# uber-research/UPSNet

Hardware: AMD Instinct MI355X
Metric: images/sec (whole node), UPSNet-50 1024x2048 (higher is better)
Workload: dtype f32

## Files before the change

include/upsnet_hip.h:

```cpp
#ifndef UPSNET_HIP_H
#define UPSNET_HIP_H

#include <stddef.h>
#include <stdint.h>

#ifdef __cplusplus
extern "C" {
#endif

const char *upsnet_last_error(void);
const char *upsnet_last_kernel_form(void);
int upsnet_abi_version(void);

int upsnet_zero_fill(void *stream, void *ptr, size_t bytes);


int upsnet_roi_align_forward(void *stream, const float *bottom_data, float spatial_scale, int num_rois,
                             int height, int width, int channels, int pooled_height, int pooled_width,
                             int sampling_ratio, const float *bottom_rois, float *top_data);

int upsnet_roi_align_forward_nhwc(void *stream, const float *feat_nhwc, int batch, int height, int width,
                                  int channels, float spatial_scale, const float *rois, int num_rois,
                                  int pooled_height, int pooled_width, int sampling_ratio, float *out_nhwc);

int upsnet_fpn_roi_align_forward(void *stream, const float *const feat_nhwc[4], const int feat_h[4],
                                 const int feat_w[4], const float spatial_scale[4], int channels,
                                 const float *rois, int num_rois, const int *num_rois_dev, int pooled_height,
                                 int pooled_width, int sampling_ratio, float *out_nhwc, int *levels_out);

int upsnet_fpn_roi_order(void *stream, const float *rois, int num_rois, const int *num_rois_dev, int image_height, int image_width,
                         int *order_out);
int upsnet_fpn_roi_align_forward_ordered(void *stream, const float *const feat_nhwc[4], const int feat_h[4], const int feat_w[4],
                                         const float spatial_scale[4], int channels, const float *rois, int num_rois, const int *num_rois_dev,
                                         int pooled_height, int pooled_width, int sampling_ratio, float *out_nhwc, int *levels_out,
                                         const int *order);

void upsnet_roi_tuning(int variant);
void upsnet_roi_geometry(int target_workgroups, int min_bins);


int upsnet_deform_im2col(void *stream, const float *data_im, const float *data_offset, int channels,
                         int height, int width, int ksize_h, int ksize_w, int pad_h, int pad_w, int stride_h,
                         int stride_w, int dilation_h, int dilation_w, int parallel_imgs, int deformable_group,
                         float *data_col);

int upsnet_mod_deform_im2col(void *stream, const float *data_im, const float *data_offset,
                             const float *data_mask, int batch_size, int channels, int height_im, int width_im,
                             int height_col, int width_col, int kernel_h, int kernel_w, int pad_h, int pad_w,
                             int stride_h, int stride_w, int dilation_h, int dilation_w, int deformable_group,
                             float *data_col);


int upsnet_roi_align_backward(void *stream, const float *top_diff, float spatial_scale, int batch_size, int num_rois,
                              int height, int width, int channels, int pooled_height, int pooled_width,
                              int sampling_ratio, const float *bottom_rois, float *bottom_diff);

int upsnet_deform_col2im(void *stream, const float *data_col, const float *data_offset, int channels, int height,
                         int width, int ksize_h, int ksize_w, int pad_h, int pad_w, int stride_h, int stride_w,
                         int dilation_h, int dilation_w, int parallel_imgs, int deformable_group, float *grad_im);

int upsnet_deform_col2im_coord(void *stream, const float *data_col, const float *data_im, const float *data_offset,
                               int channels, int height, int width, int ksize_h, int ksize_w, int pad_h, int pad_w,
                               int stride_h, int stride_w, int dilation_h, int dilation_w, int parallel_imgs,
                               int deformable_group, float *grad_offset);

int upsnet_mod_deform_col2im(void *stream, const float *data_col, const float *data_offset, const float *data_mask,
                             int batch_size, int channels, int height_im, int width_im, int height_col, int width_col,
                             int kernel_h, int kernel_w, int pad_h, int pad_w, int stride_h, int stride_w,
                             int dilation_h, int dilation_w, int deformable_group, float *grad_im);

int upsnet_mod_deform_col2im_coord(void *stream, const float *data_col, const float *data_im, const float *data_offset,
                                   const float *data_mask, int batch_size, int channels, int height_im, int width_im,
                                   int height_col, int width_col, int kernel_h, int kernel_w, int pad_h, int pad_w,
                                   int stride_h, int stride_w, int dilation_h, int dilation_w, int deformable_group,
                                   float *grad_offset, float *grad_mask);

int upsnet_deform_conv_forward_nhwc(void *stream, int nlev, const float *const x[], const float *const offset[],
                                    const float *const mask[], float *const out[], const int height[],
                                    const int width[], int cin, int cout, int kh, int kw, int pad_h, int pad_w,
                                    int stride_h, int stride_w, int dil_h, int dil_w, int deformable_group,
                                    const float *wpack, int ldw, const float *bias, int relu);

size_t upsnet_dcn_packed_weight_floats(int cout, int cin, int kh, int kw);
int upsnet_dcn_pack_weight(void *stream, const float *weight, int cout, int cin, int kh, int kw, float *wpack);
int upsnet_deform_conv_fused_nhwc(void *stream, int nlev, const float *const x[], const float *const offset[],
                                  const float *const mask[], float *const out[], const int height[], const int width[],
                                  int cin, int cout, int kh, int kw, int pad, int stride, int dil, const float *wpack,
                                  const float *bias, int relu);
size_t upsnet_deform_conv_fused_splitk_workspace_bytes(int height, int width, int cout, int kh, int kw, int pad, int stride, int dil,
                                                       int ksplit);
int upsnet_deform_conv_fused_nhwc_splitk(void *stream, const float *x, const float *offset, const float *mask, float *out, int height,
                                         int width, int cin, int cout, int kh, int kw, int pad, int stride, int dil,
                                         const float *wpack, const float *bias, int relu, int ksplit, void *workspace);
void upsnet_dcn_tuning(int variant);

size_t upsnet_dcn_packed_weight_bf16_elems(int cout, int cin, int kh, int kw);
int upsnet_dcn_pack_weight_bf16(void *stream, const float *weight, int cout, int cin, int kh, int kw, void *wpack);
int upsnet_deform_conv_fused_nhwc_bf16(void *stream, int nlev, const float *const x[], const float *const offset[],
                                       const float *const mask[], float *const out[], const int height[], const int width[], int cin,
                                       int cout, int kh, int kw, int pad, int stride, int dil, const void *wpack, const float *bias,
                                       int relu);


int upsnet_prep_image_u8(void *stream, const unsigned char *image_hwc, int height, int width, const double pixel_means[3],
                         double im_scale, int resized_h, int resized_w, int padded_h, int padded_w, int nhwc4, float *blob);

int upsnet_image_to_nhwc4(void *stream, const float *nchw, int batch, int channels, int height, int width, float *nhwc4);


int upsnet_conv2d_nhwc_f32_multiw(void *stream, int nseg, const float *const x[], float *const out[], const int batch[],
                                  const int height[], const int width[], int Cin, const float *const wpack[], int ldw, int Cout,
                                  int KH, int KW, int stride, int pad, int relu);

int upsnet_conv2d_nhwc_f32(void *stream, int nseg, const float *const x[], const float *const residual[],
                           float *const out[], const int batch[], const int height[], const int width[], int Cin,
                           const float *wpack, int ldw, const float *bias, int Cout, int KH, int KW, int stride, int pad,
                           int relu, int residual_up);

size_t upsnet_conv2d_splitk_workspace_bytes(int batch, int height, int width, int Cout, int KH, int KW, int stride, int pad, int ksplit);
int upsnet_conv2d_nhwc_f32_splitk(void *stream, const float *x, const float *residual, float *out, int batch, int height, int width,
                                  int Cin, const float *wpack, int ldw, const float *bias, int Cout, int KH, int KW, int stride,
                                  int pad, int relu, int ksplit, void *workspace);

int upsnet_conv2d_winograd_nhwc_f32(void *stream, int nseg, const float *const x[], const float *const residual[],
                                    float *const out[], const int batch[], const int height[], const int width[], int Cin,
                                    const float *wpack, int ldw, const float *bias, int Cout, int relu);

int upsnet_conv2d_winograd_nhwc_f32_splitk(void *stream, const float *x, const float *residual, float *out, int batch, int height,
                                           int width, int Cin, const float *wpack, int ldw, const float *bias, int Cout, int relu,
                                           int ksplit, void *workspace);
int upsnet_conv_pack_weight_winograd(void *stream, const float *weight, int cout, int cin, int ldw, float *wpack);

int upsnet_conv2d_winograd_nhwc_f32_tn32(void *stream, int nseg, const float *const x[], const float *const residual[],
                                         float *const out[], const int batch[], const int height[], const int width[], int Cin,
                                         const float *wpack, int ldw, const float *bias, int Cout, int relu);
int upsnet_conv_pack_weight_winograd_tn32(void *stream, const float *weight, int cout, int cin, int ldw, float *wpack);
int upsnet_conv2d_winograd_nhwc_f32_tail(void *stream, const float *x, float *out, int batch, int n_main, int height, int width, int Cin,
                                         const float *wpack, int ldw, const float *wpack32, int ldw32, const float *bias, int Cout, int relu);

int upsnet_conv2d_nhwc_bf16(void *stream, int nseg, const void *const x[], const void *const residual[], void *const out[],
                            const int batch[], const int height[], const int width[], int Cin, const void *wpack_hi,
                            const void *wpack_lo, int ldw, const float *bias, int Cout, int KH, int KW, int stride, int pad,
                            int relu);
int upsnet_conv_pack_weight_bf16(void *stream, const float *weight, int cout, int cin, int kh, int kw, int ldw, void *wpack_hi,
                                 void *wpack_lo);
int upsnet_bottleneck_proj_bf16(void *stream, const void *x, void *out, int batch, int height_in, int width_in, int cin, int cmid, int stride,
                                const void *w1, const void *w2, const void *w3d, const float *b1, const float *b2, const float *b3d);
int upsnet_conv_bf16_tuning(int enable, int tile_rows);
int upsnet_conv1x1_bf16_tuning(int enable);
int upsnet_stem_pool_pack_weight_f32(void *stream, const float *weight, int cin, float *wpack);
int upsnet_stem_pool_f32(void *stream, const float *x4, int batch, int height, int width, const float *wpack, const float *bias, float *out);
int upsnet_stem_pool_pack_weight_bf16(void *stream, const float *weight, int cin, void *wpack);
int upsnet_stem_pool_bf16(void *stream, const float *x4, int batch, int height, int width, const void *wpack, const float *bias, void *out);
int upsnet_deconv2x2_nhwc_bf16(void *stream, const void *x, int batch, int height, int width, int Cin, const void *wpack_hi, int ldw,
                               const float *bias, int Cout, int relu, void *out, int out_bf16);

int upsnet_bottleneck_bf16(void *stream, const void *x, void *out, int batch, int height, int width, int cmid, const void *w1,
                           const void *w2, const void *w3, const float *b1, const float *b2, const float *b3);

int upsnet_conv2d_stem_nhwc4_f32(void *stream, const float *x, int batch, int height, int width, const float *wpack,
                                 int ldw, const float *bias, int Cout, int KH, int KW, int stride, int pad, int relu,
                                 float *out);
int upsnet_conv_pack_weight_stem(void *stream, const float *weight, int cout, int cin, int kh, int kw, int ldw, float *wpack);

int upsnet_deconv2x2_nhwc_f32(void *stream, const float *x, int batch, int height, int width, int Cin, const float *wpack,
                              int ldw, const float *bias, int Cout, int relu, float *out);
int upsnet_deconv2x2_pack_weight(void *stream, const float *weight, int cin, int cout, int ldw, float *wpack);

int upsnet_deconv2x2_frag_nhwc_f32(void *stream, const float *x, float *out, int batch, int height, int width, int Cin,
                                   const float *wpack, const float *bias4, int Cout, int relu);

void upsnet_conv_tuning(int winograd_tiles, int force_tile);

int upsnet_conv_pack_weight(void *stream, const float *weight, int cout, int cin, int kh, int kw, int ldw, float *wpack);

int upsnet_conv1x1_frag_nhwc_f32(void *stream, const float *x, const float *residual, float *out, int batch, int height, int width,
                                 int Cin, const float *wpack, const float *bias, int Cout, int stride, int relu, int residual_up);
void upsnet_conv1x1_tuning(int bn);
int upsnet_conv1x1_siblings_nhwc_f32(void *stream, const float *x, float *out_a, float *out_b, int batch, int height, int width, int Cin,
                                     const float *wpack, const float *bias, int cout_a, int cout_b, int stride, int relu_a, int relu_b);
void upsnet_conv1x1_pair32_tuning(int waves);

int upsnet_residency_tuning(int kernel, int cap);
size_t upsnet_residency_pad_bytes(int cap, size_t static_lds, size_t dynamic_lds);
int upsnet_residency_last_dynamic_lds(void);

int upsnet_conv2d_winograd36_nhwc_f32(void *stream, int nseg, const float *const x[], float *const out[], const int batch[],
                                      const int height[], const int width[], int Cin, const float *wpack, int ldw, const float *bias,
                                      int Cout, int relu);
int upsnet_conv_pack_weight_winograd36(void *stream, const float *weight, int cout, int cin, int ldw, float *wpack);
size_t upsnet_conv2d_winograd36_splitk_workspace_bytes(int batch, int height, int width, int Cout, int ksplit);
int upsnet_conv2d_winograd36_nhwc_f32_splitk(void *stream, const float *x, float *out, int batch, int height, int width, int Cin,
                                             const float *wpack, int ldw, const float *bias, int Cout, int relu, int ksplit, void *workspace);

size_t upsnet_conv1x1_ksw_packed_weight_floats(int cout, int cin);
int upsnet_conv1x1_ksw_pack_weight(void *stream, const float *weight, int cout, int cin, float *wpack);
int upsnet_conv1x1_ksw_nhwc_f32(void *stream, const float *x, const float *residual, float *out, int batch, int height, int width, int Cin,
                                const float *wpack, const float *bias, int Cout, int stride, int relu, int tile_pixels, int tile_channels,
                                int split_n);
void upsnet_conv1x1_ksw_tuning(int tile);

size_t upsnet_conv3x3_ksw_packed_weight_floats(int cin);
int upsnet_conv3x3_ksw_pack_weight(void *stream, const float *weight, int cout, int cin, float *wpack);
int upsnet_conv3x3_ksw_nhwc_f32(void *stream, const float *x, float *out, int batch, int height, int width, int Cin, const float *wpack,
                                const float *bias, int Cout, int relu);

size_t upsnet_conv1x1_splitk_workspace_bytes(int batch, int out_height, int out_width, int Cout, int ksplit);
int upsnet_conv1x1_frag_nhwc_f32_splitk(void *stream, const float *x, const float *residual, float *out, int batch, int height, int width,
                                        int Cin, const float *wpack, const float *bias, int Cout, int stride, int relu, int ksplit,
                                        void *workspace);

int upsnet_conv1x1_pair_nhwc_f32(void *stream, const float *x, const float *residual, float *out1, float *out2, long pixels, int C0,
                                 const float *w3pack, const float *bias3, int C1, const float *w1pack, const float *bias1, int C2);


int upsnet_nms_host(int *keep_out_host, int *num_out_host, const float *boxes_host, int boxes_num,
                    int boxes_dim, float nms_overlap_thresh, int device_id);

size_t upsnet_nms_workspace_bytes(int num_problems, int nmax);
int upsnet_nms_batched(void *stream, const float *boxes, const float *scores, const int *counts,
                       const uint8_t *pre_removed, int num_problems, int nmax, float thresh, int *keep_idx,
                       int *keep_cnt, void *workspace);

void upsnet_nms_tuning(int lds_staging);

int upsnet_cpu_nms_batched(void *stream, const float *boxes, const float *scores, const int *counts, int num_problems,
                           int nmax, double thresh, int *keep_idx, int *keep_cnt, void *workspace);

size_t upsnet_soft_nms_batched_workspace_bytes(int num_problems, int nmax);
int upsnet_soft_nms_batched(void *stream, float *boxes, int64_t *inds, const int *counts, int num_problems, int nmax,
                            float sigma, float Nt, float threshold, int method, int *n_out, void *workspace);

size_t upsnet_soft_nms_workspace_bytes(int n);
int upsnet_soft_nms(void *stream, float *boxes, int64_t *inds, int n, float sigma, float Nt, float threshold,
                    int method, int *n_out, void *workspace);


size_t upsnet_proposal_workspace_bytes(int nlev, const int *heights_host, const int *widths_host, int num_anchors,
                                       int pre_nms_top_n, int post_nms_top_n);
int upsnet_pyramid_proposals(void *stream, int nlev, const float *const cls_prob[], const float *const bbox_pred[],
                             const int *heights_host, const int *widths_host, const int *strides_host,
                             const float *anchors_host, int num_anchors, const float *im_info, int pre_nms_top_n,
                             int post_nms_top_n, float nms_thresh, float min_size, float *rois_out,
                             float *scores_out, int *num_out, void *workspace);

int upsnet_pyramid_proposals_strided(void *stream, int nlev, const float *const cls_prob[], const float *const bbox_pred[],
                                     const long *cls_chan_stride, const long *cls_pix_stride, const long *box_chan_stride,
                                     const long *box_pix_stride, const int *heights_host, const int *widths_host,
                                     const int *strides_host, const float *anchors_host, int num_anchors, const float *im_info,
                                     int pre_nms_top_n, int post_nms_top_n, float nms_thresh, float min_size, float *rois_out,
                                     float *scores_out, int *num_out, void *workspace);
int upsnet_pyramid_proposals_strided_ordered(void *stream, int nlev, const float *const cls_prob[], const float *const bbox_pred[],
                                     const long *cls_chan_stride, const long *cls_pix_stride, const long *box_chan_stride,
                                     const long *box_pix_stride, const int *heights_host, const int *widths_host,
                                     const int *strides_host, const float *anchors_host, int num_anchors, const float *im_info,
                                     int pre_nms_top_n, int post_nms_top_n, float nms_thresh, float min_size, float *rois_out,
                                     float *scores_out, int *num_out, void *workspace, int *roi_order_out);

int upsnet_pyramid_proposals_joint_strided(void *stream, int nlev, const float *const cls_prob[], const float *const bbox_pred[],
                                           const long *cls_chan_stride, const long *cls_pix_stride, const long *box_chan_stride,
                                           const long *box_pix_stride, const int *heights_host, const int *widths_host,
                                           const int *strides_host, const float *anchors_host, int num_anchors, const float *im_info,
                                           int pre_nms_top_n, int post_nms_top_n, float nms_thresh, float min_size, float *rois_out,
                                           float *scores_out, int *num_out, void *workspace);


int upsnet_mask_roi_capacity(int num_rois, int num_classes, int class_agnostic);
size_t upsnet_mask_roi_workspace_bytes(int num_rois, int num_classes, int class_agnostic);
int upsnet_mask_roi(void *stream, const float *rois, const float *bbox_delta, const float *cls_prob, int num_rois,
                    const int *num_rois_dev, int num_classes, const float *im_info, int class_agnostic,
                    float score_thresh, float nms_thresh, int max_det, const float reg_weights_host[4],
                    float *boxes_out, float *scores_out, int64_t *cls_out, int *src_out, int *num_out,
                    void *workspace);
int upsnet_mask_roi_ex(void *stream, const float *rois, const float *bbox_delta, const float *cls_prob, int num_rois,
                       const int *num_rois_dev, int num_classes, const float *im_info, int class_agnostic, int clip_boxes,
                       float score_thresh, float nms_thresh, int max_det, const float reg_weights_host[4],
                       float *boxes_out, float *scores_out, int64_t *cls_out, int *src_out, int *num_out,
                       void *workspace);

int upsnet_mask_roi_dedup(void *stream, const int *a_src, const int64_t *a_cls, const int *num_a, int cap_a, const int *b_src,
                          const int64_t *b_cls, const float *b_boxes, const int *num_b, int cap_b, int *map_out,
                          float *extra_boxes, int *num_extra);

int upsnet_mask_logit_gather(void *stream, const float *mask_logit, int n_rows, int num_classes, int hw, long stride_n,
                             long stride_c, long stride_e, const int *row, const int64_t *cls, int K, float *out);


size_t upsnet_mask_removal_workspace_bytes(int m, int num_thing_classes, int height, int width);
int upsnet_mask_removal(void *stream, const float *mask_rois, const float *cls_prob, const float *mask_logit,
                        const int64_t *cls_idx, int m, const int *m_dev, int mask_size, int num_thing_classes, int height, int width,
                        double fraction_threshold, int64_t *keep_inds, int *num_keep, int *real_keep,
                        void *workspace);

int upsnet_panoptic_tail_pack(void *stream, const int64_t *keep, const int *num_keep, int K, const int64_t *cls, const float *scores,
                              const int *det_num, const int *pan_num, const int *extra_num, int64_t *kept_cls, float *kept_scores,
                              int *counters);

int upsnet_mask_paste(void *stream, const float *mask_rois, const float *mask_logit, const int64_t *keep_inds,
                      const int *num_keep, const int *real_keep, int kmax, int mask_size, int height, int width,
                      float *mask_energy);

int upsnet_seg_term(void *stream, const float *fcn_output, int num_seg, int height, int width, const float *boxes,
                    const int64_t *cls, const int64_t *class_map, int k, float *seg_inst);

int upsnet_panoptic_fuse(void *stream, const float *fcn_output, int num_seg, int height, int width, int num_stuff,
                         const float *mask_rois, const float *mask_logit, const int64_t *cls_idx,
                         const int64_t *keep_inds, const int *num_keep, const int *real_keep, int kmax,
                         int mask_size, const int64_t *class_map, int enable_void, int64_t *pan_out,
                         int64_t *sem_out);

int upsnet_fcn_score_combine(void *stream, int nlev, const float *const part[], int num_seg, int height, int width,
                             const float *bias, float *score);

int upsnet_panoptic_fuse_up(void *stream, const float *fcn_score, int score_nhwc, int num_seg, int score_h, int score_w,
                            int scale, int num_stuff, const float *mask_rois, const float *mask_logit,
                            const int64_t *cls_idx, const int64_t *keep_inds, const int *num_keep, const int *real_keep,
                            int kmax, int mask_size, const int64_t *class_map, int64_t *pan_out, int64_t *sem_out);

int upsnet_panoptic_fuse_up_conf(void *stream, const float *fcn_score, int score_nhwc, int num_seg, int score_h, int score_w,
                                 int scale, int num_stuff, const float *mask_rois, const float *mask_logit,
                                 const int64_t *cls_idx, const int64_t *keep_inds, const int *num_keep, const int *real_keep,
                                 int kmax, int mask_size, const int64_t *class_map, int64_t *pan_out, int64_t *sem_out,
                                 unsigned char *conf_out);

int upsnet_panoptic_argmax(void *stream, const float *fcn_output, int num_seg, int height, int width, int num_stuff,
                           const float *seg_inst, const float *mask_energy, int k, int enable_void,
                           int64_t *pan_out);


size_t upsnet_unified_pan_workspace_bytes(void);
int upsnet_unified_pan_result(void *stream, const int64_t *pan, const int64_t *seg, const int64_t *cls_inds, int num_inst,
                              int height, int width, int id_last_stuff, int num_seg_classes, int stuff_area_limit,
                              void *workspace, unsigned char *pan_2ch);

size_t upsnet_combined_pan_workspace_bytes(int num_images, long total_pixels);
int upsnet_combined_pan_result(void *stream, int num_images, const int64_t *images, int max_height, int max_width, long total_pixels,
                               const int *cand, const int *segments, int id_last_stuff, int num_classes, int stuff_area_limit,
                               double fraction_threshold, void *workspace);

int upsnet_im_post_rle(void *stream, const float *pred_boxes, const float *mask_prob, const int64_t *cls_inds, int num_det,
                       int num_mask_channels, int mask_size, int im_height, int im_width, int cap, unsigned *transitions,
                       int *transition_count);

int upsnet_restore_label_maps(void *stream, const int64_t *sseg, const int64_t *pano, long src_stride, int src_height, int src_width,
                              const int *y_ofs, int out_height, const int *x_ofs, int out_width, unsigned char *out_sseg,
                              unsigned char *out_pano);

int upsnet_restore_plane_u8(void *stream, const unsigned char *src, long src_stride, int src_height, int src_width, const int *y_ofs,
                            int out_height, const int *x_ofs, int out_width, unsigned char *out);


size_t upsnet_pq_workspace_bytes(int max_gt);
int upsnet_pq_accumulate(void *stream, const unsigned char *pred_2ch, const unsigned char *gt_rgb, int height, int width,
                         const int64_t *segments, int num_segments, const unsigned char *cat_known, int image_index, int max_gt,
                         void *workspace, int64_t *tp, int64_t *fp, int64_t *fn, double *iou, uint64_t *status);

size_t upsnet_pan_boundary_workspace_bytes(int height, int width);
int upsnet_pan_boundary_map(void *stream, int dilation, const unsigned char *pred_2ch, const unsigned char *gt_rgb, int height, int width,
                            void *workspace, unsigned char *out_bits);
size_t upsnet_pq_boundary_workspace_bytes(int max_gt, int height, int width);
int upsnet_pq_boundary_accumulate(void *stream, int dilation, const unsigned char *pred_2ch, const unsigned char *gt_rgb, int height,
                                  int width, const int64_t *segments, int num_segments, const unsigned char *cat_known, int image_index,
                                  int max_gt, void *workspace, int64_t *tp, int64_t *fp, int64_t *fn, double *iou, uint64_t *status);

int upsnet_confusion_accumulate(void *stream, const unsigned char *gt_label, const unsigned char *pred_label, long npix,
                                int class_num, int ignore_label, int64_t *confusion);


size_t upsnet_det_eval_image_workspace_bytes(int num_det, int num_rows, int num_gt, int height, int width, int segm);
int upsnet_det_eval_image(void *stream, int segm, int height, int width, int num_rows, int num_det, const double *det_xyxy,
                          const double *det_score, const int64_t *det_cls, const int *class_to_row, int num_classes,
                          const float *det_box_f32, const float *mask_prob, int num_mask_channels, int mask_size,
                          const int *det_trans, const int64_t *det_trans_off, int num_gt, const int *gt_row_off,
                          const double *gt_box, const double *gt_area, const int *gt_crowd, const int *gt_trans,
                          const int64_t *gt_trans_off, const int *gt_trans_dst, int num_gt_rle, const unsigned char *const *gt_u8,
                          const int *gt_u8_dst, int num_gt_u8, const int *rows_with_gt, int num_rows_with_gt,
                          const double *params, int image_index, void *workspace, double *rec_score, int *rec_img, int *rec_rk,
                          uint64_t *rec_match, uint64_t *rec_ign, int64_t *npig);

size_t upsnet_det_eval_accumulate_workspace_bytes(long num_records, int num_rows);
int upsnet_det_eval_accumulate(void *stream, long num_records, const double *rec_score, const int *rec_img, const int *rec_rk,
                               const uint64_t *rec_match, const uint64_t *rec_ign, const int *img_ord, int num_rows,
                               const int64_t *npig, const double *rec_thrs, void *workspace, double *precision, double *recall,
                               double *scores);

size_t upsnet_det_eval_boundary_image_workspace_bytes(int num_det, int num_rows, int num_gt, int height, int width);
int upsnet_det_eval_boundary_image(void *stream, int dilation, int height, int width, int num_rows, int num_det,
                                   const double *det_score, const int64_t *det_cls, const int *class_to_row, int num_classes,
                                   const float *det_box_f32, const float *mask_prob, int num_mask_channels, int mask_size,
                                   const int *det_trans, const int64_t *det_trans_off, int num_gt, const int *gt_row_off,
                                   const double *gt_area, const int *gt_crowd, const int *gt_trans,
                                   const int64_t *gt_trans_off, const int *gt_trans_dst, int num_gt_rle,
                                   const unsigned char *const *gt_u8, const int *gt_u8_dst, int num_gt_u8, const int *rows_with_gt,
                                   int num_rows_with_gt, const double *params, int image_index, void *workspace, double *rec_score,
                                   int *rec_img, int *rec_rk, uint64_t *rec_match, uint64_t *rec_ign, int64_t *npig);
int upsnet_boundary_dilation_fits(int height, int width, int dilation);

size_t upsnet_boundary_masks_workspace_bytes(int num_masks, int height, int width);
int upsnet_boundary_masks(void *stream, int dilation, int height, int width, int num_masks, const unsigned char *masks_u8,
                          const int *trans, const int64_t *trans_off, void *workspace, unsigned char *boundary_u8, int *boundary_area);

size_t upsnet_poly_raster_workspace_bytes(long total_vertices, long total_points);
int upsnet_poly_raster(void *stream, const double *vertices, const int *poly_off, const int *obj_off, const int *poly_off_dev,
                       const int *obj_off_dev, int num_poly, int num_obj, long total_points, int height, int width, void *workspace,
                       int *trans, int64_t *trans_off);


size_t upsnet_proposal_recall_workspace_bytes(int num_problems, long total_proposals);
int upsnet_proposal_recall(void *stream, int num_problems, const int64_t *problems, const float *proposals, const float *gt_boxes,
                           int max_gt, long total_proposals, void *workspace, float *out);


size_t upsnet_cs_inst_counts_ints(int num_preds);
size_t upsnet_cs_inst_workspace_bytes(int num_preds);
int upsnet_cs_inst_state_words(void);
int upsnet_cs_inst_image(void *stream, const uint16_t *gt_ids, int height, int width, int num_preds, const int *pred_cls,
                         const float *pred_scores, const int *trans, const int *trans_off, const unsigned char *masks, int walk_strided,
                         uint16_t *gt_t, const double *thresholds, int num_thr, int *counts, void *workspace, float *rec_score,
                         unsigned char *rec_cls, unsigned char *rec_code, int64_t *state);


size_t upsnet_cs_pixel_inst_ints(void);
int upsnet_cs_pixel_image(void *stream, const unsigned char *gt_labels, const uint16_t *gt_ids, const unsigned char *pred,
                          const unsigned char *lut, int height, int width, const double *avg_class_size, int64_t *conf, int *inst,
                          double *wsum, int *bad);


size_t upsnet_pan_format_workspace_bytes(void);
size_t upsnet_pan_format_table_ints(void);
int upsnet_pan_format(void *stream, const unsigned char *pred_2ch, int height, int width, const int *cat_table, void *workspace,
                      unsigned char *rgb, int *table);

int upsnet_pan_relabel(void *stream, const unsigned char *rgb, int height, int width, const int *table, int num_segments,
                       int image_index, unsigned char *out_2ch, int *counts, uint64_t *status);


size_t upsnet_gt_prepare_workspace_bytes(int seg_capacity);
int upsnet_gt_prepare(void *stream, const int *ids, const unsigned char *label_ids, int height, int width, const int *train_id,
                      const int *has_instances, const int *thing_row, int seg_capacity, int trans_capacity, void *workspace,
                      unsigned char *train_map, unsigned char *rgb, int *table, int *trans_off, int *trans, int *status);


int upsnet_vis_max_detections(void);
int upsnet_vis_max_label(void);
size_t upsnet_vis_workspace_bytes(int num_dets, int height, int width);
int upsnet_vis_font(unsigned char *cells);
int upsnet_vis_render(void *stream, const unsigned char *image, int height, int width, int num_dets, const float *boxes,
                      const unsigned char *colours, const unsigned char *labels, const int *label_len, const int *trans,
                      const int *trans_off, int num_trans, void *workspace, unsigned char *out);


size_t upsnet_pan_vis_workspace_bytes(void);
size_t upsnet_pan_vis_workspace_zeroed_bytes(void);
int upsnet_pan_vis_max_labels(void);
int upsnet_pan_vis(void *stream, int mode, const unsigned char *pred_2ch, const unsigned char *id_rgb, const int *seg_table,
                   const unsigned char *image, int height, int width, const int *cat_table, const unsigned char *names,
                   const int *name_len, int label_min_area, void *workspace, unsigned char *out, int *info);


int upsnet_group_norm_chunk_pixels(void);
size_t upsnet_group_norm_workspace_bytes(int nseg, const int batch[], const int height[], const int width[]);
int upsnet_group_norm_nhwc_f32(void *stream, int nseg, const float *const x[], float *const out[], const int batch[],
                               const int height[], const int width[], int C, const float *gamma, const float *beta, float eps,
                               int relu, const float *const residual[], const int res_height[], const int res_width[],
                               int residual_up, void *workspace);
int upsnet_group_norm_small_nhwc_f32(void *stream, const float *x, float *out, int batch, int height, int width, int C,
                                     const float *gamma, const float *beta, float eps, int relu);


int upsnet_cs_inst_expand(void *stream, const int *trans, const int *trans_off, int num_masks, int height, int width, int bits,
                          unsigned char *out);


int upsnet_tta_seg_merge(void *stream, int num_aug, const float *const maps[], const int map_h[], const int map_w[], const float q[],
                         const float resized_w[], const int flip[], int cell, int num_seg, int height, int width, float *out);

int upsnet_tta_roi_union(void *stream, int num_aug, const float *const rois[], const float *const delta[], const float *const prob[],
                         const int *const num_rois_dev[], const float r[], const float resized_w[], const int flip[], int capacity,
                         int delta_dim, int num_classes, float *rois_out, float *delta_out, float *prob_out, int *num_out);

int upsnet_tta_boxes_to_aug(void *stream, int num_aug, const float q[], const float resized_w[], const int flip[], const float *boxes,
                            int num_boxes, float *boxes_out);

int upsnet_tta_mask_merge(void *stream, int num_aug, const float *const logits[], const int flip[], int num_rois, int num_classes,
                          int mask_size, int nhwc, float *out);


int upsnet_box_vote(void *stream, const float *rois, const float *bbox_delta, const float *cls_prob, int num_rois,
                    const int *num_rois_dev, int num_classes, const float *im_info, int clip_boxes, const float reg_weights_host[4],
                    float vote_score_thresh, float vote_iou_thresh, const float *boxes, const int64_t *cls, const int *num, int cap,
                    float *voted);


size_t upsnet_mask_roi_soft_workspace_bytes(int num_rois, int num_classes);
int upsnet_mask_roi_soft(void *stream, const float *rois, const float *bbox_delta, const float *cls_prob, int num_rois,
                         const int *num_rois_dev, int num_classes, const float *im_info, int clip_boxes, float score_thresh,
// ... 63 lines not shown
```

upsnet_amd/_lib.py:

```python
import ctypes
import os

import torch

_HERE = os.path.dirname(os.path.abspath(__file__))
LIB_PATH = os.environ.get("UPSNET_LIB_PATH") or os.path.join(_HERE, "csrc", "libupsnet_hip.so")

c_int, c_float, c_double, c_void_p, c_size_t, c_long = ctypes.c_int, ctypes.c_float, ctypes.c_double, ctypes.c_void_p, ctypes.c_size_t, ctypes.c_long
P = c_void_p

_SIGNATURES = {
    "upsnet_last_error": (ctypes.c_char_p, []),
    "upsnet_last_kernel_form": (ctypes.c_char_p, []),
    "upsnet_abi_version": (c_int, []),
    "upsnet_zero_fill": (c_int, [P, P, c_size_t]),
    "upsnet_roi_align_forward": (c_int, [P, P, c_float, c_int, c_int, c_int, c_int, c_int, c_int, c_int, P, P]),
    "upsnet_roi_align_forward_nhwc": (c_int, [P, P, c_int, c_int, c_int, c_int, c_float, P, c_int, c_int, c_int, c_int, P]),
    "upsnet_fpn_roi_align_forward": (c_int, [P, P, P, P, P, c_int, P, c_int, P, c_int, c_int, c_int, P, P]),
    "upsnet_fpn_roi_order": (c_int, [P, P, c_int, P, c_int, c_int, P]),
    "upsnet_fpn_roi_align_forward_ordered": (c_int, [P, P, P, P, P, c_int, P, c_int, P, c_int, c_int, c_int, P, P, P]),
    "upsnet_roi_tuning": (None, [c_int]),
    "upsnet_roi_geometry": (None, [c_int, c_int]),
    "upsnet_deform_im2col": (c_int, [P, P, P] + [c_int] * 13 + [P]),
    "upsnet_mod_deform_im2col": (c_int, [P, P, P, P] + [c_int] * 15 + [P]),
    "upsnet_roi_align_backward": (c_int, [P, P, c_float] + [c_int] * 8 + [P, P]),
    "upsnet_deform_col2im": (c_int, [P, P, P] + [c_int] * 13 + [P]),
    "upsnet_deform_col2im_coord": (c_int, [P, P, P, P] + [c_int] * 13 + [P]),
    "upsnet_mod_deform_col2im": (c_int, [P, P, P, P] + [c_int] * 15 + [P]),
    "upsnet_mod_deform_col2im_coord": (c_int, [P, P, P, P, P] + [c_int] * 15 + [P, P]),
    "upsnet_deform_conv_forward_nhwc": (c_int, [P, c_int, P, P, P, P, P, P] + [c_int] * 11 + [P, c_int, P, c_int]),
    "upsnet_dcn_packed_weight_floats": (c_size_t, [c_int, c_int, c_int, c_int]),
    "upsnet_dcn_pack_weight": (c_int, [P, P, c_int, c_int, c_int, c_int, P]),
    "upsnet_deform_conv_fused_nhwc": (c_int, [P, c_int, P, P, P, P, P, P] + [c_int] * 7 + [P, P, c_int]),
    "upsnet_deform_conv_fused_splitk_workspace_bytes": (c_size_t, [c_int] * 9),
    "upsnet_deform_conv_fused_nhwc_splitk": (c_int, [P, P, P, P, P] + [c_int] * 9 + [P, P, c_int, c_int, P]),
    "upsnet_dcn_tuning": (None, [c_int]),
    "upsnet_dcn_packed_weight_bf16_elems": (c_size_t, [c_int, c_int, c_int, c_int]),
    "upsnet_dcn_pack_weight_bf16": (c_int, [P, P, c_int, c_int, c_int, c_int, P]),
    "upsnet_deform_conv_fused_nhwc_bf16": (c_int, [P, c_int, P, P, P, P, P, P] + [c_int] * 7 + [P, P, c_int]),
    "upsnet_conv1x1_frag_nhwc_f32": (c_int, [P, P, P, P, c_int, c_int, c_int, c_int, P, P, c_int, c_int, c_int, c_int]),
    "upsnet_conv1x1_tuning": (None, [c_int]),
    "upsnet_conv1x1_siblings_nhwc_f32": (c_int, [P, P, P, P, c_int, c_int, c_int, c_int, P, P, c_int, c_int, c_int, c_int, c_int]),
    "upsnet_conv1x1_pair32_tuning": (None, [c_int]),
    "upsnet_residency_tuning": (c_int, [c_int, c_int]),
    "upsnet_residency_pad_bytes": (c_size_t, [c_int, c_size_t, c_size_t]),
    "upsnet_residency_last_dynamic_lds": (c_int, []),
    "upsnet_conv1x1_splitk_workspace_bytes": (ctypes.c_size_t, [c_int, c_int, c_int, c_int, c_int]),
    "upsnet_conv1x1_frag_nhwc_f32_splitk": (c_int, [P, P, P, P, c_int, c_int, c_int, c_int, P, P, c_int, c_int, c_int, c_int, P]),
    "upsnet_conv1x1_ksw_packed_weight_floats": (ctypes.c_size_t, [c_int, c_int]),
    "upsnet_conv1x1_ksw_pack_weight": (c_int, [P, P, c_int, c_int, P]),
    "upsnet_conv1x1_ksw_nhwc_f32": (c_int, [P, P, P, P, c_int, c_int, c_int, c_int, P, P, c_int, c_int, c_int, c_int, c_int, c_int]),
    "upsnet_conv1x1_ksw_tuning": (None, [c_int]),
    "upsnet_conv3x3_ksw_packed_weight_floats": (ctypes.c_size_t, [c_int]),
    "upsnet_conv3x3_ksw_pack_weight": (c_int, [P, P, c_int, c_int, P]),
    "upsnet_conv3x3_ksw_nhwc_f32": (c_int, [P, P, P, c_int, c_int, c_int, c_int, P, P, c_int, c_int]),
    "upsnet_conv2d_winograd36_splitk_workspace_bytes": (ctypes.c_size_t, [c_int, c_int, c_int, c_int, c_int]),
    "upsnet_conv2d_winograd36_nhwc_f32_splitk": (c_int, [P, P, P, c_int, c_int, c_int, c_int, P, c_int, P, c_int, c_int, c_int, P]),
    "upsnet_conv1x1_pair_nhwc_f32": (c_int, [P, P, P, P, P, c_long, c_int, P, P, c_int, P, P, c_int]),
    "upsnet_conv2d_nhwc_f32": (c_int, [P, c_int, P, P, P, P, P, P, c_int, P, c_int, P, c_int, c_int, c_int, c_int, c_int, c_int, c_int]),
    "upsnet_conv2d_nhwc_f32_multiw": (c_int, [P, c_int, P, P, P, P, P, c_int, P, c_int, c_int, c_int, c_int, c_int, c_int, c_int]),
    "upsnet_conv_tuning": (None, [c_int, c_int]),
    "upsnet_conv_pack_weight": (c_int, [P, P, c_int, c_int, c_int, c_int, c_int, P]),
    "upsnet_nms_host": (c_int, [P, P, P, c_int, c_int, c_float, c_int]),
    "upsnet_nms_workspace_bytes": (c_size_t, [c_int, c_int]),
    "upsnet_nms_batched": (c_int, [P, P, P, P, P, c_int, c_int, c_float, P, P, P]),
    "upsnet_nms_tuning": (None, [c_int]),
    "upsnet_cpu_nms_batched": (c_int, [P, P, P, P, c_int, c_int, c_double, P, P, P]),
    "upsnet_soft_nms_batched_workspace_bytes": (c_size_t, [c_int, c_int]),
    "upsnet_soft_nms_batched": (c_int, [P, P, P, P, c_int, c_int, c_float, c_float, c_float, c_int, P, P]),
    "upsnet_soft_nms_workspace_bytes": (c_size_t, [c_int]),
    "upsnet_soft_nms": (c_int, [P, P, P, c_int, c_float, c_float, c_float, c_int, P, P]),
    "upsnet_proposal_workspace_bytes": (c_size_t, [c_int, P, P, c_int, c_int, c_int]),
    "upsnet_pyramid_proposals_strided": (c_int, [P, c_int, P, P, P, P, P, P, P, P, P, P, c_int, P, c_int, c_int, c_float, c_float, P, P, P, P]),
    "upsnet_pyramid_proposals_strided_ordered": (c_int, [P, c_int, P, P, P, P, P, P, P, P, P, P, c_int, P, c_int, c_int, c_float, c_float, P, P, P, P, P]),
    "upsnet_pyramid_proposals_joint_strided": (c_int, [P, c_int, P, P, P, P, P, P, P, P, P, P, c_int, P, c_int, c_int, c_float, c_float, P, P, P, P]),
    "upsnet_pyramid_proposals": (c_int, [P, c_int, P, P, P, P, P, P, c_int, P, c_int, c_int, c_float, c_float, P, P, P, P]),
    "upsnet_mask_roi_capacity": (c_int, [c_int, c_int, c_int]),
    "upsnet_mask_roi_workspace_bytes": (c_size_t, [c_int, c_int, c_int]),
    "upsnet_mask_roi": (c_int, [P, P, P, P, c_int, P, c_int, P, c_int, c_float, c_float, c_int, P, P, P, P, P, P, P]),
    "upsnet_mask_roi_ex": (c_int, [P, P, P, P, c_int, P, c_int, P, c_int, c_int, c_float, c_float, c_int, P, P, P, P, P, P, P]),
    "upsnet_mask_logit_gather": (c_int, [P, P, c_int, c_int, c_int, c_long, c_long, c_long, P, P, c_int, P]),
    "upsnet_mask_removal_workspace_bytes": (c_size_t, [c_int, c_int, c_int, c_int]),
    "upsnet_mask_removal": (c_int, [P, P, P, P, P, c_int, P, c_int, c_int, c_int, c_int, c_double, P, P, P, P]),
    "upsnet_panoptic_tail_pack": (c_int, [P, P, P, c_int, P, P, P, P, P, P, P, P]),
    "upsnet_mask_paste": (c_int, [P, P, P, P, P, P, c_int, c_int, c_int, c_int, P]),
    "upsnet_seg_term": (c_int, [P, P, c_int, c_int, c_int, P, P, P, c_int, P]),
    "upsnet_panoptic_fuse": (c_int, [P, P, c_int, c_int, c_int, c_int, P, P, P, P, P, P, c_int, c_int, P, c_int, P, P]),
    "upsnet_panoptic_fuse_up": (c_int, [P, P, c_int, c_int, c_int, c_int, c_int, c_int, P, P, P, P, P, P, c_int, c_int, P, P, P]),
    "upsnet_panoptic_fuse_up_conf": (c_int, [P, P, c_int, c_int, c_int, c_int, c_int, c_int, P, P, P, P, P, P, c_int, c_int, P, P, P, P]),
    "upsnet_conv2d_stem_nhwc4_f32": (c_int, [P, P, c_int, c_int, c_int, P, c_int, P, c_int, c_int, c_int, c_int, c_int, c_int, P]),
    "upsnet_conv_pack_weight_stem": (c_int, [P, P, c_int, c_int, c_int, c_int, c_int, P]),
    "upsnet_deconv2x2_nhwc_f32": (c_int, [P, P, c_int, c_int, c_int, c_int, P, c_int, P, c_int, c_int, P]),
    "upsnet_deconv2x2_pack_weight": (c_int, [P, P, c_int, c_int, c_int, P]),
    "upsnet_deconv2x2_frag_nhwc_f32": (c_int, [P, P, P, c_int, c_int, c_int, c_int, P, P, c_int, c_int]),
    "upsnet_prep_image_u8": (c_int, [P, P, c_int, c_int, P, c_double, c_int, c_int, c_int, c_int, c_int, P]),
    "upsnet_image_to_nhwc4": (c_int, [P, P, c_int, c_int, c_int, c_int, P]),
    "upsnet_unified_pan_workspace_bytes": (c_size_t, []),
    "upsnet_unified_pan_result": (c_int, [P, P, P, P, c_int, c_int, c_int, c_int, c_int, c_int, P, P]),
    "upsnet_combined_pan_workspace_bytes": (c_size_t, [c_int, c_long]),
    "upsnet_combined_pan_result": (c_int, [P, c_int, P, c_int, c_int, c_long, P, P, c_int, c_int, c_int, c_double, P]),
    "upsnet_mask_roi_dedup": (c_int, [P, P, P, P, c_int, P, P, P, P, c_int, P, P, P]),
    "upsnet_conv2d_winograd_nhwc_f32": (c_int, [P, c_int, P, P, P, P, P, P, c_int, P, c_int, P, c_int, c_int]),
    "upsnet_conv2d_winograd_nhwc_f32_splitk": (c_int, [P, P, P, P, c_int, c_int, c_int, c_int, P, c_int, P, c_int, c_int, c_int, P]),
    "upsnet_conv_pack_weight_winograd": (c_int, [P, P, c_int, c_int, c_int, P]),
    "upsnet_conv_pack_weight_winograd_tn32": (c_int, [P, P, c_int, c_int, c_int, P]),
    "upsnet_conv2d_winograd_nhwc_f32_tn32": (c_int, [P, c_int, P, P, P, P, P, P, c_int, P, c_int, P, c_int, c_int]),
    "upsnet_conv2d_winograd_nhwc_f32_tail": (c_int, [P, P, P, c_int, c_int, c_int, c_int, c_int, P, c_int, P, c_int, P, c_int, c_int]),
    "upsnet_conv2d_winograd36_nhwc_f32": (c_int, [P, c_int, P, P, P, P, P, c_int, P, c_int, P, c_int, c_int]),
    "upsnet_conv_pack_weight_winograd36": (c_int, [P, P, c_int, c_int, c_int, P]),
    "upsnet_conv2d_nhwc_bf16": (c_int, [P, c_int, P, P, P, P, P, P, c_int, P, P, c_int, P, c_int, c_int, c_int, c_int, c_int, c_int]),
    "upsnet_bottleneck_proj_bf16": (c_int, [P, P, P, c_int, c_int, c_int, c_int, c_int, c_int, P, P, P, P, P, P]),
    "upsnet_conv_bf16_tuning": (c_int, [c_int, c_int]),
    "upsnet_conv1x1_bf16_tuning": (c_int, [c_int]),
    "upsnet_stem_pool_pack_weight_f32": (c_int, [P, P, c_int, P]),
    "upsnet_stem_pool_f32": (c_int, [P, P, c_int, c_int, c_int, P, P, P]),
    "upsnet_stem_pool_pack_weight_bf16": (c_int, [P, P, c_int, P]),
    "upsnet_stem_pool_bf16": (c_int, [P, P, c_int, c_int, c_int, P, P, P]),
    "upsnet_deconv2x2_nhwc_bf16": (c_int, [P, P, c_int, c_int, c_int, c_int, P, c_int, P, c_int, c_int, P, c_int]),
    "upsnet_bottleneck_bf16": (c_int, [P, P, P, c_int, c_int, c_int, c_int, P, P, P, P, P, P]),
    "upsnet_conv_pack_weight_bf16": (c_int, [P, P, c_int, c_int, c_int, c_int, c_int, P, P]),
    "upsnet_conv2d_splitk_workspace_bytes": (c_size_t, [c_int, c_int, c_int, c_int, c_int, c_int, c_int, c_int, c_int]),
    "upsnet_conv2d_nhwc_f32_splitk": (c_int, [P, P, P, P, c_int, c_int, c_int, c_int, P, c_int, P, c_int, c_int, c_int, c_int, c_int, c_int, c_int, P]),
    "upsnet_im_post_rle": (c_int, [P, P, P, P, c_int, c_int, c_int, c_int, c_int, c_int, P, P]),
    "upsnet_fcn_score_combine": (c_int, [P, c_int, P, c_int, c_int, c_int, P, P]),
    "upsnet_panoptic_argmax": (c_int, [P, P, c_int, c_int, c_int, c_int, P, P, c_int, c_int, P]),
    "upsnet_pq_workspace_bytes": (c_size_t, [c_int]),
    "upsnet_pq_accumulate": (c_int, [P, P, P, c_int, c_int, P, c_int, P, c_int, c_int, P, P, P, P, P, P]),
    "upsnet_pan_boundary_workspace_bytes": (c_size_t, [c_int, c_int]),
    "upsnet_pan_boundary_map": (c_int, [P, c_int, P, P, c_int, c_int, P, P]),
    "upsnet_pq_boundary_workspace_bytes": (c_size_t, [c_int, c_int, c_int]),
    "upsnet_pq_boundary_accumulate": (c_int, [P, c_int, P, P, c_int, c_int, P, c_int, P, c_int, c_int, P, P, P, P, P, P]),
    "upsnet_restore_label_maps": (c_int, [P, P, P, c_long, c_int, c_int, P, c_int, P, c_int, P, P]),
    "upsnet_restore_plane_u8": (c_int, [P, P, c_long, c_int, c_int, P, c_int, P, c_int, P]),
    "upsnet_confusion_accumulate": (c_int, [P, P, P, c_long, c_int, c_int, P]),
    "upsnet_det_eval_image_workspace_bytes": (c_size_t, [c_int] * 6),
    "upsnet_det_eval_image": (c_int, [P, c_int, c_int, c_int, c_int, c_int, P, P, P, P, c_int, P, P, c_int, c_int, P, P, c_int, P, P, P, P,
                                      P, P, P, c_int, P, P, c_int, P, c_int, P, c_int, P, P, P, P, P, P, P]),
    "upsnet_det_eval_accumulate_workspace_bytes": (c_size_t, [c_long, c_int]),
    "upsnet_det_eval_accumulate": (c_int, [P, c_long, P, P, P, P, P, P, c_int, P, P, P, P, P, P]),
    "upsnet_det_eval_boundary_image_workspace_bytes": (c_size_t, [c_int] * 5),
    "upsnet_det_eval_boundary_image": (c_int, [P, c_int, c_int, c_int, c_int, c_int, P, P, P, c_int, P, P, c_int, c_int, P, P, c_int, P, P, P,
                                               P, P, P, c_int, P, P, c_int, P, c_int, P, c_int, P, P, P, P, P, P, P]),
    "upsnet_boundary_dilation_fits": (c_int, [c_int, c_int, c_int]),
    "upsnet_boundary_masks_workspace_bytes": (c_size_t, [c_int, c_int, c_int]),
    "upsnet_boundary_masks": (c_int, [P, c_int, c_int, c_int, c_int, P, P, P, P, P, P]),
    "upsnet_poly_raster_workspace_bytes": (c_size_t, [c_long, c_long]),
    "upsnet_poly_raster": (c_int, [P, P, P, P, P, P, c_int, c_int, c_long, c_int, c_int, P, P, P]),
    "upsnet_proposal_recall_workspace_bytes": (c_size_t, [c_int, c_long]),
    "upsnet_proposal_recall": (c_int, [P, c_int, P, P, P, c_int, c_long, P, P]),
    "upsnet_cs_inst_counts_ints": (c_size_t, [c_int]),
    "upsnet_cs_inst_workspace_bytes": (c_size_t, [c_int]),
    "upsnet_cs_inst_state_words": (c_int, []),
    "upsnet_cs_inst_image": (c_int, [P, P, c_int, c_int, c_int, P, P, P, P, P, c_int, P, P, c_int, P, P, P, P, P, P]),
    "upsnet_cs_pixel_inst_ints": (c_size_t, []),
    "upsnet_cs_pixel_image": (c_int, [P, P, P, P, P, c_int, c_int, P, P, P, P, P]),
    "upsnet_pan_format_workspace_bytes": (c_size_t, []),
    "upsnet_pan_format_table_ints": (c_size_t, []),
    "upsnet_pan_format": (c_int, [P, P, c_int, c_int, P, P, P, P]),
    "upsnet_pan_relabel": (c_int, [P, P, c_int, c_int, P, c_int, c_int, P, P, P]),
    "upsnet_gt_prepare_workspace_bytes": (c_size_t, [c_int]),
    "upsnet_gt_prepare": (c_int, [P, P, P, c_int, c_int, P, P, P, c_int, c_int, P, P, P, P, P, P, P]),
    "upsnet_vis_max_detections": (c_int, []),
    "upsnet_vis_max_label": (c_int, []),
    "upsnet_vis_workspace_bytes": (c_size_t, [c_int, c_int, c_int]),
    "upsnet_vis_font": (c_int, [P]),
    "upsnet_vis_render": (c_int, [P, P, c_int, c_int, c_int, P, P, P, P, P, P, c_int, P, P]),
    "upsnet_pan_vis_workspace_bytes": (c_size_t, []),
    "upsnet_pan_vis_workspace_zeroed_bytes": (c_size_t, []),
    "upsnet_pan_vis_max_labels": (c_int, []),
    "upsnet_pan_vis": (c_int, [P, c_int, P, P, P, P, c_int, c_int, P, P, P, c_int, P, P, P]),
    "upsnet_group_norm_chunk_pixels": (c_int, []),
    "upsnet_group_norm_workspace_bytes": (c_size_t, [c_int, P, P, P]),
    "upsnet_group_norm_nhwc_f32": (c_int, [P, c_int, P, P, P, P, P, c_int, P, P, c_float, c_int, P, P, P, c_int, P]),
    "upsnet_group_norm_small_nhwc_f32": (c_int, [P, P, P, c_int, c_int, c_int, c_int, P, P, c_float, c_int]),
    "upsnet_cs_inst_expand": (c_int, [P, P, P, c_int, c_int, c_int, c_int, P]),
    "upsnet_tta_seg_merge": (c_int, [P, c_int, P, P, P, P, P, P, c_int, c_int, c_int, c_int, P]),
    "upsnet_tta_roi_union": (c_int, [P, c_int, P, P, P, P, P, P, P, c_int, c_int, c_int, P, P, P, P]),
    "upsnet_tta_boxes_to_aug": (c_int, [P, c_int, P, P, P, P, c_int, P]),
    "upsnet_tta_mask_merge": (c_int, [P, c_int, P, P, c_int, c_int, c_int, c_int, P]),
    "upsnet_box_vote": (c_int, [P, P, P, P, c_int, P, c_int, P, c_int, P, c_float, c_float, P, P, P, c_int, P]),
    "upsnet_mask_roi_soft_workspace_bytes": (c_size_t, [c_int, c_int]),
    "upsnet_mask_roi_soft": (c_int, [P, P, P, P, c_int, P, c_int, P, c_int, c_float, c_float, c_int, P, c_int, c_float, c_float, P, P, P, P, P, P]),
    "upsnet_pan_track_workspace_bytes": (c_size_t, [c_int, c_int]),
    "upsnet_pan_track_stamp_offset": (c_size_t, []),
    "upsnet_pan_track_table_ints": (c_size_t, [c_int, c_int]),
    "upsnet_pan_track_table_offset": (c_size_t, []),
    "upsnet_pan_track_step": (c_int, [P, P, c_int, c_int, c_double, c_int, c_int, P, P, P, P, c_int]),
    "upsnet_pan_track_motion_workspace_bytes": (c_size_t, [c_int, c_int]),
    "upsnet_pan_track_motion_count_offset": (c_size_t, []),
    "upsnet_pan_track_motion_pred_offset": (c_size_t, []),
    "upsnet_pan_track_step_motion": (c_int, [P, P, c_int, c_int, c_double, c_int, c_int, P, P, P, P, c_int, P]),
    "upsnet_pan_stable_colors": (c_int, [P, P, c_int, c_int, P, c_int, P]),
    "upsnet_pan_components_workspace_bytes": (c_size_t, [c_int, c_int]),
    "upsnet_pan_components": (c_int, [P, P, c_int, c_int, c_int, c_int, c_int, P, P, P, P]),
    "upsnet_pan_absorb_workspace_bytes": (c_size_t, [c_int, c_int]),
    "upsnet_pan_absorb": (c_int, [P, P, c_int, c_int, c_int, c_int, c_int, P, P, P, P]),
    "upsnet_pan_segment_scores_workspace_bytes": (c_size_t, []),
    "upsnet_pan_segment_scores_table_ints": (c_size_t, []),
    "upsnet_pan_segment_scores": (c_int, [P, P, P, c_int, c_int, P, P]),
    "upsnet_pan_score_filter": (c_int, [P, P, c_int, c_int, P, c_double, P]),
    "upsnet_video_eval_workspace_bytes": (c_size_t, [c_int, c_int, c_int, c_int]),
    "upsnet_video_eval_sequence_ints": (c_size_t, []),
    "upsnet_video_eval_frame": (c_int, [P, P, P, c_int, c_int, P, c_int, c_int, c_int, P, c_int, c_int, c_int, c_int, P, P, P, P, P, P, P]),
    "upsnet_video_eval_end": (c_int, [P, c_int, c_int, c_int, c_int, P, P, P]),
    "upsnet_mots_eval_workspace_bytes": (c_size_t, [c_int, c_int, c_int]),
    "upsnet_mots_eval_frame": (c_int, [P, P, P, c_int, c_int, P, c_int, c_int, c_int, c_int, P, P, P, P, P]),
    "upsnet_mots_eval_end": (c_int, [P, c_int, c_int, P, c_int, c_int, P, P]),
    "upsnet_pan_rle_transitions": (c_int, [P, P, c_int, c_int, c_int, P, P]),
}

_lib = None


def exported_symbols():
    return sorted(_SIGNATURES)


def lib():
    global _lib
    if _lib is None:
        if not os.path.exists(LIB_PATH):
            raise RuntimeError("upsnet_amd: %s is missing -- build it with `python -m upsnet_amd.build` "
                               "(there is no CPU fallback)" % LIB_PATH)
        l = ctypes.CDLL(LIB_PATH)
        for name, (res, args) in _SIGNATURES.items():
            fn = getattr(l, name)
            fn.restype = res
            fn.argtypes = args
        _lib = l
    return _lib


def check(rc, what):
    if rc != 0:
        raise RuntimeError("upsnet_amd.%s failed: %s" % (what, lib().upsnet_last_error().decode()))


def ptr(t):
    return None if t is None else c_void_p(t.data_ptr())


def stream():
    return c_void_p(torch.cuda.current_stream().cuda_stream)


def require_cuda(*tensors):
    for t in tensors:
        if t is not None and not t.is_cuda:
            raise Exception("not implemented")


def f32c(t):
    if t is None:
        return None
    if t.dtype != torch.float32:
        t = t.float()
    return t.contiguous()


def i32c(t):
    if t is None:
        return None
    if t.dtype != torch.int32:
        t = t.to(torch.int32)
    return t.contiguous()


def i64c(t):
    if t is None:
        return None
    if t.dtype != torch.int64:
        t = t.to(torch.int64)
    return t.contiguous()


def written(t, dtype, what):
    if t is not None and ((dtype is not None and t.dtype != dtype) or not t.is_contiguous()):
        raise ValueError("%s must be a contiguous %s tensor (got %s, strides %s): the kernel writes it, a converted copy would swallow the writes"
                         % (what, 'any-type' if dtype is None else str(dtype).replace('torch.', ''), str(t.dtype).replace('torch.', ''),
                            tuple(t.stride())))
    return t


def nhwc(t):
    return t.contiguous(memory_format=torch.channels_last)


def int_array(vals):
    return (c_int * len(vals))(*[int(v) for v in vals])


def float_array(vals):
    return (c_float * len(vals))(*[float(v) for v in vals])


def ptr_array(tensors):
    return (c_void_p * len(tensors))(*[None if t is None else t.data_ptr() for t in tensors])


def addr(t):
    return t.data_ptr()
```

upsnet_amd/csrc/conv_wino36.hip:

```cpp
#include <cstdlib>
#include <type_traits>
#include "conv_params.h"
#include "upsnet_hip.h"

#define W36_TM 32
#define W36_TN 64
#define W36_PTS 36
#define W36_VBUF (W36_PTS * 4 * W36_TM * 16)
#define W36_BSTEP (2 * W36_TN * 16)
#define W36_STEPS (2 * W36_PTS)
#define W36_XCH (16 * W36_PTS * 64 * 4)
#define W36_RING 3

typedef unsigned w36_uintx4 __attribute__((ext_vector_type(4)));

#define W36_BT(D0, D1, D2, D3, D4, D5)                                                                               \
    {                                                                                                                \
        const float a0_ = D0, a1_ = D1, a2_ = D2, a3_ = D3, a4_ = D4, a5_ = D5;                                       \
        const float e1_ = __builtin_fmaf(-2.25f, a2_, a4_), o1_ = __builtin_fmaf(-2.25f, a1_, a3_);                   \
        const float e3_ = __builtin_fmaf(-0.5625f, a2_, a4_), o3_ = __builtin_fmaf(-0.5625f, a1_, a3_);               \
        D0 = __builtin_fmaf(1.265625f, a0_, __builtin_fmaf(-2.8125f, a2_, a4_));                                     \
        D1 = __builtin_fmaf(0.75f, o1_, e1_);                                                                        \
        D2 = __builtin_fmaf(-0.75f, o1_, e1_);                                                                       \
        D3 = __builtin_fmaf(1.5f, o3_, e3_);                                                                         \
        D4 = __builtin_fmaf(-1.5f, o3_, e3_);                                                                        \
        D5 = __builtin_fmaf(1.265625f, a1_, __builtin_fmaf(-2.8125f, a3_, a5_));                                     \
    }
#define W36_AT(M0, M1, M2, M3, M4, M5, Y0, Y1, Y2, Y3)                                                               \
    {                                                                                                                \
        const float s1_ = (M1) + (M2), d1_ = (M1) - (M2), s2_ = (M3) + (M4), d2_ = (M3) - (M4);                      \
        Y0 = ((M0) + s1_) + s2_;                                                                                     \
        Y1 = __builtin_fmaf(1.5f, d2_, 0.75f * d1_);                                                                 \
        Y2 = __builtin_fmaf(2.25f, s2_, 0.5625f * s1_);                                                              \
        Y3 = __builtin_fmaf(3.375f, d2_, __builtin_fmaf(0.421875f, d1_, (M5)));                                      \
    }

template <bool SK>
__global__ void __launch_bounds__(512, 1) conv_wino36_f32_kernel(const ConvParams p)
{
    extern __shared__ __attribute__((aligned(16))) unsigned char smem_raw[];
    const int tid = threadIdx.x, lane = tid & 63;
    const int wave = __builtin_amdgcn_readfirstlane(tid >> 6);
    const int cb = wave >> 2, pg = wave & 3;
    const int lhalf = lane >> 5, l32 = lane & 31;
    int m_t, n_t, kz = 0;
    {
        const int nt = p.n_tiles;
        const int per = (p.m_tiles + 7) >> 3;
        int bid = (int)blockIdx.x;
        if constexpr (SK) { const int base_grid = 8 * per * nt; kz = bid / base_grid; bid -= kz * base_grid; }
        const int q = bid >> 3;
        n_t = q % nt;
        const int local = q / nt;
        m_t = (bid & 7) * per + local;
        if (local >= per || m_t >= p.m_tiles) return;
    }
    int si = 0;
#pragma unroll
    for (int q = 1; q < CV_MAXSEG; ++q) if (q < p.nseg && m_t >= p.seg[q].tile_start) si = q;
    const ConvSeg sg = p.seg[si];
    const long p0 = (long)(m_t - sg.tile_start) * W36_TM;
    const int nslabs_all = p.Cin >> 4;
    const int s_first = SK ? (kz * nslabs_all) / p.ksplit : 0;
    const int nslabs = SK ? ((kz + 1) * nslabs_all) / p.ksplit - s_first : nslabs_all;
    const long HoWo = (long)sg.Ho * sg.Wo;

    const int ltile = tid >> 4, lch = tid & 15;
    int hrow0, wcol0;
    int hlo, hhi;
    unsigned tbase, nrmask = 0, ncmask = 0;
    bool lane_fix;
    {
        const long pp = p0 + ltile;
        const bool tile_ok = pp < sg.M;
        const long ppc = tile_ok ? pp : sg.M - 1;
        const int n = (int)(ppc / HoWo);
        const int rem = (int)(ppc - (long)n * HoWo);
        const int ty = rem / sg.Wo, tx = rem - ty * sg.Wo;
        const int h0 = 4 * ty - 1;
        hlo = n * sg.H; hhi = tile_ok ? hlo + sg.H : hlo;
        hrow0 = hlo + h0;
        wcol0 = 4 * tx - 1;
#pragma unroll
        for (int r = 0; r < 6; ++r) nrmask |= (h0 + r >= 0 && h0 + r < sg.H) ? 0u : (1u << r);
#pragma unroll
        for (int c = 0; c < 6; ++c) ncmask |= (wcol0 + c >= 0 && wcol0 + c < sg.W) ? 0u : (1u << c);
        lane_fix = tile_ok && (nrmask | ncmask) != 0;
        tbase = (unsigned)(hrow0 * sg.W + wcol0) * (4u * (unsigned)p.Cin) + 4u * (unsigned)lch;
    }
    const bool fix = __builtin_amdgcn_ballot_w64(lane_fix) != 0ull;
    bool risky;
    {
        const long plast = min(p0 + (long)W36_TM, sg.M) - 1;
        const long nl = plast / HoWo;
        const long tyl = (plast - nl * HoWo) / sg.Wo;
        risky = (nl * sg.H + 4 * tyl + 4) * (long)sg.W + 4L * sg.Wo >= (long)sg.N * sg.H * sg.W;
    }
    const unsigned cin4 = 4u * (unsigned)p.Cin;
    const unsigned rowpitch = (unsigned)sg.W * cin4;
    const unsigned cin4_s = __builtin_amdgcn_readfirstlane(cin4);
    const unsigned rowpitch_s = __builtin_amdgcn_readfirstlane((unsigned)sg.W) * cin4_s;
    const unsigned cbase = (unsigned)wcol0 * cin4 + 4u * (unsigned)lch;
#define W36_ROWOFF(R) (((unsigned)min(max(hrow0 + (R), hlo), max(hhi - 1, hlo)) * rowpitch) | ((hrow0 + (R) >= hlo && hrow0 + (R) < hhi) ? 0u : 0x80000000u))
    const size_t xaddr = reinterpret_cast<size_t>(sg.x);
    const unsigned xlo = __builtin_amdgcn_readfirstlane((unsigned)xaddr), xhi = __builtin_amdgcn_readfirstlane((unsigned)(xaddr >> 32));
    const unsigned xbytes = __builtin_amdgcn_readfirstlane((unsigned)(sg.N * sg.H * sg.W) * 4u * (unsigned)p.Cin - (SK ? (unsigned)s_first * 64u : 0u));
    const char *xbase = reinterpret_cast<const char *>(((size_t)xhi << 32) | xlo) + (SK ? (size_t)s_first * 64 : 0);
#define W36_SWZ(Q) ((((Q) & 1) << 2) | (((Q) >> 1) << 1))
    const unsigned st_base = (unsigned)((((lch >> 2) * W36_TM + (ltile ^ W36_SWZ(lch >> 2))) * 16) + (lch & 3) * 4);
    constexpr unsigned XI_PITCH = 4 * W36_TM * 16;
    const unsigned fr_base0 = (unsigned)((lhalf * W36_TM + (l32 ^ W36_SWZ(lhalf))) * 16) + (unsigned)pg * 9u * XI_PITCH;
    const unsigned fr_base1 = (unsigned)(((2 + lhalf) * W36_TM + (l32 ^ W36_SWZ(2 + lhalf))) * 16) + (unsigned)pg * 9u * XI_PITCH;
    const size_t waddr = reinterpret_cast<size_t>(p.w) + ((size_t)n_t * (size_t)nslabs_all + (size_t)s_first) * (W36_STEPS * W36_BSTEP);
    const unsigned wlo = __builtin_amdgcn_readfirstlane((unsigned)waddr), whi = __builtin_amdgcn_readfirstlane((unsigned)(waddr >> 32));
    const __amdgpu_buffer_rsrc_t wrsrc = __builtin_amdgcn_make_buffer_rsrc(reinterpret_cast<void *>(((size_t)whi << 32) | wlo), 0,
                                                                            nslabs * (int)(W36_STEPS * W36_BSTEP), 0x00020000);
    const unsigned b_lane = (unsigned)(lhalf * (W36_TN * 16) + (32 * cb + l32) * 16);
    const int gmax = nslabs * W36_STEPS - 1;

    floatx16 acc[9];
#pragma unroll
    for (int i = 0; i < 9; ++i)
#pragma unroll
        for (int r = 0; r < 16; ++r) acc[i][r] = 0.f;

    float ld[36];
    float4 breg[W36_RING];

#define W36_LOADROW_FAST(R, RS) { unsigned so_ = (unsigned)((R) ? (R) - 1 : 0) * rowpitch_s; asm volatile("" : "+s"(so_));              \
        ld[6 * (R)] = __uint_as_float(__builtin_amdgcn_raw_buffer_load_b32(RS, (R) ? tbase + rowpitch_s : tbase, so_, 0));               \
        _Pragma("unroll") for (int c_ = 1; c_ < 6; ++c_) ld[6 * (R) + c_] = __uint_as_float(__builtin_amdgcn_raw_buffer_load_b32(       \
            RS, ((R) ? tbase + rowpitch_s : tbase) + cin4_s, so_ + (unsigned)(c_ - 1) * cin4_s, 0)); }
#define W36_LOADROW_SAFE(R, RS) { unsigned cb_ = cbase; asm volatile("" : "+v"(cb_)); const unsigned rb_ = W36_ROWOFF(R) + cb_; _Pragma("unroll") for (int c_ = 0; c_ < 6; ++c_) \
        ld[6 * (R) + c_] = __uint_as_float(__builtin_amdgcn_raw_buffer_load_b32(RS, (rb_ + (unsigned)c_ * cin4) | ((ncmask << (30 - c_)) & 0x40000000u), 0, 0)); }
#define W36_FIXROW(R) if (fix) { asm volatile("" ::: "memory"); const unsigned bad_ = ((nrmask >> (R)) & 1u) ? 0x3fu : ncmask;           \
        _Pragma("unroll") for (int c_ = 0; c_ < 6; ++c_) ld[6 * (R) + c_] = ((bad_ >> c_) & 1u) ? 0.f : ld[6 * (R) + c_]; }
#define W36_ROWPASS(R) W36_BT(ld[6 * (R) + 0], ld[6 * (R) + 1], ld[6 * (R) + 2], ld[6 * (R) + 3], ld[6 * (R) + 4], ld[6 * (R) + 5])
#define W36_COLSTASH(J, SB)                                                                                           \
    {                                                                                                                 \
        float c0_ = ld[0 + (J)], c1_ = ld[6 + (J)], c2_ = ld[12 + (J)], c3_ = ld[18 + (J)], c4_ = ld[24 + (J)], c5_ = ld[30 + (J)]; \
        W36_BT(c0_, c1_, c2_, c3_, c4_, c5_)                                                                          \
        *reinterpret_cast<float *>(smem_raw + (SB) + (0 * 6 + (J)) * XI_PITCH) = c0_;                                 \
        *reinterpret_cast<float *>(smem_raw + (SB) + (1 * 6 + (J)) * XI_PITCH) = c1_;                                 \
        *reinterpret_cast<float *>(smem_raw + (SB) + (2 * 6 + (J)) * XI_PITCH) = c2_;                                 \
        *reinterpret_cast<float *>(smem_raw + (SB) + (3 * 6 + (J)) * XI_PITCH) = c3_;                                 \
        *reinterpret_cast<float *>(smem_raw + (SB) + (4 * 6 + (J)) * XI_PITCH) = c4_;                                 \
        *reinterpret_cast<float *>(smem_raw + (SB) + (5 * 6 + (J)) * XI_PITCH) = c5_;                                 \
    }
#define W36_BLOAD(SLOT, G) { const w36_uintx4 v_ = __builtin_amdgcn_raw_buffer_load_b128(wrsrc, b_lane, (unsigned)min((G), gmax) * W36_BSTEP, 0); \
        breg[SLOT] = make_float4(__uint_as_float(v_.x), __uint_as_float(v_.y), __uint_as_float(v_.z), __uint_as_float(v_.w)); }

#pragma unroll
    for (int u = 0; u < W36_RING; ++u) W36_BLOAD(u, 18 * pg + u)
    {
        const __amdgpu_buffer_rsrc_t xr = __builtin_amdgcn_make_buffer_rsrc(const_cast<char *>(xbase), 0, xbytes, 0x00020000);
#pragma unroll
        for (int r = 0; r < 6; ++r) { W36_LOADROW_SAFE(r, xr) }
#pragma unroll
        for (int r = 0; r < 6; ++r) { W36_ROWPASS(r) }
#pragma unroll
        for (int j = 0; j < 6; ++j) { W36_COLSTASH(j, st_base) }
    }
    __syncthreads();
    float4 afr = *reinterpret_cast<const float4 *>(smem_raw + fr_base0);

    auto slab_loop = [&](auto fast_tag) __attribute__((always_inline)) {
    constexpr bool FAST = decltype(fast_tag)::value;
    for (int s = 0; s < nslabs; ++s) {
        const int sn = min(s + 1, nslabs - 1);
        const __amdgpu_buffer_rsrc_t xr = __builtin_amdgcn_make_buffer_rsrc(const_cast<char *>(xbase) + (size_t)sn * 64, 0, xbytes - (unsigned)sn * 64u, 0x00020000);
        const unsigned cur = (s & 1) ? W36_VBUF : 0u, nxt = W36_VBUF - cur;
        const unsigned sb = nxt + st_base;
        const int g0 = s * W36_STEPS + 18 * pg;
#pragma unroll
        for (int u = 0; u < 18; ++u) {
            if (u < 6) { if constexpr (FAST) { W36_LOADROW_FAST(u, xr) } else { W36_LOADROW_SAFE(u, xr) } }
            float4 afn;
            if (u < 17) afn = *reinterpret_cast<const float4 *>(smem_raw + cur + (((u + 1) & 1) ? fr_base1 : fr_base0) + (unsigned)((u + 1) >> 1) * XI_PITCH);
            else afn = *reinterpret_cast<const float4 *>(smem_raw + nxt + fr_base0);
            if (u == 6) { if constexpr (FAST) { W36_FIXROW(0) } W36_ROWPASS(0) }
            if (u == 7) { if constexpr (FAST) { W36_FIXROW(1) } W36_ROWPASS(1) }
            if (u == 8) { if constexpr (FAST) { W36_FIXROW(2) } W36_ROWPASS(2) }
            if (u == 9) { if constexpr (FAST) { W36_FIXROW(3) } W36_ROWPASS(3) }
            if (u == 10) { if constexpr (FAST) { W36_FIXROW(4) } W36_ROWPASS(4) }
            if (u == 11) { if constexpr (FAST) { W36_FIXROW(5) } W36_ROWPASS(5) W36_COLSTASH(0, sb) }
            if (u == 12) { W36_COLSTASH(1, sb) }
            if (u == 13) { W36_COLSTASH(2, sb) }
            if (u == 14) { W36_COLSTASH(3, sb) }
            if (u == 15) { W36_COLSTASH(4, sb) }
            if (u == 16) { W36_COLSTASH(5, sb) }
            const float4 bf = breg[u % W36_RING];
            acc[u >> 1] = __builtin_amdgcn_mfma_f32_32x32x2f32(afr.x, bf.x, acc[u >> 1], 0, 0, 0);
            acc[u >> 1] = __builtin_amdgcn_mfma_f32_32x32x2f32(afr.y, bf.y, acc[u >> 1], 0, 0, 0);
            acc[u >> 1] = __builtin_amdgcn_mfma_f32_32x32x2f32(afr.z, bf.z, acc[u >> 1], 0, 0, 0);
            acc[u >> 1] = __builtin_amdgcn_mfma_f32_32x32x2f32(afr.w, bf.w, acc[u >> 1], 0, 0, 0);
            W36_BLOAD(u % W36_RING, (u + W36_RING < 18 ? g0 : g0 + W36_STEPS - 18) + u + W36_RING)
            if (u == 16) __syncthreads();
            afr = afn;
            __builtin_amdgcn_sched_barrier(0);
        }
    }
    };
    if (risky) slab_loop(std::false_type{}); else slab_loop(std::true_type{});
#undef W36_LOADROW_FAST
#undef W36_LOADROW_SAFE
#undef W36_ROWOFF
#undef W36_FIXROW
#undef W36_ROWPASS
#undef W36_COLSTASH
#undef W36_BLOAD

    const unsigned crow = (unsigned)p.Cout * 4u;
    const size_t oaddr_ = reinterpret_cast<size_t>(SK ? p.partial + (size_t)kz * (size_t)p.m_total * (size_t)p.Cout : sg.out);
    const unsigned obytes_ = __builtin_amdgcn_readfirstlane((unsigned)((long)sg.N * sg.OH * sg.OW) * crow);
    const __amdgpu_buffer_rsrc_t orsrc = __builtin_amdgcn_make_buffer_rsrc(
        reinterpret_cast<void *>(((size_t)(unsigned)__builtin_amdgcn_readfirstlane((unsigned)(oaddr_ >> 32)) << 32) | (unsigned)__builtin_amdgcn_readfirstlane((unsigned)oaddr_)),
        0, (int)obytes_, 0x00020000);
    float *xch = reinterpret_cast<float *>(smem_raw);
#pragma unroll 1
    for (int bb = 0; bb < 2; ++bb) {
        __syncthreads();
        if (cb == bb) {
#pragma unroll
            for (int u = 0; u < 9; ++u)
#pragma unroll
                for (int r = 0; r < 16; ++r) xch[(r * W36_PTS + 9 * pg + u) * 64 + lane] = acc[u][r];
        }
        __syncthreads();
        const int co_ch = n_t * W36_TN + 32 * bb + l32;
        const bool co_ok = co_ch < p.Cout;
        const float bv = (p.bias != nullptr && co_ok) ? p.bias[co_ch] : 0.f;
#pragma unroll 1
        for (int rr = 0; rr < 2; ++rr) {
            const int r = 2 * wave + rr;
            const long pp = p0 + 8 * (r >> 2) + 4 * lhalf + (r & 3);
            float m[36];
#pragma unroll
            for (int x = 0; x < 36; ++x) m[x] = xch[(r * W36_PTS + x) * 64 + lane];
            if (!(co_ok && pp < sg.M)) continue;
            const int n = (int)(pp / HoWo);
            const int rem = (int)(pp - (long)n * HoWo);
            const int ty = rem / sg.Wo, tx = rem - ty * sg.Wo;
            float t[6][4];
#pragma unroll
            for (int i = 0; i < 6; ++i) W36_AT(m[6 * i + 0], m[6 * i + 1], m[6 * i + 2], m[6 * i + 3], m[6 * i + 4], m[6 * i + 5], t[i][0], t[i][1], t[i][2], t[i][3])
#pragma unroll
            for (int c = 0; c < 4; ++c) {
                float y[4];
                W36_AT(t[0][c], t[1][c], t[2][c], t[3][c], t[4][c], t[5][c], y[0], y[1], y[2], y[3])
                const int ox = 4 * tx + c;
#pragma unroll
                for (int a = 0; a < 4; ++a) {
                    const int oy = 4 * ty + a;
                    float v = y[a];
                    if constexpr (!SK) { v = v + bv; if (p.relu) v = fmaxf(v, 0.f); }
                    const unsigned off = (oy < sg.OH && ox < sg.OW) ? (unsigned)((n * sg.OH + oy) * sg.OW + ox) * crow + 4u * (unsigned)co_ch : 0x80000000u;
                    __builtin_amdgcn_raw_buffer_store_b32(__float_as_uint(v), orsrc, off, 0, 0);
                }
            }
        }
    }
}

static int w36_fill(ConvParams &p, const char *who, int nseg, const float *const x[], float *const out[], const int batch[], const int height[],
                    const int width[], int Cin, int Cout, const float *wpack, int ldw, const float *bias, int relu)
{
    UPS_REQUIRE(Cin > 0 && Cin % 32 == 0 && ldw % W36_TN == 0, "%s: Cin %% 32 == 0 and ldw %% 64 == 0 (got %d, %d)", who, Cin, ldw);
    int rc = conv_fill(p, who, nseg, x, nullptr, nullptr, nullptr, out, batch, height, width, Cin, Cout, wpack, ldw, bias, 3, 3, 1, 1, 1, relu);
    if (rc) return rc;
    UPS_REQUIRE((long)W36_PTS * Cin * ldw < (1L << 29), "%s: packed weight exceeds 2 GiB", who);
    int tiles = 0;
    for (int i = 0; i < nseg; ++i) {
        ConvSeg &s = p.seg[i];
        s.OH = s.Ho; s.OW = s.Wo;
        s.Ho = (s.OH + 3) / 4; s.Wo = (s.OW + 3) / 4;
        s.M = (long)s.N * s.Ho * s.Wo;
        UPS_REQUIRE((long)s.N * s.H * s.W * Cin < (1L << 28), "%s: feature map %d exceeds 1 GiB; split the batch", who, i);
        UPS_REQUIRE((long)s.N * s.OH * s.OW * Cout < (1L << 29), "%s: output %d exceeds 2 GiB; split the batch", who, i);
        s.tile_start = tiles;
        tiles += (int)((s.M + W36_TM - 1) / W36_TM);
    }
    p.m_tiles = tiles;
    p.n_tiles = ldw / W36_TN;
    return 0;
}

extern "C" int upsnet_conv2d_winograd36_nhwc_f32(void *stream, int nseg, const float *const x[], float *const out[], const int batch[],
                                                 const int height[], const int width[], int Cin, const float *wpack, int ldw, const float *bias,
                                                 int Cout, int relu)
{
    ConvParams p;
    int rc = w36_fill(p, "conv2d_winograd36_nhwc_f32", nseg, x, out, batch, height, width, Cin, Cout, wpack, ldw, bias, relu);
    if (rc) return rc;
    static std::atomic<unsigned long long> attr_dev{0};
    UPS_ONCE_PER_DEVICE(attr_dev, UPS_CHECK_HIP(hipFuncSetAttribute(reinterpret_cast<const void *>(&conv_wino36_f32_kernel<false>), hipFuncAttributeMaxDynamicSharedMemorySize, W36_XCH)));
    const int grid = 8 * ((p.m_tiles + 7) / 8) * p.n_tiles;
    hipLaunchKernelGGL(conv_wino36_f32_kernel<false>, dim3(grid), dim3(512), W36_XCH, (hipStream_t)stream, p);
    UPS_CHECK_LAUNCH("conv_wino36_f32_kernel");
    ups_set_form("wino36<%d,%d>", W36_TM, W36_TN);
    return 0;
}

extern "C" size_t upsnet_conv2d_winograd36_splitk_workspace_bytes(int batch, int height, int width, int Cout, int ksplit)
{
    return (size_t)ksplit * (size_t)batch * height * width * Cout * sizeof(float);
}

extern "C" int upsnet_conv2d_winograd36_nhwc_f32_splitk(void *stream, const float *x, float *out, int batch, int height, int width, int Cin,
                                                        const float *wpack, int ldw, const float *bias, int Cout, int relu, int ksplit,
                                                        void *workspace)
{
    const float *xs[1] = {x};
    float *os[1] = {out};
    const int nb[1] = {batch}, hh[1] = {height}, ww[1] = {width};
    ConvParams p;
    int rc = w36_fill(p, "conv2d_winograd36_nhwc_f32_splitk", 1, xs, os, nb, hh, ww, Cin, Cout, wpack, ldw, bias, relu);
    if (rc) return rc;
    UPS_REQUIRE(workspace && ksplit >= 2 && ksplit <= 8 && Cin / 16 >= ksplit, "conv2d_winograd36_nhwc_f32_splitk: ksplit 2..8, <= Cin / 16, and a workspace");
    p.ksplit = ksplit;
    p.partial = (float *)workspace;
    p.m_total = (long)batch * height * width;
    UPS_REQUIRE(p.m_total * Cout < (1L << 29), "conv2d_winograd36_nhwc_f32_splitk: output exceeds 2 GiB; split the batch");
    static std::atomic<unsigned long long> attr_dev{0};
    UPS_ONCE_PER_DEVICE(attr_dev, UPS_CHECK_HIP(hipFuncSetAttribute(reinterpret_cast<const void *>(&conv_wino36_f32_kernel<true>), hipFuncAttributeMaxDynamicSharedMemorySize, W36_XCH)));
    const int grid = 8 * ((p.m_tiles + 7) / 8) * p.n_tiles * ksplit;
    hipLaunchKernelGGL(conv_wino36_f32_kernel<true>, dim3(grid), dim3(512), W36_XCH, (hipStream_t)stream, p);
    UPS_CHECK_LAUNCH("conv_wino36_f32_kernel<splitk>");
    ups_set_form("wino36<%d,%d> splitk%d", W36_TM, W36_TN, ksplit);
    return conv_splitk_reduce((hipStream_t)stream, p.partial, ksplit, p.m_total, p.m_total, Cout, bias, nullptr, relu, out);
}

__global__ void conv_pack_weight_wino36_kernel(const float *__restrict__ w, int cout, int cin, int ldw, float *__restrict__ wp)
{
    const long total = (long)ldw * cin;
    const int nslabs = cin >> 4;
    const double G[6][3] = {{64.0 / 81, 0.0, 0.0}, {-128.0 / 243, -32.0 / 81, -8.0 / 27}, {-128.0 / 243, 32.0 / 81, -8.0 / 27},
                            {32.0 / 243, 16.0 / 81, 8.0 / 27}, {32.0 / 243, -16.0 / 81, 8.0 / 27}, {0.0, 0.0, 1.0}};
    for (long idx = (long)blockIdx.x * blockDim.x + threadIdx.x; idx < total; idx += (long)blockDim.x * gridDim.x) {
        const int co = idx % ldw, c = idx / ldw;
        double g[3][3], t[6][3];
#pragma unroll
        for (int a = 0; a < 3; ++a)
#pragma unroll
            for (int b = 0; b < 3; ++b) g[a][b] = co < cout ? (double)w[(((long)co * cin + c) * 3 + a) * 3 + b] : 0.0;
#pragma unroll
        for (int i = 0; i < 6; ++i)
#pragma unroll
            for (int b = 0; b < 3; ++b) t[i][b] = G[i][0] * g[0][b] + G[i][1] * g[1][b] + G[i][2] * g[2][b];
        const long blk = ((long)(co / W36_TN) * nslabs + (c >> 4)) * W36_PTS;
        const int q = (c & 15) >> 2, ci = c & 3, cl = co % W36_TN;
#pragma unroll
        for (int i = 0; i < 6; ++i)
#pragma unroll
            for (int j = 0; j < 6; ++j) {
                const double u = t[i][0] * G[j][0] + t[i][1] * G[j][1] + t[i][2] * G[j][2];
                wp[(((blk + i * 6 + j) * 4 + q) * W36_TN + cl) * 4 + ci] = (float)u;
            }
    }
}

extern "C" int upsnet_conv_pack_weight_winograd36(void *stream, const float *weight, int cout, int cin, int ldw, float *wpack)
{
    UPS_REQUIRE(weight && wpack && cout > 0 && cin > 0 && ldw >= cout, "conv_pack_weight_winograd36: bad args");
    UPS_REQUIRE(cin % 16 == 0 && ldw % W36_TN == 0, "conv_pack_weight_winograd36: Cin %% 16 must be 0 and ldw a multiple of 64");
    const long total = (long)ldw * cin;
    int blocks = (int)((total + 255) / 256);
    if (blocks > 65535) blocks = 65535;
    hipLaunchKernelGGL(conv_pack_weight_wino36_kernel, dim3(blocks), dim3(256), 0, (hipStream_t)stream, weight, cout, cin, ldw, wpack);
    UPS_CHECK_LAUNCH("conv_pack_weight_wino36_kernel");
    return 0;
}
```

upsnet_amd/knobs.py:

```python
import os
import re

_ROOT = os.path.dirname(os.path.abspath(__file__))
_NAME = re.compile(r'UPSNET_[A-Z0-9_]+')

REGISTRY = {
    'UPSNET_ALLOW_LIBRARY_CONV': ('0', 'models/hipconv.py', 'a convolution no hand-written kernel covers runs on the library instead of raising'),
    'UPSNET_BF16_ACT': ('1', 'models/hipconv.py', 'bf16 mode: bf16 activations between the layers (0: fp32 activations)'),
    'UPSNET_BF16_BLOCK': ('1', 'models/hipconv.py', 'bf16 mode: one-launch bottlenecks (0: three launches)'),
    'UPSNET_BF16_BLOCK_MIN_TILES': ('128', 'models/hipconv.py', 'bf16 mode: fewest tiles for the one-launch bottleneck'),
    'UPSNET_BF16_HALO': ('1', 'csrc/conv_bf16.hip', 'bf16 3x3 layers on the haloed-patch kernel (0: general kernel)'),
    'UPSNET_BF16_MIN_WG': ('192', 'models/hipconv.py', 'bf16 mode: fewest workgroups for a bf16 layer'),
    'UPSNET_BF16_MIN_WG_WREG': ('16', 'models/hipconv.py', 'bf16 mode: fewest workgroups for the weights-from-L2 3x3 kernel'),
    'UPSNET_BF16_NARROW_BELOW': ('384', 'csrc/conv_bf16.hip', 'bf16 general kernel: 128 x 64 tiles below this many workgroups'),
    'UPSNET_BF16_PROJ': ('1', 'models/hipconv.py', 'bf16 mode: projection bottlenecks as one launch'),
    'UPSNET_BF16_STEM': ('1', 'models/hipconv.py', 'bf16 mode: fused stem + pool kernel'),
    'UPSNET_BF16_WREG': ('1', 'csrc/conv3x3_wreg_bf16.hip', 'bf16 3x3 layers on the weights-from-L2 kernel'),
    'UPSNET_BF16_WREG1': ('1', 'csrc/conv1x1_wreg_bf16.hip', 'bf16 1x1 layers on the no-LDS kernel where it wins'),
    'UPSNET_BF16_WREG_TH': ('auto', 'csrc/conv3x3_wreg_bf16.hip', 'tile rows of the weights-from-L2 3x3 kernel'),
    'UPSNET_CONV1X1': ('1', 'models/hipconv.py', '1x1 layers on the lean GEMM kernel (0: implicit-GEMM kernel)'),
    'UPSNET_CONV1X1_BALANCE': ('0', 'models/hipconv.py', 'split-K tail for unevenly tiled 1x1 layers'),
    'UPSNET_CONV1X1_MIN_WG': ('256', 'models/hipconv.py', 'fewest workgroups for the lean 1x1 kernel'),
    'UPSNET_CONV1X1_KSW': ('1', 'models/hipconv.py', 'small-tile (16x16x4 fragment) 1x1 kernel for maps the 64-pixel tiles do not fill evenly'),
    'UPSNET_CONV1X1_KSW_MAX_FILL': ('0.75', 'models/hipconv.py', 'use it when the last round of 64-pixel workgroups is less than this full'),
    'UPSNET_CONV3X3_KSW': ('1', 'models/hipconv.py', 'small-tile 3x3 kernel for <= 32-channel layers (offset predictors) on small maps'),
    'UPSNET_CONV1X1_PAIR': ('1', 'models/hipconv.py', 'conv3 + next conv1 in one launch'),
    'UPSNET_CONV1X1_PAIR32_WAVES': ('8', 'ops.py', 'waves per workgroup of the res4 pair kernel'),
    'UPSNET_CONV1X1_PAIR_MIN_TILES': ('1024', 'models/hipconv.py', 'fewest tiles for the res2 pair kernel'),
    'UPSNET_CONV1X1_PAIR_RES3': ('1', 'models/hipconv.py', 'pair kernel on res3'),
    'UPSNET_CONV1X1_PAIR_RES4': ('1', 'models/hipconv.py', 'pair kernel on res4'),
    'UPSNET_CONV1X1_SIBLINGS': ('1', 'models/hipconv.py', 'conv1 + projection shortcut in one launch'),
    'UPSNET_CONV_PRECISION': ('fp32', 'models/hipconv.py', 'fp32 | bf16 | bf16x3 (bench.py --conv-precision)'),
    'UPSNET_DCN_BF16': ('1', 'ops.py', 'bf16 mode: fused deformable convolution on the bf16 cores'),
    'UPSNET_DCN_KERNEL': ('frag', 'ops.py', 'generation of the fused deformable kernel'),
    'UPSNET_DCN_SMALL_GRID': ('0', 'csrc/deform_fused.hip', 'small-grid variant threshold of the fused deformable kernel'),
    'UPSNET_DCN_SPLITK': ('1', 'ops.py', 'split-K for the offset predictors of small maps'),
    'UPSNET_DCN_VARIANT': ('5', 'csrc/deform_fused.hip', 'schedule variant of the fused deformable kernel'),
    'UPSNET_DECONV_FRAG': ('1', 'models/hipconv.py', 'transposed convolution on the lean GEMM kernel'),
    'UPSNET_DIST_BACKEND': ('nccl', 'upsnet_end2end_test.py', 'torch.distributed backend of the harness (gloo when ranks share a GPU)'),
    'UPSNET_EARLY_MASK': ('1', 'models/resnet_upsnet.py', 'mask head on the side stream as soon as the detections exist'),
    'UPSNET_FC_RELU': ('1', 'models/rcnn.py', 'ReLU of fc6 / fc7 in the library GEMM epilogue (0: separate elementwise launch)'),
    'UPSNET_GRAPH': ('1', 'models/resnet_upsnet.py', 'whole forward as one HIP graph'),
    'UPSNET_GRAPH_ALIAS': ('1', 'models/resnet_upsnet.py', 'outputs are views into the graph buffers (0: copies)'),
    'UPSNET_GRAPH_OWN_STREAM': ('0', 'models/resnet_upsnet.py', 'capture / replay on an own stream with one instance'),
    'UPSNET_GRAPH_SLOTS': ('2', 'models/resnet_upsnet.py', 'graph instances per input shape'),
    'UPSNET_HIP_MEMSET': ('0', 'csrc/fill.hip', 'zero scratch with hipMemsetAsync instead of a kernel'),
    'UPSNET_LIB_PATH': ('', '_lib.py', 'path of libupsnet_hip.so (same-box A/B of two builds)'),
    'UPSNET_NMS_LDS': ('0', 'csrc/nms.hip', 'stage the suppression mask in LDS'),
    'UPSNET_NMS_SCAN16': ('1', 'csrc/nms.hip', 'unrolled scan for <= 1024 boxes'),
    'UPSNET_OVERLAP': ('1', 'models/resnet_upsnet.py', 'semantic branch on a side stream'),
    'UPSNET_PIN': ('1', 'upsnet_end2end_test.py', 'pin each rank to its CPU slice'),
    'UPSNET_ROI_KERNEL': ('auto', 'csrc/roi_align.hip', 'ROIAlign kernel variant 0..4; auto = 3 (corner-sharing) for >= 100 bins per ROI, else 0 -- so '
                                                        '"0" is NOT the default; upsnet_roi_tuning(v >= 0) overrides the variable, (v < 0) returns to it'),
    'UPSNET_ROI_XCD_ORDER': ('1', 'ops.py', 'deal the ROIs of the box head\'s ROIAlign launch to the XCDs by image neighbourhood (table written by prop_merge_kernel)'),
    'UPSNET_ROI_XCD_ORDER_MIN': ('512', 'ops.py', 'only for launches with at least this many ROIs'),
    'UPSNET_ROI_XCD_ORDER_STANDALONE': ('0', 'ops.py', 'build the table with a launch of its own for ROI sets that do not come from pyramid_proposals'),
    'UPSNET_ROI_PER_BIN': ('0', 'csrc/roi_align.hip', 'one wave per (roi, bin) (older decomposition)'),
    'UPSNET_SHARE_GPU': ('0', 'upsnet_end2end_test.py', 'let N ranks share one GPU (functional runs of the N > 1 path)'),
    'UPSNET_SPLITK': ('1', 'models/hipconv.py', 'split-K forms for small maps'),
    'UPSNET_STEM_POOL': ('1', 'models/hipconv.py', 'fused stem + pool kernel (0: stem kernel + library pool)'),
    'UPSNET_WINO36': ('1', 'models/hipconv.py', 'largest 3x3 / stride 1 layers on the Winograd F(4x4,3x3) kernel'),
    'UPSNET_WINO36_SPLITK': ('0', 'models/hipconv.py', 'res3 / res4 conv2 and FPN P4 on the split-K F(4x4) form (3-5 us per launch; more rounding error)'),
    'UPSNET_WINO36_PREFIX': ('0', 'models/hipconv.py', 'multi-map F(4x4) launches keep only the leading maps that fill whole rounds of workgroups (measured: no gain)'),
    'UPSNET_WINO36_ROI': ('1', 'models/hipconv.py', 'mask head (ROI batches) on the Winograd F(4x4,3x3) kernel (0: F(2x2) with the half-size tail)'),
    'UPSNET_WINO36_MIN_FILL': ('0.65', 'models/hipconv.py', 'F(4x4,3x3) only if its last round of workgroups is at least this full'),
    'UPSNET_WINOGRAD': ('1', 'models/hipconv.py', '3x3 / stride 1 layers on the Winograd kernel'),
    'UPSNET_WINOGRAD_MIN_WG': ('128', 'models/hipconv.py', 'fewest workgroups for the Winograd kernel'),
    'UPSNET_WINO_TAIL_FUSED': ('1', 'models/hipconv.py', 'mask-head tail inside the main launch (0: two launches)'),
    'UPSNET_WINO_TAIL_SPLIT': ('1', 'models/hipconv.py', 'mask-head tail on half-size workgroups'),
    'UPSNET_WINO_TM64_MIN': ('768', 'models/hipconv.py', '64-tile Winograd workgroups above this many'),
}


def known():
    return set(REGISTRY)


def scan_sources():
    names = set()
    files = [os.path.join(os.path.dirname(_ROOT), 'bench.py')]
    for d, _, fs in os.walk(_ROOT):
        files += [os.path.join(d, f) for f in fs if f.endswith(('.py', '.hip', '.cpp', '.h')) and f != 'knobs.py']
    for f in files:
        try:
            with open(f, errors='ignore') as fh:
                names.update(_NAME.findall(fh.read()))
        except OSError:
            pass
    return names


def active(env=None):
    env = os.environ if env is None else env
    return {k: env[k] for k in sorted(env) if k.startswith('UPSNET_')}


def check(env=None):
    act = active(env)
    unknown = sorted(set(act) - known())
    if unknown:
        raise ValueError('unknown UPSNET_* environment variable(s) %s -- no source file reads them (typo?)' % ', '.join(unknown))
    return act
```

upsnet_amd/models/fpn.py:

```python
import torch.nn as nn
import torch.nn.functional as F

from ..config.config import config
from . import hipconv


class FPN(nn.Module):

    def __init__(self, feature_dim, with_extra_level=True, with_bottom_up_path_aggregation=False, with_norm='none',
                 upsample_method='nearest'):
        super(FPN, self).__init__()
        assert upsample_method in ['nearest', 'bilinear']
        norm = hipconv.head_norm(with_norm)
        self.feature_dim = feature_dim
        self.upsample_method = upsample_method
        if with_extra_level:
            self.fpn_p6 = nn.MaxPool2d(kernel_size=1, stride=2)
        if config.network.fpn_with_gap:
            self.fpn_gap = nn.Linear(2048, feature_dim)
        self.with_norm = with_norm
        if norm is not None:
            for name, cin in (('fpn_p5_1x1', 2048), ('fpn_p4_1x1', 1024), ('fpn_p3_1x1', 512), ('fpn_p2_1x1', 256)):
                setattr(self, name, nn.Sequential(nn.Conv2d(cin, feature_dim, 1, bias=False), norm(feature_dim)))
            for name in ('fpn_p5', 'fpn_p4', 'fpn_p3', 'fpn_p2'):
                setattr(self, name, nn.Sequential(nn.Conv2d(feature_dim, feature_dim, 3, padding=1, bias=False), norm(feature_dim)))
        else:
            self.fpn_p5_1x1 = nn.Conv2d(2048, feature_dim, 1)
            self.fpn_p4_1x1 = nn.Conv2d(1024, feature_dim, 1)
            self.fpn_p3_1x1 = nn.Conv2d(512, feature_dim, 1)
            self.fpn_p2_1x1 = nn.Conv2d(256, feature_dim, 1)
            self.fpn_p5 = nn.Conv2d(feature_dim, feature_dim, 3, padding=1)
            self.fpn_p4 = nn.Conv2d(feature_dim, feature_dim, 3, padding=1)
            self.fpn_p3 = nn.Conv2d(feature_dim, feature_dim, 3, padding=1)
            self.fpn_p2 = nn.Conv2d(feature_dim, feature_dim, 3, padding=1)
        self.initialize()

    def initialize(self):
        for m in self.modules():
            if isinstance(m, nn.Conv2d):
                nn.init.kaiming_uniform_(m.weight.data, a=1)
                if m.bias is not None:
                    m.bias.data.zero_()

    def fpn_upsample(self, x):
        return F.interpolate(x, scale_factor=2, mode=self.upsample_method,
                             align_corners=False if self.upsample_method == 'bilinear' else None)

    def _forward_norm(self, res2, res3, res4, res5):
        cn = lambda seq, x, **kw: hipconv.norm(seq[1], hipconv.conv(seq[0], x), **kw)
        p5_1x1 = cn(self.fpn_p5_1x1, res5)
        if hasattr(self, 'fpn_gap'):
            gap = self.fpn_gap(F.adaptive_avg_pool2d(res5.float(), (1, 1)).flatten(1)).view(-1, self.feature_dim, 1, 1)
            p5_1x1 = p5_1x1 + gap
        if self.upsample_method == 'nearest' and all(t.shape[2] % 2 == 0 and t.shape[3] % 2 == 0 for t in (res2, res3, res4)):
            up = lambda t: dict(residual=t, residual_up=True)
        else:
            up = lambda t: dict(residual=self.fpn_upsample(t))
        p4_plus = cn(self.fpn_p4_1x1, res4, **up(p5_1x1))
        p3_plus = cn(self.fpn_p3_1x1, res3, **up(p4_plus))
        p2_plus = cn(self.fpn_p2_1x1, res2, **up(p3_plus))
        p5, p4, p3, p2 = (cn(seq, x) for seq, x in ((self.fpn_p5, p5_1x1), (self.fpn_p4, p4_plus), (self.fpn_p3, p3_plus), (self.fpn_p2, p2_plus)))
        if hasattr(self, 'fpn_p6'):
            return p2, p3, p4, p5, self.fpn_p6(p5)
        return p2, p3, p4, p5

    def forward(self, res2, res3, res4, res5):
        if self.with_norm != 'none':
            return self._forward_norm(res2, res3, res4, res5)
        p5_1x1 = hipconv.conv(self.fpn_p5_1x1, res5)
        if hasattr(self, 'fpn_gap'):
            gap = self.fpn_gap(F.adaptive_avg_pool2d(res5.float(), (1, 1)).flatten(1)).view(-1, self.feature_dim, 1, 1)
            p5_1x1 = p5_1x1 + gap
        if self.upsample_method == 'nearest' and all(t.shape[2] % 2 == 0 and t.shape[3] % 2 == 0 for t in (res2, res3, res4)):
            ad = hipconv.act_dtype()
            p4_plus = hipconv.conv(self.fpn_p4_1x1, res4, residual=p5_1x1, residual_up=True)
            p3_plus = hipconv.conv(self.fpn_p3_1x1, res3, residual=p4_plus, residual_up=True, out_dtype=ad)
            p2_plus = hipconv.conv(self.fpn_p2_1x1, res2, residual=p3_plus, residual_up=True, out_dtype=ad)
        else:
            p4_plus = hipconv.conv(self.fpn_p4_1x1, res4, residual=self.fpn_upsample(p5_1x1))
            p3_plus = hipconv.conv(self.fpn_p3_1x1, res3, residual=self.fpn_upsample(p4_plus))
            p2_plus = hipconv.conv(self.fpn_p2_1x1, res2, residual=self.fpn_upsample(p3_plus))
        p5 = hipconv.conv(self.fpn_p5, p5_1x1)
        p4 = hipconv.conv(self.fpn_p4, p4_plus)
        p3 = hipconv.conv(self.fpn_p3, p3_plus)
        p2 = hipconv.conv(self.fpn_p2, p2_plus)
        if hasattr(self, 'fpn_p6'):
            return p2, p3, p4, p5, self.fpn_p6(p5)
        return p2, p3, p4, p5
```

upsnet_amd/models/hipconv.py:

```python
import collections
import os

import torch
import torch.nn as nn
import torch.nn.functional as F

from .. import group_norm, ops

ENABLED = True
ALLOW_LIBRARY = os.environ.get('UPSNET_ALLOW_LIBRARY_CONV', '0') == '1'
FALLBACKS = []
TRACE = None


def _library(m, x, why):
    if x.is_cuda:
        FALLBACKS.append((repr(m), why))
        if not ALLOW_LIBRARY:
            raise RuntimeError('upsnet_amd.hipconv: %r on a CUDA tensor %s is not covered by the hand-written kernels (%s); set '
                               'UPSNET_ALLOW_LIBRARY_CONV=1 to run it on the library convolution' % (m, tuple(x.shape), why))


def _trace(kind, **kw):
    if TRACE is not None:
        kw['kind'] = kind
        TRACE.append(kw)


WINOGRAD = os.environ.get('UPSNET_WINOGRAD', '1') != '0'
WINOGRAD_MIN_WORKGROUPS = int(os.environ.get('UPSNET_WINOGRAD_MIN_WG', '128'))
WINO_TM64_MIN = int(os.environ.get('UPSNET_WINO_TM64_MIN', '768'))
WINO36 = os.environ.get('UPSNET_WINO36', '1') != '0'
WINO36_ROI = os.environ.get('UPSNET_WINO36_ROI', '1') != '0'
WINO36_MIN_FILL = float(os.environ.get('UPSNET_WINO36_MIN_FILL', '0.65'))
WINO36_SPLITK = os.environ.get('UPSNET_WINO36_SPLITK', '0') != '0'
SPLITK = os.environ.get('UPSNET_SPLITK', '1') != '0'
CONV1X1 = os.environ.get('UPSNET_CONV1X1', '1') != '0'
CONV1X1_MIN_WG = int(os.environ.get('UPSNET_CONV1X1_MIN_WG', '256'))
PRECISION = os.environ.get('UPSNET_CONV_PRECISION', 'fp32')
BF16_ACT = os.environ.get('UPSNET_BF16_ACT', '1') != '0'


def act_dtype():
    return torch.bfloat16 if (PRECISION == 'bf16' and BF16_ACT) else torch.float32


def _pack(m, slot, pack, *extra):
    return ops.cached_pack(m, slot, (m.weight, m.bias), lambda: pack(m.weight.detach()), *extra)


def _out_hw(m, x):
    k, st, pd, dl = m.kernel_size[0], m.stride[0], m.padding[0], m.dilation[0]
    return (x.shape[2] + 2 * pd - dl * (k - 1) - 1) // st + 1, (x.shape[3] + 2 * pd - dl * (k - 1) - 1) // st + 1


def _out_pixels(m, xs):
    pix = 0
    for x in xs:
        ho, wo = _out_hw(m, x)
        pix += x.shape[0] * ho * wo
    return pix


def _plain(m, k, pad, strides=(1,)):
    return (tuple(m.kernel_size) == (k, k) and tuple(m.padding) == (pad, pad) and m.stride[0] == m.stride[1] and m.stride[0] in strides and
            tuple(m.dilation) == (1, 1) and m.groups == 1)


def _tiles(x, t):
    return -(-x.shape[2] // t) * -(-x.shape[3] // t)


def _wino_workgroups(m, xs, tm=64):
    tiles = sum(-(-(x.shape[0] * _tiles(x, 2)) // tm) for x in xs)
    return tiles * (1 if m.out_channels <= 32 else -(-m.out_channels // 64))


def _wino36_workgroups(m, xs):
    return [-(-(x.shape[0] * _tiles(x, 4)) // 32) * (m.out_channels // 64) for x in xs]


def _ldw32(cout):
    return (cout + 31) // 32 * 32


def _plan(m):
    return _pack(m, 'direct', ops.pack_conv_weight)


def _conv1x1_plan(m):
    return _pack(m, 'c1x1', ops.pack_conv1x1_weight)


def _use_conv1x1(m, x, always=False):
    if not (CONV1X1 and _plain(m, 1, 0, (1, 2)) and m.in_channels % 32 == 0 and m.out_channels >= 32):
        return False
    if always:
        return True
    return -(-_out_pixels(m, [x]) // 64) * -(-m.out_channels // 64) >= CONV1X1_MIN_WG


BALANCE = os.environ.get('UPSNET_CONV1X1_BALANCE', '0') == '1'
_BAL_OVERHEAD_US = 6.0
_BAL_STEP_US = 0.49
_CUS = {}


def _cus(device):
    if device.index not in _CUS:
        _CUS[device.index] = torch.cuda.get_device_properties(device).multi_processor_count
    return _CUS[device.index]


def _c1_bn(m_tiles, cout):
    return 128 if (cout > 64 and m_tiles * -(-cout // 128) >= 512) else 64


def _c1_walk_us(m_tiles, cin, cout):
    bn = _c1_bn(m_tiles, cout)
    return m_tiles * -(-cout // bn), (cin // 32) * (2 if bn == 128 else 1) * _BAL_STEP_US


def _c1_best_split(wgs, walk_us, nsl, cus):
    best, best_t = 1, -(-wgs // cus) * walk_us
    for ks in range(2, min(16, nsl // 2) + 1):
        if -(-nsl // ks) * (ks - 1) >= nsl:
            continue
        t = -(-wgs * ks // cus) * (walk_us / ks) + _BAL_OVERHEAD_US
        if t < best_t - 1.0:
            best, best_t = ks, t
    return best, best_t


def _c1_balance(m, x, cus=None):
    M = _out_pixels(m, [x])
    if not BALANCE or m.stride[0] != 1:
        return M, 1
    cus = cus or _cus(x.device)
    cin, cout, nsl = m.in_channels, m.out_channels, m.in_channels // 32
    m_tiles = -(-M // 64)
    wgs, walk = _c1_walk_us(m_tiles, cin, cout)
    plain = -(-wgs // cus) * walk
    if wgs % cus == 0 or wgs >= 8 * cus:
        return M, 1
    nt = wgs // m_tiles
    main_tiles = (wgs // cus) * cus // nt
    main_t = 0.0
    if main_tiles > 0:
        mw, mwalk = _c1_walk_us(main_tiles, cin, cout)
        main_t = -(-mw // cus) * mwalk
    tw, twalk = _c1_walk_us(m_tiles - main_tiles, cin, cout)
    ks, tail_t = _c1_best_split(tw, twalk, nsl, cus)
    if ks == 1 or main_t + tail_t + (_BAL_OVERHEAD_US if main_tiles else 0.0) >= plain - 1.0:
        return M, 1
    return main_tiles * 64, ks


def _conv1x1_balanced(m, x, rows_main, ks, relu, residual):
    wp = _conv1x1_plan(m)
    x = ops.nhwc(x.float())
    N, C, H, W = x.shape
    M, co = N * H * W, m.out_channels
    out = ops._nhwc_out(N, co, H, W, x.device)
    slab = lambda t, c: t.permute(0, 2, 3, 1).reshape(M, c)
    img = lambda rows, c: rows.view(1, 1, rows.shape[0], c).permute(0, 3, 1, 2)
    xr, orow = slab(x, C), slab(out, co)
    rr = None if residual is None else slab(ops.nhwc(residual.float()), co)
    if rows_main:
        ops.conv1x1_frag(img(xr[:rows_main], C), wp, m.bias, co, 1, relu=relu, residual=None if rr is None else img(rr[:rows_main], co),
                         out=img(orow[:rows_main], co))
    ops.conv1x1_frag(img(xr[rows_main:], C), wp, m.bias, co, 1, relu=relu, residual=None if rr is None else img(rr[rows_main:], co),
                     out=img(orow[rows_main:], co), ksplit=ks)
    return out


KSW = os.environ.get('UPSNET_CONV1X1_KSW', '1') != '0'
KSW_MAX_FILL = float(os.environ.get('UPSNET_CONV1X1_KSW_MAX_FILL', '0.75'))
KSW_TILE = (16, 64)


def _ksw_plan(m):
    return _pack(m, 'ksw', ops.pack_conv1x1_ksw_weight)


def _use_ksw(m, x, cus=None):
    if not (KSW and PRECISION == 'fp32' and x.dtype == torch.float32 and _plain(m, 1, 0, (1, 2)) and m.in_channels % 16 == 0 and
            m.out_channels % 4 == 0 and m.in_channels >= 256 and m.in_channels >= 2 * m.out_channels):
        return False
    m_tiles = -(-_out_pixels(m, [x]) // 64)
    wgs = m_tiles * -(-m.out_channels // _c1_bn(m_tiles, m.out_channels))
    cus = cus or _cus(x.device)
    return wgs < KSW_MAX_FILL * -(-wgs // cus) * cus


KSW3 = os.environ.get('UPSNET_CONV3X3_KSW', '1') != '0'


def _ksw3_plan(m):
    return _pack(m, 'ksw3', ops.pack_conv3x3_ksw_weight)


def _use_ksw3(m, x):
    return KSW3 and PRECISION == 'fp32' and x.dtype == torch.float32 and _plain(m, 3, 1) and m.out_channels <= 32 and m.in_channels % 16 == 0


PAIR = os.environ.get('UPSNET_CONV1X1_PAIR', '1') != '0'
PAIR_MIN_TILES = int(os.environ.get('UPSNET_CONV1X1_PAIR_MIN_TILES', '1024'))


PAIR_RES3 = os.environ.get('UPSNET_CONV1X1_PAIR_RES3', '1') != '0'
PAIR_RES4 = os.environ.get('UPSNET_CONV1X1_PAIR_RES4', '1') != '0'


def use_pair(m3, m1, x, residual):
    if not (PAIR and CONV1X1 and PRECISION == 'fp32' and supported(m3, x) and residual is not None and isinstance(m1, nn.Conv2d)):
        return False
    if not (_plain(m3, 1, 0) and _plain(m1, 1, 0) and m3.out_channels % 128 == 0 and m1.in_channels == m3.out_channels):
        return False
    tiles = _out_pixels(m3, [x]) // 64
    if m3.in_channels == 64 and m1.out_channels == 64:
        return tiles >= PAIR_MIN_TILES
    if PAIR_RES3 and m3.in_channels == 128 and m1.out_channels == 128:
        return tiles >= PAIR_MIN_TILES // 2
    if PAIR_RES4 and m3.in_channels == 256 and m1.out_channels == 256:
        return 2 * tiles >= PAIR_MIN_TILES // 4
    return False


def conv_pair(m3, m1, x, residual):
    out1, out2 = ops.conv1x1_pair(x, residual, _conv1x1_plan(m3), m3.bias, m3.out_channels, _conv1x1_plan(m1), m1.bias, m1.out_channels)
    _trace('conv', module=m3, x=x, out=out1, relu=True, residual=residual, residual_up=False, form='pair(conv3)')
    _trace('conv', module=m1, x=out1, out=out2, relu=True, residual=None, residual_up=False, form='pair(conv1)')
    return out1, out2


SIBLINGS = os.environ.get('UPSNET_CONV1X1_SIBLINGS', '1') != '0'


def use_siblings(ma, mb, x):
    if not (SIBLINGS and CONV1X1 and PRECISION == 'fp32' and isinstance(ma, nn.Conv2d) and isinstance(mb, nn.Conv2d) and supported(ma, x) and
            supported(mb, x) and x.dtype == torch.float32):
        return False
    if not (_use_conv1x1(ma, x) and _use_conv1x1(mb, x)):
        return False
    return (_plain(ma, 1, 0, (1, 2)) and _plain(mb, 1, 0, (1, 2)) and ma.stride == mb.stride and ma.in_channels == mb.in_channels and ma.in_channels % 32 == 0 and
            ma.out_channels % 32 == 0 and (ma.bias is None) == (mb.bias is None))


def conv_siblings(ma, mb, x, relu_a=True, relu_b=False):
    wp, b = ops.cached_pack(ma, 'siblings', (ma.weight, ma.bias, mb.weight, mb.bias), lambda: (
        ops.pack_conv1x1_weight(torch.cat([ma.weight.detach(), mb.weight.detach()], 0)),
        None if ma.bias is None else torch.cat([ma.bias.detach(), mb.bias.detach()], 0).contiguous()))
    ya, yb = ops.conv1x1_siblings(x, wp, b, ma.out_channels, mb.out_channels, ma.stride[0], relu_a=relu_a, relu_b=relu_b)
    _trace('conv', module=ma, x=x, out=ya, relu=relu_a, residual=None, residual_up=False, form='conv1x1 siblings(a)')
    _trace('conv', module=mb, x=x, out=yb, relu=relu_b, residual=None, residual_up=False, form='conv1x1 siblings(b)')
    return ya, yb


def supported(m, x):
    return (ENABLED and isinstance(m, nn.Conv2d) and x.is_cuda and
            (x.dtype == torch.float32 or (x.dtype == torch.bfloat16 and PRECISION == 'bf16')) and
            ops.conv_supported(m.in_channels, m.kernel_size[0], m.kernel_size[1], m.groups, m.dilation) and
            m.stride[0] == m.stride[1] and m.padding[0] == m.padding[1] and m.padding_mode == 'zeros')


BF16_MIN_WG = int(os.environ.get('UPSNET_BF16_MIN_WG', '192'))
BF16_MIN_WG_WREG = int(os.environ.get('UPSNET_BF16_MIN_WG_WREG', '16'))


def _use_bf16(m, xs, always=False):
    if PRECISION == 'fp32' or m.kernel_size[0] * m.kernel_size[1] > 9 or m.out_channels < 64:
        return False
    if always or xs[0].dtype == torch.bfloat16:
        return True
    k, st, dl = m.kernel_size[0], m.stride[0], m.dilation[0]
    wgs = sum(-(-_out_pixels(m, [x]) // 128) for x in xs)
    small_ok = PRECISION == 'bf16' and k == 3 and st == 1 and dl == 1 and m.out_channels % 256 == 0
    return wgs * -(-m.out_channels // 128) >= (BF16_MIN_WG_WREG if small_ok else BF16_MIN_WG)


def _bf16_form():
    return PRECISION if TRACE is None else '%s %s' % (PRECISION, ops.last_kernel_form())


def _bf16_plan(m):
    return _pack(m, 'bf16', lambda w: ops.pack_conv_weight_bf16(w, split=(PRECISION == 'bf16x3')), PRECISION)


BF16_BLOCK = os.environ.get('UPSNET_BF16_BLOCK', '1') != '0'
BF16_BLOCK_MIN_TILES = int(os.environ.get('UPSNET_BF16_BLOCK_MIN_TILES', '128'))
BF16_PROJ = os.environ.get('UPSNET_BF16_PROJ', '1') != '0'


def use_block(blk, x):
    if not (ENABLED and BF16_BLOCK and PRECISION == 'bf16' and BF16_ACT and x.is_cuda and x.dtype == torch.bfloat16 and not blk.deformable):
        return False
    c1, c2, c3 = blk.conv1, blk.conv2, blk.conv3
    cm, cin, st = c1.out_channels, c1.in_channels, c1.stride[0]
    plain = lambda m, k, p, s=1: _plain(m, k, p, (s,))
    if not (plain(c2, 3, 1) and plain(c3, 1, 0) and c2.in_channels == cm and c2.out_channels == cm and c3.in_channels == cm and
            c3.out_channels == 4 * cm):
        return False
    ho, wo = _out_hw(c1, x)
    th, tw = {64: (8, 16), 128: (8, 8)}.get(cm, (4, 8))
    if x.shape[0] * -(-ho // th) * -(-wo // tw) < BF16_BLOCK_MIN_TILES or x.shape[0] * ho * wo * 4 * cm >= (1 << 30):
        return False
    if blk.downsample is None:
        return cm in (64, 128, 256, 512) and plain(c1, 1, 0) and cin == 4 * cm
    pr = blk.downsample[0]
    return (BF16_PROJ and isinstance(pr, nn.Conv2d) and len(blk.downsample) == 2 and isinstance(blk.downsample[1], nn.Identity) and
            st in (1, 2) and plain(c1, 1, 0, st) and plain(pr, 1, 0, st) and pr.in_channels == cin and pr.out_channels == 4 * cm and
            (cm, cin) in ((64, 64), (128, 256), (256, 512)))


def block(blk, x):
    ms = (blk.conv1, blk.conv2, blk.conv3) + (() if blk.downsample is None else (blk.downsample[0],))
    pack = ops.pack_bottleneck_bf16 if blk.downsample is None else ops.pack_bottleneck_proj_bf16
    p = ops.cached_pack(blk.conv1, 'block16', [t for m in ms for t in (m.weight, m.bias)], lambda: pack(*(m.weight for m in ms), *(m.bias for m in ms)))
    if blk.downsample is None:
        y = ops.bottleneck_bf16(x, p)
    else:
        y = ops.bottleneck_proj_bf16(x, p, blk.conv1.stride[0])
    _trace('block', module=blk, x=x, out=y, form='bottleneck_bf16' if blk.downsample is None else 'bottleneck_proj_bf16')
    return y


def _winograd_plan(m, tn32=False):
    return _pack(m, 'wino32' if tn32 else 'wino', lambda w: ops.pack_winograd_weight(w, tn32=tn32))


WINO_TAIL_SPLIT = os.environ.get('UPSNET_WINO_TAIL_SPLIT', '1') != '0'


def _wino_tail_split(m, x, tm=None):
    if not WINO_TAIL_SPLIT or x.shape[0] < 2 or m.out_channels % 64:
        return 0
    cus = _cus(x.device)
    n, tiles, nt = x.shape[0], _tiles(x, 2), m.out_channels // 64
    slots = 2 * cus
    wgs = _wino_workgroups(m, [x], 32)
    if wgs <= slots or (_wino_tm(m, [x]) if tm is None else tm) != 32:
        return 0
    n_main = ((wgs // slots) * slots // nt) * 32 // tiles
    fit = (cus // (m.out_channels // 32)) * 32 // tiles
    n_main = min(n_main, n - fit) if n - fit > 0 else n_main
    tail = n - n_main
    if n_main <= 0 or tail <= 0 or -(-(tail * tiles) // 32) * (m.out_channels // 32) > cus:
        return 0
    return n_main


WINO_TAIL_FUSED = os.environ.get('UPSNET_WINO_TAIL_FUSED', '1') != '0'


def _wino_split_launch(m, x, n_main, relu):
    wp, ldw = _winograd_plan(m)
    if WINO_TAIL_FUSED:
        wp32, ldw32 = _winograd_plan(m, tn32=True)
        return ops.conv2d_winograd_tail(x, wp, ldw, wp32, ldw32, m.bias, m.out_channels, n_main, relu=relu)
    out = ops._nhwc_out(x.shape[0], m.out_channels, x.shape[2], x.shape[3], x.device)
    ops.conv2d_winograd_multi([x[:n_main]], wp, ldw, m.bias, m.out_channels, relu=relu, outs=[out[:n_main]])
    wp32, ldw32 = _winograd_plan(m, tn32=True)
    ops.conv2d_winograd_multi([x[n_main:]], wp32, ldw32, m.bias, m.out_channels, relu=relu, outs=[out[n_main:]], tn32=True)
    return out


def _winograd36_plan(m):
    return _pack(m, 'wino36', ops.pack_winograd36_weight)


def _winograd36_shape_ok(m):
    return _plain(m, 3, 1) and m.in_channels % 32 == 0 and m.out_channels % 64 == 0


def _use_winograd36(m, xs):
    if not (WINO36 and WINOGRAD and _winograd36_shape_ok(m) and all(x.dtype == torch.float32 for x in xs)):
        return False
    cus = _cus(xs[0].device)
    wgs = sum(_wino36_workgroups(m, xs))
    if cus // 2 <= wgs < cus and m.in_channels >= 256:
        return True
    return wgs >= cus and wgs >= WINO36_MIN_FILL * (-(-wgs // cus)) * cus


WINO36_PREFIX = os.environ.get('UPSNET_WINO36_PREFIX', '0') != '0'


def _wino36_round_prefix(m, xs):
    n = len(xs)
    if not WINO36_PREFIX or n < 2:
        return n
    cus = _cus(xs[0].device)
    per = _wino36_workgroups(m, xs)
    fill = lambda w: w / float(-(-w // cus) * cus)
    last = sum(per) % cus
    if last == 0 or last >= cus // 2:
        return n
    for k in range(n - 1, 0, -1):
        w = sum(per[:k])
        if w >= cus and fill(w) >= 0.95:
            return k
    return n


def _wino36_ksplit(m, x):
    if not (WINO36 and WINOGRAD and _winograd36_shape_ok(m) and x.dtype == torch.float32):
        return 1
    cus = _cus(x.device)
    wgs = _wino36_workgroups(m, [x])[0]
    if wgs >= cus or wgs < cus // 4 or (wgs >= cus // 2 and m.in_channels >= 256):
        return 1
    ks = min(cus // wgs, (m.in_channels // 16) // 4, 8)
    return ks if ks >= 2 else 1


def _wino_choice(m, xs, always=False):
    if not (WINOGRAD and _plain(m, 3, 1) and m.in_channels % 16 == 0):
        return None
    tm = _wino_tm(m, xs)
    ks = 1 if always else _wino_ksplit(m, xs, tm)
    return (tm, ks) if always or _wino_workgroups(m, xs, tm) * ks >= WINOGRAD_MIN_WORKGROUPS else None


def _use_winograd(m, xs, always=False):
    return _wino_choice(m, xs, always) is not None


def _wino_tm(m, xs):
    return 64 if m.out_channels > 32 and _wino_workgroups(m, xs, 64) > WINO_TM64_MIN else 32


def _wino_ksplit(m, xs, tm=None):
    if not SPLITK or len(xs) != 1 or m.out_channels % 4 or (_wino_tm(m, xs) if tm is None else tm) == 64:
        return 1
    wgs, slabs = _wino_workgroups(m, xs, 32), m.in_channels // 16
    if wgs >= 256:
        return 1
    k = 1
    while k < 8 and wgs * (k + 1) <= 512 and slabs // (k + 1) >= 4:
        k += 1
    return k


def _ksplit(m, x, ldw):
    if not SPLITK:
        return 1
    pix = _out_pixels(m, [x])
    slabs = m.kernel_size[0] * m.kernel_size[0] * m.in_channels // 32
    if ldw == 32:
        blocks, ks = -(-pix // 128), 1
        while ks < 8 and blocks * (ks + 1) <= 384 and slabs // (ks + 1) >= 6:
            ks += 1
        while ks > 1 and -(-slabs // ks) * (ks - 1) >= slabs:
            ks -= 1
        return ks
    if ldw % 64 or m.out_channels % 4:
        return 1
    blocks = -(-pix // 64) * (ldw // 64)
    if blocks <= 128 and slabs >= 32:
        return 4
    if blocks <= 256 and slabs >= 128:
        return 3
    return 1


Route = collections.namedtuple('Route', 'launcher form ksplit n_main prefix tile out_dtype widen_x widen_residual',
                               defaults=(1, 0, None, None, torch.float32, False, False))
_Map = collections.namedtuple('_Map', 'shape dtype device is_cuda')


def _same_geometry(ms):
    m0 = ms[0]
    return all(isinstance(m, nn.Conv2d) and m.kernel_size == m0.kernel_size and m.stride == m0.stride and m.padding == m0.padding and
               m.dilation == m0.dilation and m.in_channels == m0.in_channels and (m.bias is None) == (m0.bias is None) for m in ms)


def route(m, xs, residual=None, residual_up=False, winograd=True, pin=False, out_dtype=None, multi=False, cat=None):
    pinned, sfx, widen = pin or winograd == 'always', ' multi' if multi else '', {}
    if multi:
        if len(xs) > 5 or not all(supported(m, x) for x in xs):
            return Route('per_map', None)
        x, use16 = xs[0], _use_bf16(m, xs)
    else:
        x = xs[0]
        ok = supported(m, x)
        if not ok and x.dtype == torch.bfloat16:
            x = _Map(x.shape, torch.float32, x.device, x.is_cuda)
            ok = supported(m, x)
        use16 = ok and _use_bf16(m, [x], always=pinned)
        if not use16 and x.dtype == torch.bfloat16:
            x = _Map(x.shape, torch.float32, x.device, x.is_cuda)
        widen = dict(widen_x=x.dtype != xs[0].dtype, widen_residual=residual is not None and residual.dtype == torch.bfloat16 and not use16)
        if not ok:
            return Route('library', 'library', **widen)
        xs = [x]
    f32, bare = x.dtype == torch.float32, residual is None
    if use16 and (not residual_up or tuple(m.kernel_size) == (1, 1)):
        return Route('bf16', PRECISION, out_dtype=out_dtype if (out_dtype == torch.bfloat16 and PRECISION != 'bf16x3') else torch.float32, **widen)
    if winograd is True and not pinned and bare:
        if WINO36_SPLITK and not multi:
            ks = _wino36_ksplit(m, x)
            if ks > 1:
                return Route('wino36', 'winograd36 splitk%d' % ks, ksplit=ks, **widen)
        if _use_winograd36(m, xs):
            return Route('wino36', 'winograd36' + sfx, prefix=_wino36_round_prefix(m, xs), **widen)
    if winograd == 'always' and WINO36 and WINO36_ROI and bare and f32 and _winograd36_shape_ok(m) and x.shape[2] * x.shape[3] <= 1024:
        return Route('wino36', 'winograd36 roi', **widen)
    wino = _wino_choice(m, xs, winograd == 'always') if (winograd and not residual_up) else None
    if wino:
        tm, ks = wino
        if ks > 1 and not multi:
            return Route('wino', 'winograd splitk%d' % ks, ksplit=ks, **widen)
        n_main = _wino_tail_split(m, x, tm) if (bare and f32 and not multi) else 0
        if n_main:
            return Route('wino', 'winograd tm32 + tail tn32', n_main=n_main, **widen)
        return Route('wino', 'winograd tm%d%s' % (tm, sfx), **widen)
    if not multi:
        if not pinned and bare and _use_ksw3(m, x):
            return Route('ksw3', 'conv3x3 ksw 16x32', **widen)
        if not pinned and not residual_up and _use_ksw(m, x):
            return Route('ksw', 'conv1x1 ksw %dx%d' % KSW_TILE, tile=KSW_TILE, **widen)
        if _use_conv1x1(m, x, always=pinned):
            if not pinned and not residual_up and m.stride[0] == 1:
                rows_main, ks = _c1_balance(m, x)
                if ks > 1:
                    return Route('c1x1', 'conv1x1 %s splitk%d' % ('main + tail' if rows_main else 'all', ks), ksplit=ks, n_main=rows_main, **widen)
            return Route('c1x1', 'conv1x1', **widen)
        ks = 1 if (residual_up or pinned) else _ksplit(m, x, _ldw32(m.out_channels))
        if ks > 1:
            return Route('igemm', 'igemm splitk%d' % ks, ksplit=ks, **widen)
    if cat is not None and f32 and _ldw32(sum(c.out_channels for c in cat)) == 32 and _same_geometry(cat):
        return Route('cat', 'igemm multi cat')
    return Route('igemm', 'igemm' + sfx, **widen)


def _each(t):
    return None if t is None else [t]


def _launch_library(m, xs, r, relu, residual, residual_up):
    _library(m, xs[0], 'hipconv.supported() is false')
    y = m(xs[0])
    if residual is not None:
        y = y + (F.interpolate(residual, scale_factor=2, mode='nearest') if residual_up else residual)
    return [F.relu(y, inplace=True) if relu else y]


def _launch_bf16(m, xs, r, relu, residual, residual_up):
    hi, lo, ldw = _bf16_plan(m)
    return ops.conv2d_nhwc_bf16_multi(xs, hi, lo, ldw, m.bias, m.out_channels, m.kernel_size[0], m.stride[0], m.padding[0], relu=relu,
                                      residuals=_each(residual), residual_up=residual_up, out_dtype=r.out_dtype)


def _launch_wino36(m, xs, r, relu, residual, residual_up):
    wp, ldw = _winograd36_plan(m)
    if r.ksplit > 1:
        return [ops.conv2d_winograd36_splitk(xs[0], wp, ldw, m.bias, m.out_channels, r.ksplit, relu=relu)]
    return ops.conv2d_winograd36_multi(xs, wp, ldw, m.bias, m.out_channels, relu=relu)


def _launch_wino(m, xs, r, relu, residual, residual_up):
    if r.n_main:
        return [_wino_split_launch(m, xs[0], r.n_main, relu)]
    wp, ldw = _winograd_plan(m)
    if r.ksplit > 1:
        return [ops.conv2d_winograd_splitk(xs[0], wp, ldw, m.bias, m.out_channels, r.ksplit, relu=relu, residual=residual)]
    return ops.conv2d_winograd_multi(xs, wp, ldw, m.bias, m.out_channels, relu=relu, residuals=_each(residual))


def _launch_ksw3(m, xs, r, relu, residual, residual_up):
    return [ops.conv3x3_ksw(xs[0], _ksw3_plan(m), m.bias, m.out_channels, relu=relu)]


def _launch_ksw(m, xs, r, relu, residual, residual_up):
    return [ops.conv1x1_ksw(xs[0], _ksw_plan(m), m.bias, m.out_channels, r.tile, stride=m.stride[0], relu=relu, residual=residual)]


def _launch_c1x1(m, xs, r, relu, residual, residual_up):
    if r.ksplit > 1:
        return [_conv1x1_balanced(m, xs[0], r.n_main, r.ksplit, relu, residual)]
    return [ops.conv1x1_frag(xs[0], _conv1x1_plan(m), m.bias, m.out_channels, m.stride[0], relu=relu, residual=residual, residual_up=residual_up)]


def _launch_igemm(m, xs, r, relu, residual, residual_up):
    wp, ldw = _plan(m)
    geom = (m.out_channels, m.kernel_size[0], m.stride[0], m.padding[0])
    if r.ksplit > 1:
        return [ops.conv2d_nhwc_splitk(xs[0], wp, ldw, m.bias, *geom, r.ksplit, relu=relu, residual=residual)]
    return ops.conv2d_nhwc_multi(xs, wp, ldw, m.bias, *geom, relu=relu, residuals=_each(residual), residual_up=residual_up)


def _launch_cat(ms, xs, r, relu, residual, residual_up):
    m0 = ms[0]
    (wp, ldw), b = ops.cached_pack(m0, 'cat', [t for m in ms for t in (m.weight, m.bias)], lambda: (
        ops.pack_conv_weight(torch.cat([m.weight.detach() for m in ms], 0)),
        None if m0.bias is None else torch.cat([m.bias.detach() for m in ms], 0)))
    return ops.conv2d_nhwc_multi(xs, wp, ldw, b, sum(m.out_channels for m in ms), m0.kernel_size[0], m0.stride[0], m0.padding[0], relu=relu)


_LAUNCH = {'library': _launch_library, 'bf16': _launch_bf16, 'wino36': _launch_wino36, 'wino': _launch_wino, 'ksw3': _launch_ksw3, 'ksw': _launch_ksw,
           'c1x1': _launch_c1x1, 'igemm': _launch_igemm, 'cat': _launch_cat}


def _form(r):
    return _bf16_form() if r.launcher == 'bf16' else r.form


def conv(m, x, relu=False, residual=None, residual_up=False, winograd=True, pin=False, out_dtype=None):
    r = route(m, [x], residual, residual_up, winograd, pin, out_dtype)
    if r.widen_x:
        x = x.float()
    if r.widen_residual:
        residual = residual.float()
    y = _LAUNCH[r.launcher](m, [x], r, relu, residual, residual_up)[0]
    _trace('conv', module=m, x=x, out=y, relu=relu, residual=residual, residual_up=residual_up, form=_form(r))
    return y


def conv_multi(m, xs, relu=False):
    xs = list(xs)
    r = route(m, xs, multi=True)
    if r.launcher == 'per_map':
        return [conv(m, x, relu=relu) for x in xs]
    n = len(xs) if r.prefix is None else r.prefix
    ys = _LAUNCH[r.launcher](m, xs[:n], r, relu, None, False)
    form = _form(r)
    for x, y in zip(xs, ys):
        _trace('conv', module=m, x=x, out=y, relu=relu, residual=None, residual_up=False, form=form)
    return ys if n == len(xs) else ys + conv_multi(m, xs[n:], relu=relu)


def conv_multi_cat(ms, xs, return_flat=False):
    xs = list(xs)
    r = route(ms[0], xs, multi=True, cat=ms)
    if r.launcher != 'cat':
        res = [conv_multi(m, xs) for m in ms]
        return (res, None, None) if return_flat else res
    outs = _LAUNCH['cat'](ms, xs, r, False, None, False)
    res, c0 = [], 0
    for m in ms:
        res.append([o[:, c0:c0 + m.out_channels] for o in outs])
        for x, y in zip(xs, res[-1]):
            _trace('conv', module=m, x=x, out=y, relu=False, residual=None, residual_up=False, form=r.form)
        c0 += m.out_channels
    if return_flat:
        return res, getattr(outs[0], '_ups_flat', None), outs
    return res


def stem_supported(m, x):
    return (ENABLED and isinstance(m, nn.Conv2d) and x.is_cuda and x.dtype == torch.float32 and m.in_channels <= 4 and
            m.kernel_size[1] <= 8 and m.groups == 1 and tuple(m.dilation) == (1, 1) and m.stride[0] == m.stride[1] and
            m.padding[0] == m.padding[1] and m.padding_mode == 'zeros')


def conv_stem(m, x, relu=False):
    if not stem_supported(m, x):
        _library(m, x, 'hipconv.stem_supported() is false')
        y = m(x[:, :m.in_channels] if x.shape[1] != m.in_channels else x)
        return F.relu(y, inplace=True) if relu else y
    wp, ldw = _pack(m, 'stem', ops.pack_stem_weight)
    is_nhwc4 = x.shape[1] == 4 and x.is_contiguous(memory_format=torch.channels_last)
    x4 = x if is_nhwc4 else ops.image_to_nhwc4(x)
    y = ops.conv2d_stem(x4, wp, ldw, m.bias, m.out_channels, m.kernel_size[0], m.kernel_size[1], m.stride[0], m.padding[0], relu=relu)
    _trace('conv', module=m, x=x4[:, :m.in_channels], out=y, relu=relu, residual=None, residual_up=False, form='stem')
    return y


STEM_POOL = os.environ.get('UPSNET_STEM_POOL', '1') != '0'
BF16_STEM = os.environ.get('UPSNET_BF16_STEM', '1') != '0'


def _stem_geometry(m, x):
    return (ENABLED and stem_supported(m, x) and m.out_channels == 64 and m.in_channels <= 3 and tuple(m.kernel_size) == (7, 7) and
            tuple(m.stride) == (2, 2) and tuple(m.padding) == (3, 3))


def use_stem_pool(m, x):
    if not _stem_geometry(m, x):
        return None
    if PRECISION == 'bf16' and BF16_ACT and BF16_STEM:
        return 'bf16'
    return 'f32' if STEM_POOL else None


def stem_pool(m, x):
    kind = use_stem_pool(m, x)
    wp = _pack(m, 'stem_pool_' + kind, ops.pack_stem_pool_weight_bf16 if kind == 'bf16' else ops.pack_stem_pool_weight_f32)
    is_nhwc4 = x.shape[1] == 4 and x.is_contiguous(memory_format=torch.channels_last)
    x4 = x if is_nhwc4 else ops.image_to_nhwc4(x)
    y = ops.stem_pool_bf16(x4, wp, m.bias) if kind == 'bf16' else ops.stem_pool_f32(x4, wp, m.bias)
    _trace('stem_pool', module=m, x=x4[:, :m.in_channels], out=y, form='stem + pool bf16' if kind == 'bf16' else 'stem + pool')
    return y


DECONV_FRAG = os.environ.get('UPSNET_DECONV_FRAG', '1') != '0'


def deconv2x2(m, x, relu=False):
    geom = (ENABLED and isinstance(m, nn.ConvTranspose2d) and x.is_cuda and tuple(m.kernel_size) == (2, 2) and
            tuple(m.stride) == (2, 2) and tuple(m.padding) == (0, 0) and tuple(m.output_padding) == (0, 0) and m.groups == 1 and
            tuple(m.dilation) == (1, 1) and m.in_channels % 32 == 0)
    if geom and x.dtype == torch.bfloat16 and PRECISION == 'bf16' and m.in_channels % 64 == 0 and m.out_channels % 32 == 0:
        whi, ldw = _pack(m, 'deconv16', ops.pack_deconv2x2_weight_bf16)
        y = ops.deconv2x2_bf16(x, whi, ldw, m.bias, m.out_channels, relu=relu)
        _trace('deconv', module=m, x=x, out=y, relu=relu, form='deconv2x2 bf16')
        return y
    if x.dtype == torch.bfloat16:
        x = x.float()
    ok = geom and x.dtype == torch.float32
    if not ok:
        _library(m, x, 'not a 2x2 / stride-2 transposed convolution with Cin % 32 == 0')
        y = m(x)
        return F.relu(y, inplace=True) if relu else y
    if DECONV_FRAG and m.out_channels % 32 == 0:
        wp, bias4 = _pack(m, 'deconv_frag', lambda w: ops.pack_deconv2x2_weight_frag(w, m.bias))
        y = ops.deconv2x2_frag(x, wp, bias4, m.out_channels, relu=relu)
        _trace('deconv', module=m, x=x, out=y, relu=relu, form='deconv2x2 frag')
        return y
    wp, ldw = _pack(m, 'deconv', ops.pack_deconv2x2_weight)
    y = ops.deconv2x2(x, wp, ldw, m.bias, m.out_channels, relu=relu)
    _trace('deconv', module=m, x=x, out=y, relu=relu, form='deconv2x2')
    return y


def dcn(m, x, offset, relu=False):
    if (ENABLED and x.is_cuda and x.shape[0] == 1 and not torch.is_grad_enabled() and
            ops.fused_dcn_supported(m.in_channels, m.out_channels, m.deformable_groups, m.groups, m.padding, m.stride, m.dilation)):
        return ops.deform_conv_fused([x], [offset], ops.cached_dcn_pack(m.weight), m.bias, m.in_channels, m.out_channels, m.kernel_size,
                                     m.stride, m.padding, m.dilation, relu=relu)[0]
    y = m(x, offset)
    return torch.relu_(y) if relu else y


def head_norm(with_norm):
    assert with_norm in ['batch_norm', 'group_norm', 'none']
    if with_norm == 'batch_norm':
        raise NotImplementedError(
            "with_norm='batch_norm': the reference takes this layer from upsnet/operators/modules/distbatchnorm.py (a synchronised "
            "BatchNorm2d imported only under Horovod + syncbn), which is not part of its tree -- there is no BatchNorm2d to reproduce; "
            "use 'group_norm' or 'none'")
    return None if with_norm == 'none' else (lambda num_channels: nn.GroupNorm(32, num_channels))


def norm_supported(gn, x):
    return (ENABLED and isinstance(gn, nn.GroupNorm) and gn.affine and x.is_cuda and x.dim() in (2, 4) and x.shape[1] == gn.num_channels and
            group_norm.supported(gn.num_channels, gn.num_groups))


def _norm_library(gn, x, relu, residual, residual_up):
    _library(gn, x, 'hipconv.norm_supported() is false')
    y = gn(x)
    if residual is not None:
        y = y + (F.interpolate(residual, scale_factor=2, mode='nearest') if residual_up else residual)
    return F.relu(y, inplace=True) if relu else y


def norm(gn, x, relu=False, residual=None, residual_up=False):
    if norm_supported(gn, x):
        if x.dim() == 2 or (residual is None and x.shape[2] * x.shape[3] <= group_norm.chunk_pixels()):
            y = group_norm.group_norm_small(x, gn.weight, gn.bias, gn.eps, relu=relu)
            form = 'gn rows' if x.dim() == 2 or x.shape[2] * x.shape[3] == 1 else 'gn small'
        else:
            y, form = group_norm.group_norm(x, gn.weight, gn.bias, gn.eps, relu=relu, residual=residual, residual_up=residual_up), 'gn'
    else:
        y, form = _norm_library(gn, x, relu, residual, residual_up), 'library'
    _trace('gn', module=gn, x=x, out=y, relu=relu, residual=residual, residual_up=residual_up, form=form)
    return y


def norm_multi(gn, xs, relu=False):
    xs = list(xs)
    if 1 <= len(xs) <= group_norm.MAX_MAPS and all(x.dim() == 4 and norm_supported(gn, x) for x in xs):
        ys = group_norm.group_norm_multi(xs, gn.weight, gn.bias, gn.eps, relu=relu)
        for x, y in zip(xs, ys):
            _trace('gn', module=gn, x=x, out=y, relu=relu, residual=None, residual_up=False, form='gn multi')
        return ys
    return [norm(gn, x, relu=relu) for x in xs]


def clear_cache(model=None):
    if model is not None:
        for m in model.modules():
            m.__dict__.pop('_hip_plans', None)
            for p in m.parameters(recurse=False):
                p.__dict__.pop('_hip_plans', None)
```

upsnet_amd/models/resnet.py:

```python
import warnings

import torch
import torch.nn as nn

from ..config.config import config
from ..operators.modules.deform_conv import DeformConv
from . import hipconv


def _frozen_bn(ch):
    bn = nn.BatchNorm2d(ch)
    bn.eval()
    for p in bn.parameters():
        p.requires_grad = False
    return bn


class _Block(nn.Module):
    expansion = 4
    deformable = False
    feeds_deformable = False

    def __init__(self, inplanes, planes, stride=1, dilation=1, downsample=None, fix_bn=True, deformable_group=1):
        super().__init__()
        make_bn = _frozen_bn if fix_bn else nn.BatchNorm2d
        self.conv1 = nn.Conv2d(inplanes, planes, 1, stride=stride, bias=False)
        self.bn1 = make_bn(planes)
        if self.deformable:
            self.conv2_offset = nn.Conv2d(planes, 18 * deformable_group, 3, padding=1)
            nn.init.zeros_(self.conv2_offset.weight)
            nn.init.zeros_(self.conv2_offset.bias)
            self.conv2 = DeformConv(planes, planes, 3, stride=1, padding=dilation, dilation=dilation, bias=False)
        else:
            self.conv2 = nn.Conv2d(planes, planes, 3, padding=dilation, dilation=dilation, bias=False)
        self.bn2 = make_bn(planes)
        self.conv3 = nn.Conv2d(planes, planes * self.expansion, 1, bias=False)
        self.bn3 = make_bn(planes * self.expansion)
        self.downsample = downsample
        self.stride = stride

    def forward(self, x):
        if isinstance(self.bn1, nn.Identity):
            return self.forward_chain(x)[0]
        y = torch.relu_(self.bn1(self.conv1(x)))
        y = self.conv2(y, self.conv2_offset(y)) if self.deformable else self.conv2(y)
        y = torch.relu_(self.bn2(y))
        y = self.bn3(self.conv3(y))
        y += x if self.downsample is None else self.downsample(x)
        return torch.relu_(y)


    def forward_chain(self, x, y1=None, nxt=None):
        if y1 is None and hipconv.use_block(self, x):
            return hipconv.block(self, x), None
        ad = hipconv.act_dtype()
        shortcut = None
        if y1 is None and self.downsample is not None and hipconv.use_siblings(self.conv1, self.downsample[0], x):
            y, shortcut = hipconv.conv_siblings(self.conv1, self.downsample[0], x)
        else:
            y = hipconv.conv(self.conv1, x, relu=True, out_dtype=torch.float32 if self.deformable else ad) if y1 is None else y1
        if self.deformable:
            off = hipconv.conv(self.conv2_offset, y)
            y, y_in = hipconv.dcn(self.conv2, y, off, relu=True), y
            hipconv._trace('dcn', module=self.conv2, xs=[y_in], offsets=[off], outs=[y], relu=True, 
                           form='dcn_fused' + (' bf16' if hipconv.ops.dcn_precision() == 'bf16' else ''))
        else:
            y = hipconv.conv(self.conv2, y, relu=True, out_dtype=ad, winograd='f2x2' if self.feeds_deformable else True)
        if shortcut is None:
            shortcut = x if self.downsample is None else hipconv.conv(self.downsample[0], x, out_dtype=ad)
        if nxt is not None and isinstance(nxt.bn1, nn.Identity) and hipconv.use_pair(self.conv3, nxt.conv1, y, shortcut):
            return hipconv.conv_pair(self.conv3, nxt.conv1, y, shortcut)
        return hipconv.conv(self.conv3, y, relu=True, residual=shortcut, out_dtype=ad), None


class Bottleneck(_Block):
    deformable = False


class DCNBottleneck(_Block):
    deformable = True


class conv1(nn.Module):

    def __init__(self, requires_grad=False):
        super().__init__()
        self.conv1 = nn.Conv2d(3, 64, 7, stride=2, padding=3, bias=False)
        self.bn1 = nn.BatchNorm2d(64)
        if not requires_grad:
            self.eval()
            for p in self.parameters():
                p.requires_grad = False

    def forward(self, x):
        if isinstance(self.bn1, nn.Identity) and hipconv.use_stem_pool(self.conv1, x):
            return hipconv.stem_pool(self.conv1, x)
        if isinstance(self.bn1, nn.Identity):
            return nn.functional.max_pool2d(hipconv.conv_stem(self.conv1, x, relu=True), 3, stride=2, padding=1)
        return nn.functional.max_pool2d(torch.relu_(self.bn1(self.conv1(x))), 3, stride=2, padding=1)


class res_block(nn.Module):

    def __init__(self, planes, blocks, block=Bottleneck, stride=1, dilation=1, fix_bn=True, with_dpyramid=False):
        super().__init__()
        width_in = planes if planes == 64 else planes * 2
        width_out = planes * block.expansion
        proj = None
        if stride != 1 or width_in != width_out:
            proj = nn.Sequential(nn.Conv2d(width_in, width_out, 1, stride=stride, bias=False),
                                 _frozen_bn(width_out) if fix_bn else nn.BatchNorm2d(width_out))
        kinds = [block] * blocks
        if with_dpyramid:
            kinds[-1] = DCNBottleneck
        mods = [kinds[0](width_in, planes, stride, dilation, proj, fix_bn)]
        mods += [k(width_out, planes, dilation=dilation, fix_bn=fix_bn) for k in kinds[1:]]
        self.layers = nn.Sequential(*mods)

    def forward(self, x):
        blocks = list(self.layers)
        if not all(isinstance(b.bn1, nn.Identity) for b in blocks):
            return self.layers(x)
        y1 = None
        for i, blk in enumerate(blocks):
            x, y1 = blk.forward_chain(x, y1, blocks[i + 1] if i + 1 < len(blocks) else None)
        return x


class ResNetBackbone(nn.Module):

    def __init__(self, blocks):
        super().__init__()
        net = config.network
        self.fix_bn, self.freeze_at = net.backbone_fix_bn, net.backbone_freeze_at
        dconv_from = net.backbone_with_dconv
        r5 = dict(stride=1, dilation=2) if net.backbone_with_dilation else dict(stride=2, dilation=1)
        self.conv1 = conv1(requires_grad=False)
        self.res2 = res_block(64, blocks[0], fix_bn=self.fix_bn)
        for idx, (planes, n, kw) in enumerate([(128, blocks[1], dict(stride=2, with_dpyramid=net.backbone_with_dpyramid)),
                                               (256, blocks[2], dict(stride=2, with_dpyramid=net.backbone_with_dpyramid)),
                                               (512, blocks[3], r5)], start=3):
            kind = DCNBottleneck if dconv_from <= idx else Bottleneck
            setattr(self, 'res%d' % idx, res_block(planes, n, block=kind, fix_bn=self.fix_bn, **kw))
        blocks_in_order = [b for name in ('res2', 'res3', 'res4', 'res5') for b in getattr(self, name).layers]
        last_dcn = max([i for i, b in enumerate(blocks_in_order) if b.deformable], default=-1)
        for b in blocks_in_order[:last_dcn + 1]:
            b.feeds_deformable = not b.deformable

    def forward(self, x):
        feats = []
        x = self.conv1(x)
        for name in ('res2', 'res3', 'res4', 'res5'):
            x = getattr(self, name)(x)
            feats.append(x)
        return tuple(feats)


def _fold(conv, bn):
    with torch.no_grad():
        scale = bn.weight / torch.sqrt(bn.running_var + bn.eps)
        shift = bn.bias - bn.running_mean * scale
        conv.weight.mul_(scale.view(-1, 1, 1, 1))
        if conv.bias is None:
            conv.bias = nn.Parameter(shift.clone(), requires_grad=False)
        else:
            conv.bias.mul_(scale).add_(shift)


def fold_frozen_bn(module):
    for m in module.modules():
        if isinstance(m, _Block):
            for c, b in (('conv1', 'bn1'), ('conv2', 'bn2'), ('conv3', 'bn3')):
                if isinstance(getattr(m, b), nn.BatchNorm2d):
                    _fold(getattr(m, c), getattr(m, b))
                    setattr(m, b, nn.Identity())
            if m.downsample is not None and isinstance(m.downsample[1], nn.BatchNorm2d):
                _fold(m.downsample[0], m.downsample[1])
                m.downsample[1] = nn.Identity()
        elif isinstance(m, conv1) and isinstance(m.bn1, nn.BatchNorm2d):
            _fold(m.conv1, m.bn1)
            m.bn1 = nn.Identity()
    return module


_TORCHVISION_STAGE = {'layer1': 'res2', 'layer2': 'res3', 'layer3': 'res4', 'layer4': 'res5'}


class resnet_rcnn(nn.Module):

    def name_mapping(self, name, resume=False):
        if resume:
            return name[len('module.'):] if name.startswith('module.') else name
        if name.startswith(('conv1', 'bn1')):
            return 'resnet_backbone.conv1.' + name
        for tv, ours in _TORCHVISION_STAGE.items():
            name = name.replace(tv, 'resnet_backbone.%s.layers' % ours)
        return name

    def load_state_dict(self, state_dict, resume=False, strict=False):
        own = self.state_dict()
        mapped = {self.name_mapping(k, resume): v for k, v in state_dict.items()}
        for key, val in mapped.items():
            if key not in own:
                warnings.warn('unexpected key "%s" in state_dict' % key)
            elif own[key].shape != val.shape:
                warnings.warn('shape mismatch for %s: model %s vs checkpoint %s' % (key, tuple(own[key].shape), tuple(val.shape)))
            else:
                own[key].copy_(val.data if isinstance(val, nn.Parameter) else val)
        missing = sorted(set(own) - set(mapped))
        if missing:
            warnings.warn('missing keys in state_dict: %s' % missing)
```

upsnet_amd/ops.py:

```python
import os

import numpy as np
import torch

from . import _lib
from ._lib import addr, check, f32c, float_array, i32c, i64c, int_array, lib, nhwc, ptr, ptr_array, require_cuda, stream, written


PROFILE = {'enabled': False, 'events': []}


def _prof_begin():
    if not PROFILE['enabled']:
        return None
    ev0 = torch.cuda.Event(enable_timing=True)
    ev0.record()
    return ev0


def _prof_end(ev0, kind, flops, nbytes, label=None):
    ev1 = torch.cuda.Event(enable_timing=True)
    ev1.record()
    PROFILE['events'].append((kind, ev0, ev1, flops, nbytes) if label is None else (kind, ev0, ev1, flops, nbytes, label))

# ... 1182 lines not shown
            if per.max(initial=0) > 255:
                raise ValueError("combined_pan_result: image %d class %d has %d candidates at or above the score threshold; the "
                                 "instance ids are uint8" % (i, int(per.argmax()), int(per.max())))
            for k in order:
                cnt = rl[k]['counts']
                if not isinstance(cnt, (str, bytes)):
                    raise ValueError("combined_pan_result: image %d: RLE counts must be a compressed string" % i)
                strings.append(cnt)
            cls_of.append(cls)
        npix_of.append(np.full(len(order) if sc else 0, H * W, np.int64))
        img_ncand.append(len(order) if sc else 0)
    cls_all = np.concatenate(cls_of) if cls_of else np.zeros(0, np.int32)
    npix_all = np.concatenate(npix_of)
    counts, off = decode_rle_strings(strings)
    ncodes = np.diff(off)
    str_of = np.repeat(np.arange(len(strings)), ncodes)
    if counts.size and counts.min() < 0:
        raise ValueError("combined_pan_result: negative RLE count (string %d)" % int(str_of[np.argmax(counts < 0)]))
    total = np.bincount(str_of, weights=counts.astype(np.float64), minlength=len(strings))
    bad = np.flatnonzero(total != npix_all)
    if bad.size:
        raise ValueError("combined_pan_result: RLE counts of candidate %d sum to %d, not H * W = %d" %
                         (int(bad[0]), int(total[bad[0]]), int(npix_all[bad[0]])))
    first = np.zeros(counts.size, bool)
    first[off[:-1][ncodes > 0]] = True
    pos = _segmented_cumsum(counts, first) if counts.size else counts
    j = np.arange(counts.size) - np.repeat(off[:-1], ncodes)
    odd = np.flatnonzero(((j & 1) == 1) & (counts > 0))
    run_b = pos[odd]
    run_a = run_b - counts[odd]
    run_str = str_of[odd]
    area = np.bincount(run_str, weights=(run_b - run_a).astype(np.float64), minlength=len(strings)).astype(np.int64)
    blk_a, blk_b = run_a // _SEG_BLOCK, (run_b - 1) // _SEG_BLOCK
    nseg = blk_b - blk_a + 1
    run_idx = np.repeat(np.arange(run_a.size), nseg)
    blk = blk_a[run_idx] + (np.arange(run_idx.size) - np.repeat(np.cumsum(nseg) - nseg, nseg))
    seg_a = np.maximum(run_a[run_idx], blk * _SEG_BLOCK)
    seg_b = np.minimum(run_b[run_idx], (blk + 1) * _SEG_BLOCK)
    seg_str = run_str[run_idx]
    seg_cnt = np.bincount(seg_str, minlength=len(strings))
    keep = area > 0
    cand_img = np.repeat(np.arange(n), img_ncand)
    out = [torch.empty((int(t.shape[0]), int(t.shape[1]), 3), dtype=torch.uint8, device=dev) for t in seg_t]
    live = [i for i in range(n) if seg_t[i].numel()]
    chunks, cur, cur_pix = [], [], 0
    for i in live:
        p = seg_t[i].numel()
        if cur and (len(cur) >= COMBINED_PAN_CHUNK_IMAGES or cur_pix + p > COMBINED_PAN_CHUNK_PIXELS):
            chunks.append(cur)
            cur, cur_pix = [], 0
        cur.append(i)
        cur_pix += p
    if cur:
        chunks.append(cur)
    for ch in chunks:
        in_chunk = keep & np.isin(cand_img, ch)
        sel = np.flatnonzero(in_chunk)
        cbeg = np.concatenate([[0], np.cumsum(np.bincount(np.searchsorted(ch, cand_img[sel]), minlength=len(ch)))])
        segs_sel = np.flatnonzero(in_chunk[seg_str])
        c_seg_end = np.cumsum(seg_cnt[sel])
        cand = np.stack([cls_all[sel], area[sel], c_seg_end - seg_cnt[sel], c_seg_end], 1).astype(np.int32) if sel.size else None
        segs_np = np.stack([seg_a[segs_sel], seg_b[segs_sel]], 1).astype(np.int32) if segs_sel.size else None
        hw = np.array([[int(seg_t[i].shape[0]), int(seg_t[i].shape[1])] for i in ch], np.int64)
        npx = hw[:, 0] * hw[:, 1]
        img = np.zeros((len(ch), 8), np.int64)
        img[:, 0:2] = hw
        img[:, 2] = [addr(seg_t[i]) for i in ch]
        img[:, 3] = [addr(out[i]) for i in ch]
        img[:, 4], img[:, 5] = cbeg[:-1], cbeg[1:]
        img[:, 6] = np.concatenate([[0], np.cumsum((npx + 63) // 64)[:-1]])
        img[:, 7] = np.concatenate([[0], np.cumsum(npx)[:-1]])
        total_pix = int(npx.sum())
        img_d = torch.from_numpy(img).to(dev)
        cand_d = torch.from_numpy(cand).to(dev) if cand is not None else None
        segs_d = torch.from_numpy(segs_np).to(dev) if segs_np is not None else None
        ws = torch.empty((int(lib().upsnet_combined_pan_workspace_bytes(len(ch), total_pix)),), dtype=torch.uint8, device=dev)
        check(lib().upsnet_combined_pan_result(stream(), len(ch), ptr(img_d), int(hw[:, 0].max()), int(hw[:, 1].max()), total_pix,
                                               ptr(cand_d), ptr(segs_d), int(id_last_stuff), num_classes, int(stuff_area_limit),
                                               float(fraction_threshold), ptr(ws)), "combined_pan_result")
    return out


def pq_workspace(max_gt, device):
    nbytes = int(lib().upsnet_pq_workspace_bytes(int(max_gt)))
    if nbytes == 0:
        raise ValueError("pq_workspace: max_gt %d outside 0..4096" % max_gt)
    return torch.zeros((nbytes,), dtype=torch.uint8, device=device)


def pq_accumulate(pred_2ch, gt_rgb, segments, cat_known, image_index, max_gt, workspace, tp, fp, fn, iou, status):
    require_cuda(pred_2ch, gt_rgb, segments, cat_known, workspace, tp, fp, fn, iou, status)
    if pred_2ch.dtype != torch.uint8 or gt_rgb.dtype != torch.uint8 or pred_2ch.dim() != 3 or pred_2ch.shape[2] != 3 \
            or tuple(pred_2ch.shape) != tuple(gt_rgb.shape):
        raise ValueError("pq_accumulate: pred_2ch %s %s and gt_rgb %s %s must both be uint8 [H,W,3]"
                         % (tuple(pred_2ch.shape), pred_2ch.dtype, tuple(gt_rgb.shape), gt_rgb.dtype))
    if segments.dtype != torch.int64 or segments.dim() != 2 or segments.shape[1] != 4:
        raise ValueError("pq_accumulate: segments must be int64 [n,4]")
    for t, dt, n in ((cat_known, torch.uint8, 256), (tp, torch.int64, 256), (fp, torch.int64, 256), (fn, torch.int64, 256),
                     (iou, torch.float64, 256), (status, torch.int64, 1)):
        if t.dtype != dt or t.numel() != n or not t.is_contiguous():
            raise ValueError("pq_accumulate: accumulator / table of %d %s expected, got %s %s" % (n, dt, tuple(t.shape), t.dtype))
    written(workspace, None, "pq_accumulate: workspace")
    pred_2ch, gt_rgb, segments = pred_2ch.contiguous(), gt_rgb.contiguous(), segments.contiguous()
    H, W = pred_2ch.shape[:2]
    check(lib().upsnet_pq_accumulate(stream(), ptr(pred_2ch), ptr(gt_rgb), H, W, ptr(segments) if segments.numel() else None,
                                     int(segments.shape[0]), ptr(cat_known), int(image_index), int(max_gt), ptr(workspace), ptr(tp), ptr(fp),
                                     ptr(fn), ptr(iou), ptr(status)), "pq_accumulate")


def pq_boundary_workspace(max_gt, height, width, device):
    nbytes = int(lib().upsnet_pq_boundary_workspace_bytes(int(max_gt), int(height), int(width)))
    if nbytes == 0:
        raise ValueError("pq_boundary_workspace: max_gt %d outside 0..4096 or image size %dx%d out of range" % (max_gt, height, width))
    return torch.zeros((nbytes,), dtype=torch.uint8, device=device)


def pq_boundary_accumulate(dilation, pred_2ch, gt_rgb, segments, cat_known, image_index, max_gt, workspace, tp, fp, fn, iou, status):
    require_cuda(pred_2ch, gt_rgb, segments, cat_known, workspace, tp, fp, fn, iou, status)
    if pred_2ch.dtype != torch.uint8 or gt_rgb.dtype != torch.uint8 or pred_2ch.dim() != 3 or pred_2ch.shape[2] != 3 \
            or tuple(pred_2ch.shape) != tuple(gt_rgb.shape):
        raise ValueError("pq_boundary_accumulate: pred_2ch %s %s and gt_rgb %s %s must both be uint8 [H,W,3]"
                         % (tuple(pred_2ch.shape), pred_2ch.dtype, tuple(gt_rgb.shape), gt_rgb.dtype))
    if segments.dtype != torch.int64 or segments.dim() != 2 or segments.shape[1] != 4:
        raise ValueError("pq_boundary_accumulate: segments must be int64 [n,4]")
    for t, dt, n in ((cat_known, torch.uint8, 256), (tp, torch.int64, 256), (fp, torch.int64, 256), (fn, torch.int64, 256),
                     (iou, torch.float64, 256), (status, torch.int64, 1)):
        if t.dtype != dt or t.numel() != n or not t.is_contiguous():
            raise ValueError("pq_boundary_accumulate: accumulator / table of %d %s expected, got %s %s" % (n, dt, tuple(t.shape), t.dtype))
    if int(dilation) < 1:
        raise ValueError("pq_boundary_accumulate: dilation %d < 1" % dilation)
    H, W = pred_2ch.shape[:2]
    need = int(lib().upsnet_pq_boundary_workspace_bytes(int(max_gt), H, W))
    if need == 0 or workspace.dtype != torch.uint8 or not workspace.is_contiguous() or workspace.numel() < need:
        raise ValueError("pq_boundary_accumulate: a uint8 workspace of at least %d bytes expected for max_gt %d and %dx%d, got %s %s"
                         % (need, max_gt, H, W, tuple(workspace.shape), workspace.dtype))
    pred_2ch, gt_rgb, segments = pred_2ch.contiguous(), gt_rgb.contiguous(), segments.contiguous()
    check(lib().upsnet_pq_boundary_accumulate(stream(), int(dilation), ptr(pred_2ch), ptr(gt_rgb), H, W,
                                              ptr(segments) if segments.numel() else None, int(segments.shape[0]), ptr(cat_known),
                                              int(image_index), int(max_gt), ptr(workspace), ptr(tp), ptr(fp), ptr(fn), ptr(iou), ptr(status)),
          "pq_boundary_accumulate")


def pan_boundary_workspace_bytes(height, width):
    nbytes = int(lib().upsnet_pan_boundary_workspace_bytes(int(height), int(width)))
    if nbytes == 0:
        raise ValueError("pan_boundary_map: image size %dx%d out of range" % (height, width))
    return nbytes


def pan_boundary_map(dilation, pred_2ch, gt_rgb, workspace, out):
    maps = [m for m in (pred_2ch, gt_rgb) if m is not None]
    if not maps:
        raise ValueError("pan_boundary_map: neither pred_2ch nor gt_rgb given")
    require_cuda(workspace, out, *maps)
    for m in maps:
        if m.dtype != torch.uint8 or m.dim() != 3 or m.shape[2] != 3 or tuple(m.shape) != tuple(maps[0].shape):
            raise ValueError("pan_boundary_map: maps must be uint8 [H,W,3] of one shape, got %s %s" % (tuple(m.shape), m.dtype))
    if int(dilation) < 1:
        raise ValueError("pan_boundary_map: dilation %d < 1" % dilation)
    H, W = maps[0].shape[:2]
    nbytes = pan_boundary_workspace_bytes(H, W)
    if workspace.dtype != torch.uint8 or not workspace.is_contiguous() or workspace.numel() < nbytes:
        raise ValueError("pan_boundary_map: a uint8 workspace of at least %d bytes expected, got %s %s"
                         % (nbytes, tuple(workspace.shape), workspace.dtype))
    if out.dtype != torch.uint8 or tuple(out.shape) != (H, W) or not out.is_contiguous():
        raise ValueError("pan_boundary_map: out must be a contiguous uint8 [%d,%d], got %s %s" % (H, W, tuple(out.shape), out.dtype))
    pred_2ch = pred_2ch.contiguous() if pred_2ch is not None else None
    gt_rgb = gt_rgb.contiguous() if gt_rgb is not None else None
    with torch.cuda.device(out.device):
        check(lib().upsnet_pan_boundary_map(stream(), int(dilation), ptr(pred_2ch) if pred_2ch is not None else None,
                                            ptr(gt_rgb) if gt_rgb is not None else None, H, W, ptr(workspace), ptr(out)), "pan_boundary_map")
    return out


def confusion_accumulate(gt_label, pred_label, class_num, ignore_label, confusion):
    require_cuda(gt_label, pred_label, confusion)
    if gt_label.dtype != torch.uint8 or pred_label.dtype != torch.uint8 or gt_label.shape != pred_label.shape:
        raise ValueError("confusion_accumulate: gt %s %s and pred %s %s must both be uint8 of one shape"
                         % (tuple(gt_label.shape), gt_label.dtype, tuple(pred_label.shape), pred_label.dtype))
    if confusion.dtype != torch.int64 or tuple(confusion.shape) != (class_num, class_num) or not confusion.is_contiguous():
        raise ValueError("confusion_accumulate: confusion must be a contiguous int64 [%d,%d] tensor" % (class_num, class_num))
    gt_label, pred_label = gt_label.contiguous(), pred_label.contiguous()
    check(lib().upsnet_confusion_accumulate(stream(), ptr(gt_label), ptr(pred_label), int(gt_label.numel()), int(class_num),
                                            int(ignore_label), ptr(confusion)), "confusion_accumulate")
    return confusion


def mask_roi_dedup(a_src, a_cls, a_num, b_src, b_cls, b_boxes, b_num):
    require_cuda(a_src, b_src, b_boxes)
    cap_a, cap_b = a_src.shape[0], b_src.shape[0]
    dev = b_boxes.device
    mp = torch.empty((cap_b,), dtype=torch.int32, device=dev)
    extra = torch.empty((cap_b, 5), dtype=torch.float32, device=dev)
    n_extra = torch.empty((1,), dtype=torch.int32, device=dev)
    a_src, a_cls, a_num = i32c(a_src), i64c(a_cls), i32c(a_num)
    b_src, b_cls, b_boxes, b_num = i32c(b_src), i64c(b_cls), f32c(b_boxes), i32c(b_num)
    check(lib().upsnet_mask_roi_dedup(stream(), ptr(a_src), ptr(a_cls), ptr(a_num), cap_a, ptr(b_src), ptr(b_cls), ptr(b_boxes),
                                      ptr(b_num), cap_b, ptr(mp), ptr(extra), ptr(n_extra)), "mask_roi_dedup")
    return mp, extra, n_extra


def pack_winograd_weight(weight, tn32=False):
    require_cuda(weight)
    weight = f32c(weight)
    Cout, Cin, kh, kw = weight.shape
    if (kh, kw) != (3, 3):
        raise RuntimeError("pack_winograd_weight: kernel must be 3x3")
    if tn32:
        ldw = (Cout + 31) // 32 * 32
        wp = torch.empty((16 * Cin, ldw), dtype=torch.float32, device=weight.device)
        check(lib().upsnet_conv_pack_weight_winograd_tn32(stream(), ptr(weight), Cout, Cin, ldw, ptr(wp)), "conv_pack_weight_winograd_tn32")
        return wp, ldw
    ldw = 32 if Cout <= 32 else (Cout + 63) // 64 * 64
    wp = torch.empty((16 * Cin, ldw), dtype=torch.float32, device=weight.device)
    check(lib().upsnet_conv_pack_weight_winograd(stream(), ptr(weight), Cout, Cin, ldw, ptr(wp)), "conv_pack_weight_winograd")
    return wp, ldw


def conv2d_winograd_splitk(x, wpack, ldw, bias, cout, ksplit, relu=False, residual=None):
    require_cuda(x, wpack)
    wpack = f32c(wpack)
    x = nhwc(x.float())
    N, C, H, W = x.shape
    out = _nhwc_out(N, cout, H, W, x.device)
    res = None
    if residual is not None:
        res = nhwc(residual.float())
        if tuple(res.shape) != tuple(out.shape):
            raise RuntimeError("conv2d_winograd_splitk: residual shape %s != %s" % (tuple(res.shape), tuple(out.shape)))
    ws = _ws(lib().upsnet_conv2d_splitk_workspace_bytes(N, H, W, int(cout), 3, 3, 1, 1, int(ksplit)), x.device)
    ev0 = _prof_begin()
    bias = None if bias is None else f32c(bias)
    check(lib().upsnet_conv2d_winograd_nhwc_f32_splitk(stream(), ptr(x), ptr(res), ptr(out), N, H, W, C, ptr(wpack), int(ldw),
                                                       ptr(bias), int(cout), int(bool(relu)), int(ksplit),
                                                       ptr(ws)), "conv2d_winograd_nhwc_f32_splitk")
    if ev0 is not None:
        npix = N * H * W
        _prof_end(ev0, 'conv', 2.0 * cout * C * 9 * npix, 4.0 * (C * npix + cout * npix * (2 if res is not None else 1) + cout * C * 9),
                  "winograd split-K x%d 3x3/1 %d->%d %s" % (ksplit, C, cout, (N, H, W)))
    return out


def conv2d_winograd_tail(x, wpack, ldw, wpack32, ldw32, bias, cout, n_main, relu=False):
    require_cuda(wpack, wpack32, x)
    wpack, wpack32 = f32c(wpack), f32c(wpack32)
    x = nhwc(x.float())
    N, C, H, W = x.shape
    out = _nhwc_out(N, cout, H, W, x.device)
    ev0 = _prof_begin()
    bias = None if bias is None else f32c(bias)
    check(lib().upsnet_conv2d_winograd_nhwc_f32_tail(stream(), ptr(x), ptr(out), int(N), int(n_main), int(H), int(W), int(C), ptr(wpack), int(ldw),
                                                     ptr(wpack32), int(ldw32), ptr(bias), int(cout),
                                                     int(bool(relu))), "conv2d_winograd_nhwc_f32_tail")
    if ev0 is not None:
        npix = N * H * W
        _prof_end(ev0, 'conv', 2.0 * cout * C * 9 * npix, 4.0 * (C * npix + cout * npix + cout * C * 9),
                  "winograd 3x3/1 %d->%d [%s] tail %d" % (C, cout, (N, H, W), N - n_main))
    return out


def conv2d_winograd_multi(xs, wpack, ldw, bias, cout, relu=False, residuals=None, outs=None, tn32=False):
    require_cuda(wpack, *xs)
    wpack = f32c(wpack)
    assert 1 <= len(xs) <= 5
    xs = [nhwc(x.float()) for x in xs]
    cin = xs[0].shape[1]
    given, outs, ress = outs, [], None
    for i, x in enumerate(xs):
        N, C, H, W = x.shape
        if C != cin:
            raise RuntimeError("conv2d_winograd_multi: channel mismatch")
        if given is not None:
            o = given[i]
            if tuple(o.shape) != (N, cout, H, W) or o.dtype != torch.float32 or not o.permute(0, 2, 3, 1).is_contiguous():
                raise RuntimeError("conv2d_winograd_multi: outs[%d] must be a channels_last fp32 [%d,%d,%d,%d]" % (i, N, cout, H, W))
            outs.append(o)
        else:
            outs.append(_nhwc_out(N, cout, H, W, x.device))
    if residuals is not None:
        ress = [nhwc(r.float()) for r in residuals]
        for r, o in zip(ress, outs):
            if tuple(r.shape) != tuple(o.shape):
                raise RuntimeError("conv2d_winograd: residual shape %s != %s" % (tuple(r.shape), tuple(o.shape)))
    ev0 = _prof_begin()
    fn = lib().upsnet_conv2d_winograd_nhwc_f32_tn32 if tn32 else lib().upsnet_conv2d_winograd_nhwc_f32
    bias = None if bias is None else f32c(bias)
    check(fn(stream(), len(xs), ptr_array(xs), ptr_array(ress) if ress is not None else None,
             ptr_array(outs), int_array([x.shape[0] for x in xs]), int_array([x.shape[2] for x in xs]),
             int_array([x.shape[3] for x in xs]), int(cin), ptr(wpack), int(ldw),
             ptr(bias), int(cout), int(bool(relu))),
          "conv2d_winograd_nhwc_f32")
    if ev0 is not None:
        npix = sum(o.shape[0] * o.shape[2] * o.shape[3] for o in outs)
        _prof_end(ev0, 'conv', 2.0 * cout * cin * 9 * npix, 4.0 * (cin * npix + cout * npix * (2 if ress is not None else 1) + cout * cin * 9),
                  "winograd 3x3/1 %d->%d %s%s%s" % (cin, cout, [tuple(x.shape[0:1] + x.shape[2:]) for x in xs],
                                                    " +res" if ress is not None else "", " tn32" if tn32 else ""))
    return outs


def pack_winograd36_weight(weight):
    require_cuda(weight)
    weight = f32c(weight)
    Cout, Cin, kh, kw = weight.shape
    if (kh, kw) != (3, 3) or Cin % 32:
        raise RuntimeError("pack_winograd36_weight: 3x3 kernel and Cin %% 32 == 0")
    ldw = (Cout + 63) // 64 * 64
    wp = torch.empty((36 * Cin, ldw), dtype=torch.float32, device=weight.device)
    check(lib().upsnet_conv_pack_weight_winograd36(stream(), ptr(weight), Cout, Cin, ldw, ptr(wp)), "conv_pack_weight_winograd36")
    return wp, ldw


def conv2d_winograd36_multi(xs, wpack, ldw, bias, cout, relu=False, outs=None):
    require_cuda(wpack, *xs)
    wpack = f32c(wpack)
    assert 1 <= len(xs) <= 5
    xs = [nhwc(x.float()) for x in xs]
    cin = xs[0].shape[1]
    given, outs = outs, []
    for i, x in enumerate(xs):
        N, C, H, W = x.shape
        if C != cin:
            raise RuntimeError("conv2d_winograd36_multi: channel mismatch")
        if given is not None:
            o = given[i]
            if tuple(o.shape) != (N, cout, H, W) or o.dtype != torch.float32 or not o.permute(0, 2, 3, 1).is_contiguous():
                raise RuntimeError("conv2d_winograd36_multi: outs[%d] must be a channels_last fp32 [%d,%d,%d,%d]" % (i, N, cout, H, W))
            outs.append(o)
        else:
            outs.append(_nhwc_out(N, cout, H, W, x.device))
    ev0 = _prof_begin()
    bias = None if bias is None else f32c(bias)
    check(lib().upsnet_conv2d_winograd36_nhwc_f32(stream(), len(xs), ptr_array(xs), ptr_array(outs), int_array([x.shape[0] for x in xs]),
                                                  int_array([x.shape[2] for x in xs]), int_array([x.shape[3] for x in xs]), int(cin), ptr(wpack),
                                                  int(ldw), ptr(bias), int(cout), int(bool(relu))),
          "conv2d_winograd36_nhwc_f32")
    if ev0 is not None:
        npix = sum(o.shape[0] * o.shape[2] * o.shape[3] for o in outs)
        _prof_end(ev0, 'conv', 2.0 * cout * cin * 9 * npix, 4.0 * (cin * npix + cout * npix + cout * cin * 9),
                  "winograd36 3x3/1 %d->%d %s" % (cin, cout, [tuple(x.shape[0:1] + x.shape[2:]) for x in xs]))
    return outs


def conv2d_winograd36_splitk(x, wpack, ldw, bias, cout, ksplit, relu=False):
    require_cuda(wpack, x)
    wpack = f32c(wpack)
    x = nhwc(x.float())
    N, cin, H, W = x.shape
    out = _nhwc_out(N, cout, H, W, x.device)
    ws = _ws(lib().upsnet_conv2d_winograd36_splitk_workspace_bytes(N, H, W, int(cout), int(ksplit)), x.device)
    ev0 = _prof_begin()
    bias = None if bias is None else f32c(bias)
    check(lib().upsnet_conv2d_winograd36_nhwc_f32_splitk(stream(), ptr(x), ptr(out), N, H, W, int(cin), ptr(wpack), int(ldw),
                                                         ptr(bias), int(cout), int(bool(relu)), int(ksplit), ptr(ws)),
          "conv2d_winograd36_nhwc_f32_splitk")
    if ev0 is not None:
        npix = N * H * W
        _prof_end(ev0, 'conv', 2.0 * cout * cin * 9 * npix, 4.0 * (cin * npix + cout * npix + cout * cin * 9),
                  "winograd36 split-K x%d 3x3/1 %d->%d %s" % (ksplit, cin, cout, (N, H, W)))
    return out


def pack_conv_weight_bf16(weight, split=True):
    require_cuda(weight)
    weight = f32c(weight)
    Cout, Cin, kh, kw = weight.shape
    ldw = (Cout + 127) // 128 * 128
    shape = (kh * kw * Cin // 32, ldw, 32)
    hi = torch.empty(shape, dtype=torch.bfloat16, device=weight.device)
    lo = torch.empty(shape, dtype=torch.bfloat16, device=weight.device) if split else None
    check(lib().upsnet_conv_pack_weight_bf16(stream(), ptr(weight), Cout, Cin, kh, kw, ldw, ptr(hi), ptr(lo)), "conv_pack_weight_bf16")
    return hi, lo, ldw


def conv2d_nhwc_bf16_multi(xs, whi, wlo, ldw, bias, cout, ksize, stride, pad, relu=False, residuals=None, residual_up=False,
                           out_dtype=torch.float32):
    require_cuda(whi, *xs)
    whi, wlo = whi.contiguous(), None if wlo is None else wlo.contiguous()
    assert 1 <= len(xs) <= 5
    in16 = xs[0].dtype == torch.bfloat16
    out16 = out_dtype == torch.bfloat16
    if (in16 or out16) and wlo is not None:
        raise RuntimeError("conv2d_nhwc_bf16_multi: bf16 tensors only in the plain bf16 mode")
    xs = [nhwc(x if (in16 and x.dtype == torch.bfloat16) else x.float()) for x in xs]
    if in16 and any(x.dtype != torch.bfloat16 for x in xs):
        raise RuntimeError("conv2d_nhwc_bf16_multi: mixed input dtypes in one launch")
    cin = xs[0].shape[1]
    outs, ress = [], None
    for x in xs:
        N, C, H, W = x.shape
        if C != cin:
            raise RuntimeError("conv2d_nhwc_bf16_multi: channel mismatch")
        Ho, Wo = (H + 2 * pad - ksize) // stride + 1, (W + 2 * pad - ksize) // stride + 1
        outs.append(torch.empty((N, Ho, Wo, cout), dtype=torch.bfloat16, device=x.device).permute(0, 3, 1, 2) if out16
                    else _nhwc_out(N, cout, Ho, Wo, x.device))
    res16 = False
    if residuals is not None:
        res16 = residuals[0].dtype == torch.bfloat16 and wlo is None
        ress = [nhwc(r if (res16 and r.dtype == torch.bfloat16) else r.float()) for r in residuals]
        if res16 and any(r.dtype != torch.bfloat16 for r in ress):
            raise RuntimeError("conv2d_nhwc_bf16_multi: mixed residual dtypes in one launch")
        for r, o in zip(ress, outs):
            want = (o.shape[0], o.shape[1], o.shape[2] // 2, o.shape[3] // 2) if residual_up else tuple(o.shape)
            if tuple(r.shape) != want:
                raise RuntimeError("conv2d_nhwc_bf16: residual shape %s != %s" % (tuple(r.shape), want))
    ev0 = _prof_begin()
    bias = None if bias is None else f32c(bias)
    check(lib().upsnet_conv2d_nhwc_bf16(stream(), len(xs), ptr_array(xs), ptr_array(ress) if ress is not None else None, ptr_array(outs),
                                        int_array([x.shape[0] for x in xs]), int_array([x.shape[2] for x in xs]),
                                        int_array([x.shape[3] for x in xs]), int(cin), ptr(whi), ptr(wlo), int(ldw),
                                        ptr(bias), int(cout), int(ksize), int(ksize), int(stride), int(pad),
                                        int(bool(relu)) | (2 if (residual_up and ress is not None) else 0) | (4 if in16 else 0) |
                                        (8 if out16 else 0) | (16 if res16 else 0)), "conv2d_nhwc_bf16")
    if ev0 is not None:
        npix = sum(o.shape[0] * o.shape[2] * o.shape[3] for o in outs)
        nin = sum(x.shape[0] * x.shape[2] * x.shape[3] for x in xs)
        _prof_end(ev0, 'conv_bf16', 2.0 * cout * cin * ksize * ksize * npix,
                  (2.0 if in16 else 4.0) * cin * nin + (2.0 if out16 else 4.0) * cout * npix +
                  ((2.0 if res16 else 4.0) * cout * npix * (0.25 if residual_up else 1.0) if ress is not None else 0.0) +
                  2.0 * cout * cin * ksize * ksize)
    return outs


def _bf16_fragments(w2d):
    cout, k = w2d.shape
    return w2d.to(torch.bfloat16).view(cout // 32, 32, k // 16, 2, 8).permute(0, 2, 3, 1, 4).contiguous()


def pack_bottleneck_bf16(w1, w2, w3, b1, b2, b3):
    require_cuda(w1, w2, w3)
    cm, c = w1.shape[0], w1.shape[1]
    if not (c == 4 * cm and tuple(w2.shape) == (cm, cm, 3, 3) and tuple(w3.shape) == (c, cm, 1, 1) and cm in (64, 128, 256, 512)):
        raise RuntimeError("pack_bottleneck_bf16: not an identity bottleneck of width 64/128/256/512")
    zeros = lambda n: torch.zeros(n, dtype=torch.float32, device=w1.device)
    return (_bf16_fragments(w1.detach().float().reshape(cm, c)),
            _bf16_fragments(w2.detach().float().permute(0, 2, 3, 1).reshape(cm, 9 * cm)),
            _bf16_fragments(w3.detach().float().reshape(c, cm)),
            zeros(cm) if b1 is None else f32c(b1.detach()), zeros(cm) if b2 is None else f32c(b2.detach()),
            zeros(c) if b3 is None else f32c(b3.detach()), cm)


def pack_bottleneck_proj_bf16(w1, w2, w3, wd, b1, b2, b3, bd):
    require_cuda(w1, w2, w3, wd)
    cm, cin = w1.shape[0], w1.shape[1]
    c = 4 * cm
    if not (tuple(w2.shape) == (cm, cm, 3, 3) and tuple(w3.shape) == (c, cm, 1, 1) and tuple(wd.shape) == (c, cin, 1, 1) and
            (cm, cin) in ((64, 64), (128, 256), (256, 512))):
        raise RuntimeError("pack_bottleneck_proj_bf16: not the first bottleneck of res2 / res3 / res4")
    z = lambda b, n: torch.zeros(n, dtype=torch.float32, device=w1.device) if b is None else f32c(b.detach())
    w3d = torch.cat([w3.detach().float().reshape(c, cm), wd.detach().float().reshape(c, cin)], 1)
    return (_bf16_fragments(w1.detach().float().reshape(cm, cin)),
            _bf16_fragments(w2.detach().float().permute(0, 2, 3, 1).reshape(cm, 9 * cm)),
            _bf16_fragments(w3d), z(b1, cm), z(b2, cm), (z(b3, c) + z(bd, c)).contiguous(), cm, cin)


def bottleneck_proj_bf16(x, pack, stride):
    w1, w2, w3d, b1, b2, b3d, cm, cin = pack
    require_cuda(x, w1)
    w1, w2, w3d, b1, b2, b3d = w1.contiguous(), w2.contiguous(), w3d.contiguous(), f32c(b1), f32c(b2), f32c(b3d)
    if x.dtype != torch.bfloat16 or x.shape[1] != cin:
        raise RuntimeError("bottleneck_proj_bf16: expects a bf16 map of %d channels" % cin)
    x = nhwc(x)
    N, C, H, W = x.shape
    Ho, Wo = (H - 1) // stride + 1, (W - 1) // stride + 1
    out = torch.empty((N, Ho, Wo, 4 * cm), dtype=torch.bfloat16, device=x.device).permute(0, 3, 1, 2)
    ev0 = _prof_begin()
    check(lib().upsnet_bottleneck_proj_bf16(stream(), ptr(x), ptr(out), N, H, W, int(cin), int(cm), int(stride), ptr(w1), ptr(w2), ptr(w3d),
                                            ptr(b1), ptr(b2), ptr(b3d)), "bottleneck_proj_bf16")
    if ev0 is not None:
        k = cm * cin + 9 * cm * cm + 4 * cm * (cm + cin)
        _prof_end(ev0, 'bottleneck_bf16', 2.0 * k * N * Ho * Wo, 2.0 * C * N * Ho * Wo + 2.0 * 4 * cm * N * Ho * Wo + 2.0 * k)
    return out


def bottleneck_bf16(x, pack):
    w1, w2, w3, b1, b2, b3, cm = pack
    require_cuda(x, w1)
    w1, w2, w3, b1, b2, b3 = w1.contiguous(), w2.contiguous(), w3.contiguous(), f32c(b1), f32c(b2), f32c(b3)
    if x.dtype != torch.bfloat16 or x.shape[1] != 4 * cm:
        raise RuntimeError("bottleneck_bf16: expects a bf16 map of %d channels" % (4 * cm))
    x = nhwc(x)
    N, C, H, W = x.shape
    out = torch.empty((N, H, W, C), dtype=torch.bfloat16, device=x.device).permute(0, 3, 1, 2)
    ev0 = _prof_begin()
    check(lib().upsnet_bottleneck_bf16(stream(), ptr(x), ptr(out), N, H, W, cm, ptr(w1), ptr(w2), ptr(w3), ptr(b1), ptr(b2), ptr(b3)),
          "bottleneck_bf16")
    if ev0 is not None:
        _prof_end(ev0, 'bottleneck_bf16', 2.0 * 17 * cm * cm * N * H * W, 2.0 * 2 * C * N * H * W + 2.0 * 17 * cm * cm)
    return out


def conv2d_nhwc_splitk(x, wpack, ldw, bias, cout, ksize, stride, pad, ksplit, relu=False, residual=None):
    require_cuda(x, wpack)
    wpack = f32c(wpack)
    x = nhwc(x.float())
    N, C, H, W = x.shape
    Ho, Wo = (H + 2 * pad - ksize) // stride + 1, (W + 2 * pad - ksize) // stride + 1
    out = _nhwc_out(N, cout, Ho, Wo, x.device)
    res = None
    if residual is not None:
        res = nhwc(residual.float())
        if tuple(res.shape) != tuple(out.shape):
            raise RuntimeError("conv2d_nhwc_splitk: residual shape %s != %s" % (tuple(res.shape), tuple(out.shape)))
    ws = _ws(lib().upsnet_conv2d_splitk_workspace_bytes(N, H, W, int(cout), int(ksize), int(ksize), int(stride), int(pad), int(ksplit)), x.device)
    ev0 = _prof_begin()
    bias = None if bias is None else f32c(bias)
    check(lib().upsnet_conv2d_nhwc_f32_splitk(stream(), ptr(x), ptr(res), ptr(out), N, H, W, C, ptr(wpack), int(ldw),
                                              ptr(bias), int(cout), int(ksize), int(ksize), int(stride),
                                              int(pad), int(bool(relu)), int(ksplit), ptr(ws)), "conv2d_nhwc_f32_splitk")
    if ev0 is not None:
        npix = N * Ho * Wo
        _prof_end(ev0, 'conv', 2.0 * cout * C * ksize * ksize * npix,
                  4.0 * (C * N * H * W + cout * npix * (2 if res is not None else 1) + cout * C * ksize * ksize),
                  "split-K x%d %dx%d/%d %d->%d %s" % (ksplit, ksize, ksize, stride, C, cout, (N, H, W)))
    return out


PROPOSAL_RECALL_MAX_GT = 4096


def proposal_recall_workspace_bytes(num_problems, total_proposals):
    return int(lib().upsnet_proposal_recall_workspace_bytes(int(num_problems), int(total_proposals)))


def proposal_recall(problems, proposals, gt_boxes, max_gt, total_proposals, workspace, out):
    require_cuda(problems, proposals, gt_boxes, workspace, out)
    if problems.dtype != torch.int64 or problems.dim() != 2 or problems.shape[1] != 6 or not problems.is_contiguous():
        raise ValueError("proposal_recall: problems must be a contiguous int64 [n, 6] table, got %s %s" % (problems.dtype, tuple(problems.shape)))
    for name, b in (('proposals', proposals), ('gt_boxes', gt_boxes)):
        if b.dtype != torch.float32 or b.dim() != 2 or b.shape[1] != 4 or not b.is_contiguous():
            raise ValueError("proposal_recall: %s must be contiguous float32 [., 4], got %s %s" % (name, b.dtype, tuple(b.shape)))
    if not 0 <= int(max_gt) <= PROPOSAL_RECALL_MAX_GT:
        raise ValueError("proposal_recall: %d GT boxes in a problem (at most %d)" % (int(max_gt), PROPOSAL_RECALL_MAX_GT))
    n = int(problems.shape[0])
    written(workspace, None, "proposal_recall: workspace")
    if workspace.numel() * workspace.element_size() < proposal_recall_workspace_bytes(n, total_proposals):
        raise ValueError("proposal_recall: workspace of %d bytes, %d needed" % (workspace.numel() * workspace.element_size(),
                                                                             proposal_recall_workspace_bytes(n, total_proposals)))
    if out.dtype != torch.float32 or not out.is_contiguous():
        raise ValueError("proposal_recall: out must be contiguous float32")
    check(lib().upsnet_proposal_recall(stream(), n, ptr(problems), ptr(proposals), ptr(gt_boxes), int(max_gt), int(total_proposals),
                                       ptr(workspace), ptr(out)), "proposal_recall")
    return out


def gt_prepare_workspace(device, seg_capacity=4096):
    from .dataset import gt_prepare as impl
    return impl.gt_prepare_workspace(device, seg_capacity)


def gt_prepare_launch(ids, tables, label_ids=None, seg_capacity=4096, trans_capacity=None, workspace=None):
    from .dataset import gt_prepare as impl
    return impl.gt_prepare_launch(ids, tables, label_ids, seg_capacity, trans_capacity, workspace)


def gt_prepare(ids, tables, label_ids=None, seg_capacity=4096, trans_capacity=None, workspace=None):
    from .dataset import gt_prepare as impl
    return impl.gt_prepare(ids, tables, label_ids, seg_capacity, trans_capacity, workspace)


def panoptic_semantic(rgb, segments_info):
    from .dataset import gt_prepare as impl
    return impl.panoptic_semantic(rgb, segments_info)


TTA_MAX_AUG = 8


def tta_seg_merge(maps, q, resized_w, flip, cell):
    from . import tta as impl
    return impl.seg_merge(maps, q, resized_w, flip, cell)


def tta_roi_union(rois, delta, prob, num_rois_dev, r, resized_w, flip):
    from . import tta as impl
    return impl.roi_union(rois, delta, prob, num_rois_dev, r, resized_w, flip)


def tta_boxes_to_aug(boxes, q, resized_w, flip):
    from . import tta as impl
    return impl.boxes_to_aug(boxes, q, resized_w, flip)


def tta_mask_merge(logits, flip):
    from . import tta as impl
    return impl.mask_merge(logits, flip)


def box_vote(rois, bbox_delta, cls_prob, im_info, boxes, cls, num, vote_score_thresh, vote_iou_thresh, reg_weights,
             num_rois_dev=None, clip_boxes=True):
    from . import tta as impl
    return impl.box_vote(rois, bbox_delta, cls_prob, im_info, boxes, cls, num, vote_score_thresh, vote_iou_thresh, reg_weights,
                         num_rois_dev, clip_boxes)


def mask_roi_soft(rois, bbox_delta, cls_prob, im_info, score_thresh, nms_thresh, max_det, reg_weights, method, sigma, floor,
                  num_rois_dev=None, clip_boxes=True):
    from . import tta as impl
    return impl.mask_roi_soft(rois, bbox_delta, cls_prob, im_info, score_thresh, nms_thresh, max_det, reg_weights, method, sigma, floor,
                              num_rois_dev, clip_boxes)


def pan_track_step(pan_2ch, iou_thresh, max_age, frame, workspace, memory, out, host_table=None):
    return _pan_track_step("pan_track_step", pan_2ch, iou_thresh, max_age, frame, workspace, memory, out, host_table, None)


def pan_track_step_motion(pan_2ch, iou_thresh, max_age, frame, workspace, memory, out, motion_workspace, host_table=None):
    require_cuda(motion_workspace)
    if motion_workspace.dtype != torch.uint8 or not motion_workspace.is_contiguous() or motion_workspace.data_ptr() % 16:
        raise ValueError("pan_track_step_motion: motion_workspace must be a contiguous, 16-byte aligned uint8 tensor")
    return _pan_track_step("pan_track_step_motion", pan_2ch, iou_thresh, max_age, frame, workspace, memory, out, host_table, motion_workspace)


def _pan_track_step(what, pan_2ch, iou_thresh, max_age, frame, workspace, memory, out, host_table, motion_workspace):
    require_cuda(pan_2ch, workspace, memory, out)
    if pan_2ch.dtype != torch.uint8 or pan_2ch.dim() != 3 or pan_2ch.shape[2] != 3 or not pan_2ch.is_contiguous():
        raise ValueError("pan_track_step: pan_2ch must be contiguous uint8 [H,W,3], got %s %s" % (tuple(pan_2ch.shape), pan_2ch.dtype))
    H, W = int(pan_2ch.shape[0]), int(pan_2ch.shape[1])
    if out.dtype != torch.uint8 or tuple(out.shape) != (H, W, 3) or not out.is_contiguous():
        raise ValueError("pan_track_step: out must be contiguous uint8 [%d,%d,3], got %s %s" % (H, W, tuple(out.shape), out.dtype))
    if memory.dtype != torch.int16 or tuple(memory.shape) != (H, W) or not memory.is_contiguous():
        raise ValueError("pan_track_step: memory must be a contiguous int16 [%d,%d] tensor, got %s %s" % (H, W, tuple(memory.shape), memory.dtype))
    written(workspace, None, "pan_track_step: workspace")
    written(motion_workspace, None, "pan_track_step: motion_workspace")
    need = int(lib().upsnet_pan_track_workspace_bytes(H, W))
    if need == 0 or workspace.numel() * workspace.element_size() < need:
        raise ValueError("pan_track_step: workspace too small for (or no workspace exists for) a frame of %d x %d" % (H, W))
    host_rows = 0
    if host_table is not None:
        if host_table.is_cuda or not host_table.is_pinned() or host_table.dtype != torch.int32 or host_table.numel() < 8 \
                or not host_table.is_contiguous():
            raise ValueError("pan_track_step: host_table must be contiguous pinned int32 host memory of at least 8 ints")
        host_rows = (host_table.numel() - 8) // 8
    args = (stream(), ptr(pan_2ch), H, W, float(iou_thresh), int(max_age), int(frame), ptr(workspace), ptr(memory), ptr(out),
            ptr(host_table), host_rows)
    if motion_workspace is None:
        check(lib().upsnet_pan_track_step(*args), what)
    else:
        if motion_workspace.numel() < int(lib().upsnet_pan_track_motion_workspace_bytes(H, W)):
            raise ValueError("pan_track_step_motion: motion_workspace too small for a frame of %d x %d" % (H, W))
        check(lib().upsnet_pan_track_step_motion(*(args + (ptr(motion_workspace),))), what)
    return out


# ... 232 lines not shown
```

Baseline: 172.4.

## Add 32x32 Winograd F(4x4) form splitting K across wave pairs for small maps

Adds a KW instance of the F(4x4,3x3) Winograd kernel. Each workgroup covers 32 output channels instead of 64, and its two wave halves each take alternate K steps. The partial accumulators are then reduced through LDS before the epilogue. Single-map convs whose 32x64 grid would leave many CUs idle (FPN outputs, ResNet conv2 layers) are routed to it, doubling the workgroup count to raise CU fill, at the cost of an extra LDS reduction and half the per-workgroup reuse of the input transform.

```diff
diff --git a/include/upsnet_hip.h b/include/upsnet_hip.h
--- a/include/upsnet_hip.h
+++ b/include/upsnet_hip.h
@@ -192,6 +192,8 @@
 size_t upsnet_conv2d_winograd36_splitk_workspace_bytes(int batch, int height, int width, int Cout, int ksplit);
 int upsnet_conv2d_winograd36_nhwc_f32_splitk(void *stream, const float *x, float *out, int batch, int height, int width, int Cin,
                                              const float *wpack, int ldw, const float *bias, int Cout, int relu, int ksplit, void *workspace);
+int upsnet_conv2d_winograd36_nhwc_f32_kw(void *stream, const float *x, float *out, int batch, int height, int width, int Cin,
+                                         const float *wpack, int ldw, const float *bias, int Cout, int relu);
 
 size_t upsnet_conv1x1_ksw_packed_weight_floats(int cout, int cin);
 int upsnet_conv1x1_ksw_pack_weight(void *stream, const float *weight, int cout, int cin, float *wpack);
diff --git a/upsnet_amd/_lib.py b/upsnet_amd/_lib.py
--- a/upsnet_amd/_lib.py
+++ b/upsnet_amd/_lib.py
@@ -56,6 +56,7 @@
     "upsnet_conv3x3_ksw_nhwc_f32": (c_int, [P, P, P, c_int, c_int, c_int, c_int, P, P, c_int, c_int]),
     "upsnet_conv2d_winograd36_splitk_workspace_bytes": (ctypes.c_size_t, [c_int, c_int, c_int, c_int, c_int]),
     "upsnet_conv2d_winograd36_nhwc_f32_splitk": (c_int, [P, P, P, c_int, c_int, c_int, c_int, P, c_int, P, c_int, c_int, c_int, P]),
+    "upsnet_conv2d_winograd36_nhwc_f32_kw": (c_int, [P, P, P, c_int, c_int, c_int, c_int, P, c_int, P, c_int, c_int]),
     "upsnet_conv1x1_pair_nhwc_f32": (c_int, [P, P, P, P, P, c_long, c_int, P, P, c_int, P, P, c_int]),
     "upsnet_conv2d_nhwc_f32": (c_int, [P, c_int, P, P, P, P, P, P, c_int, P, c_int, P, c_int, c_int, c_int, c_int, c_int, c_int, c_int]),
     "upsnet_conv2d_nhwc_f32_multiw": (c_int, [P, c_int, P, P, P, P, P, c_int, P, c_int, c_int, c_int, c_int, c_int, c_int, c_int]),
diff --git a/upsnet_amd/csrc/conv_wino36.hip b/upsnet_amd/csrc/conv_wino36.hip
--- a/upsnet_amd/csrc/conv_wino36.hip
+++ b/upsnet_amd/csrc/conv_wino36.hip
@@ -35,9 +35,10 @@
         Y3 = __builtin_fmaf(3.375f, d2_, __builtin_fmaf(0.421875f, d1_, (M5)));                                      \
     }
 
-template <bool SK>
+template <bool SK, bool KW = false>
 __global__ void __launch_bounds__(512, 1) conv_wino36_f32_kernel(const ConvParams p)
 {
+    static_assert(!(SK && KW), "the K split over wave pairs has no split-K instance");
     extern __shared__ __attribute__((aligned(16))) unsigned char smem_raw[];
     const int tid = threadIdx.x, lane = tid & 63;
     const int wave = __builtin_amdgcn_readfirstlane(tid >> 6);
@@ -111,11 +112,12 @@
     constexpr unsigned XI_PITCH = 4 * W36_TM * 16;
     const unsigned fr_base0 = (unsigned)((lhalf * W36_TM + (l32 ^ W36_SWZ(lhalf))) * 16) + (unsigned)pg * 9u * XI_PITCH;
     const unsigned fr_base1 = (unsigned)(((2 + lhalf) * W36_TM + (l32 ^ W36_SWZ(2 + lhalf))) * 16) + (unsigned)pg * 9u * XI_PITCH;
-    const size_t waddr = reinterpret_cast<size_t>(p.w) + ((size_t)n_t * (size_t)nslabs_all + (size_t)s_first) * (W36_STEPS * W36_BSTEP);
+    const size_t waddr = reinterpret_cast<size_t>(p.w) + ((size_t)(KW ? n_t >> 1 : n_t) * (size_t)nslabs_all + (size_t)s_first) * (W36_STEPS * W36_BSTEP);
     const unsigned wlo = __builtin_amdgcn_readfirstlane((unsigned)waddr), whi = __builtin_amdgcn_readfirstlane((unsigned)(waddr >> 32));
     const __amdgpu_buffer_rsrc_t wrsrc = __builtin_amdgcn_make_buffer_rsrc(reinterpret_cast<void *>(((size_t)whi << 32) | wlo), 0,
                                                                             nslabs * (int)(W36_STEPS * W36_BSTEP), 0x00020000);
-    const unsigned b_lane = (unsigned)(lhalf * (W36_TN * 16) + (32 * cb + l32) * 16);
+    const unsigned b_lane = (unsigned)(lhalf * (W36_TN * 16) + (32 * (KW ? n_t & 1 : cb) + l32) * 16);
+    const unsigned fr_k = cb ? fr_base1 : fr_base0;
     const int gmax = nslabs * W36_STEPS - 1;
 
     floatx16 acc[9];
@@ -151,7 +153,7 @@
         breg[SLOT] = make_float4(__uint_as_float(v_.x), __uint_as_float(v_.y), __uint_as_float(v_.z), __uint_as_float(v_.w)); }
 
 #pragma unroll
-    for (int u = 0; u < W36_RING; ++u) W36_BLOAD(u, 18 * pg + u)
+    for (int u = 0; u < W36_RING; ++u) W36_BLOAD(u, KW ? 18 * pg + 2 * u + cb : 18 * pg + u)
     {
         const __amdgpu_buffer_rsrc_t xr = __builtin_amdgcn_make_buffer_rsrc(const_cast<char *>(xbase), 0, xbytes, 0x00020000);
 #pragma unroll
@@ -162,7 +164,7 @@
         for (int j = 0; j < 6; ++j) { W36_COLSTASH(j, st_base) }
     }
     __syncthreads();
-    float4 afr = *reinterpret_cast<const float4 *>(smem_raw + fr_base0);
+    float4 afr = *reinterpret_cast<const float4 *>(smem_raw + (KW ? fr_k : fr_base0));
 
     auto slab_loop = [&](auto fast_tag) __attribute__((always_inline)) {
     constexpr bool FAST = decltype(fast_tag)::value;
@@ -172,6 +174,32 @@
         const unsigned cur = (s & 1) ? W36_VBUF : 0u, nxt = W36_VBUF - cur;
         const unsigned sb = nxt + st_base;
         const int g0 = s * W36_STEPS + 18 * pg;
+        if constexpr (KW) {
+#pragma unroll
+        for (int u = 0; u < 9; ++u) {
+            if (u < 2) {
+#pragma unroll
+                for (int r = 3 * u; r < 3 * u + 3; ++r) { if constexpr (FAST) { W36_LOADROW_FAST(r, xr) } else { W36_LOADROW_SAFE(r, xr) } }
+            }
+            float4 afn;
+            if (u < 8) afn = *reinterpret_cast<const float4 *>(smem_raw + cur + fr_k + (unsigned)(u + 1) * XI_PITCH);
+            else afn = *reinterpret_cast<const float4 *>(smem_raw + nxt + fr_k);
+            if (u == 3 || u == 4) {
+#pragma unroll
+                for (int r = 3 * (u - 3); r < 3 * (u - 3) + 3; ++r) { if constexpr (FAST) { W36_FIXROW(r) } W36_ROWPASS(r) }
+            }
+            if (u >= 5 && u <= 7) { W36_COLSTASH(2 * (u - 5), sb) W36_COLSTASH(2 * (u - 5) + 1, sb) }
+            const float4 bf = breg[u % W36_RING];
+            acc[u] = __builtin_amdgcn_mfma_f32_32x32x2f32(afr.x, bf.x, acc[u], 0, 0, 0);
+            acc[u] = __builtin_amdgcn_mfma_f32_32x32x2f32(afr.y, bf.y, acc[u], 0, 0, 0);
+            acc[u] = __builtin_amdgcn_mfma_f32_32x32x2f32(afr.z, bf.z, acc[u], 0, 0, 0);
+            acc[u] = __builtin_amdgcn_mfma_f32_32x32x2f32(afr.w, bf.w, acc[u], 0, 0, 0);
+            W36_BLOAD(u % W36_RING, (u + W36_RING < 9 ? g0 : g0 + W36_STEPS - 18) + 2 * (u + W36_RING) + cb)
+            if (u == 7) __syncthreads();
+            afr = afn;
+            __builtin_amdgcn_sched_barrier(0);
+        }
+        } else {
 #pragma unroll
         for (int u = 0; u < 18; ++u) {
             if (u < 6) { if constexpr (FAST) { W36_LOADROW_FAST(u, xr) } else { W36_LOADROW_SAFE(u, xr) } }
@@ -199,6 +227,7 @@
             afr = afn;
             __builtin_amdgcn_sched_barrier(0);
         }
+        }
     }
     };
     if (risky) slab_loop(std::false_type{}); else slab_loop(std::true_type{});
@@ -218,16 +247,33 @@
         0, (int)obytes_, 0x00020000);
     float *xch = reinterpret_cast<float *>(smem_raw);
 #pragma unroll 1
-    for (int bb = 0; bb < 2; ++bb) {
+    for (int bb = 0; bb < (KW ? 1 : 2); ++bb) {
         __syncthreads();
-        if (cb == bb) {
+        if constexpr (KW) {
+            if (cb == 1) {
+#pragma unroll
+                for (int u = 0; u < 9; ++u)
+#pragma unroll
+                    for (int r = 0; r < 16; ++r) xch[(r * W36_PTS + 9 * pg + u) * 64 + lane] = acc[u][r];
+            }
+            __syncthreads();
+            if (cb == 0) {
+#pragma unroll
+                for (int u = 0; u < 9; ++u)
+#pragma unroll
+                    for (int r = 0; r < 16; ++r) {
+                        float *slot = &xch[(r * W36_PTS + 9 * pg + u) * 64 + lane];
+                        *slot = acc[u][r] + *slot;
+                    }
+            }
+        } else if (cb == bb) {
 #pragma unroll
             for (int u = 0; u < 9; ++u)
 #pragma unroll
                 for (int r = 0; r < 16; ++r) xch[(r * W36_PTS + 9 * pg + u) * 64 + lane] = acc[u][r];
         }
         __syncthreads();
-        const int co_ch = n_t * W36_TN + 32 * bb + l32;
+        const int co_ch = n_t * (KW ? 32 : W36_TN) + 32 * bb + l32;
         const bool co_ok = co_ch < p.Cout;
         const float bv = (p.bias != nullptr && co_ok) ? p.bias[co_ch] : 0.f;
 #pragma unroll 1
@@ -263,11 +309,12 @@
 }
 
 static int w36_fill(ConvParams &p, const char *who, int nseg, const float *const x[], float *const out[], const int batch[], const int height[],
-                    const int width[], int Cin, int Cout, const float *wpack, int ldw, const float *bias, int relu)
-{
-    UPS_REQUIRE(Cin > 0 && Cin % 32 == 0 && ldw % W36_TN == 0, "%s: Cin %% 32 == 0 and ldw %% 64 == 0 (got %d, %d)", who, Cin, ldw);
-    int rc = conv_fill(p, who, nseg, x, nullptr, nullptr, nullptr, out, batch, height, width, Cin, Cout, wpack, ldw, bias, 3, 3, 1, 1, 1, relu);
+                    const int width[], int Cin, int Cout, const float *wpack, int ldw, const float *bias, int relu, int cin_mult = 32)
+{
+    UPS_REQUIRE(Cin > 0 && Cin % cin_mult == 0 && ldw % W36_TN == 0, "%s: Cin %% %d == 0 and ldw %% 64 == 0 (got %d, %d)", who, cin_mult, Cin, ldw);
+    int rc = conv_fill(p, who, nseg, x, nullptr, nullptr, nullptr, out, batch, height, width, (Cin + 31) / 32 * 32, Cout, wpack, ldw, bias, 3, 3, 1, 1, 1, relu);
     if (rc) return rc;
+    p.Cin = Cin;
     UPS_REQUIRE((long)W36_PTS * Cin * ldw < (1L << 29), "%s: packed weight exceeds 2 GiB", who);
     int tiles = 0;
     for (int i = 0; i < nseg; ++i) {
@@ -298,6 +345,25 @@
     hipLaunchKernelGGL(conv_wino36_f32_kernel<false>, dim3(grid), dim3(512), W36_XCH, (hipStream_t)stream, p);
     UPS_CHECK_LAUNCH("conv_wino36_f32_kernel");
     ups_set_form("wino36<%d,%d>", W36_TM, W36_TN);
+    return 0;
+}
+
+extern "C" int upsnet_conv2d_winograd36_nhwc_f32_kw(void *stream, const float *x, float *out, int batch, int height, int width, int Cin,
+                                                    const float *wpack, int ldw, const float *bias, int Cout, int relu)
+{
+    const float *xs[1] = {x};
+    float *os[1] = {out};
+    const int nb[1] = {batch}, hh[1] = {height}, ww[1] = {width};
+    ConvParams p;
+    int rc = w36_fill(p, "conv2d_winograd36_nhwc_f32_kw", 1, xs, os, nb, hh, ww, Cin, Cout, wpack, ldw, bias, relu, 16);
+    if (rc) return rc;
+    p.n_tiles = (Cout + 31) / 32;
+    static std::atomic<unsigned long long> attr_dev{0};
+    UPS_ONCE_PER_DEVICE(attr_dev, UPS_CHECK_HIP(hipFuncSetAttribute(reinterpret_cast<const void *>(&conv_wino36_f32_kernel<false, true>), hipFuncAttributeMaxDynamicSharedMemorySize, W36_XCH)));
+    const int grid = 8 * ((p.m_tiles + 7) / 8) * p.n_tiles;
+    hipLaunchKernelGGL((conv_wino36_f32_kernel<false, true>), dim3(grid), dim3(512), W36_XCH, (hipStream_t)stream, p);
+    UPS_CHECK_LAUNCH("conv_wino36_f32_kernel<kw>");
+    ups_set_form("wino36<%d,%d> kw2", W36_TM, 32);
     return 0;
 }
 
diff --git a/upsnet_amd/knobs.py b/upsnet_amd/knobs.py
--- a/upsnet_amd/knobs.py
+++ b/upsnet_amd/knobs.py
@@ -60,6 +60,8 @@
     'UPSNET_SPLITK': ('1', 'models/hipconv.py', 'split-K forms for small maps'),
     'UPSNET_STEM_POOL': ('1', 'models/hipconv.py', 'fused stem + pool kernel (0: stem kernel + library pool)'),
     'UPSNET_WINO36': ('1', 'models/hipconv.py', 'largest 3x3 / stride 1 layers on the Winograd F(4x4,3x3) kernel'),
+    'UPSNET_WINO36_KW': ('0.5', 'models/hipconv.py', 'single maps with fewer 32 x 64 F(4x4) workgroups than CUs on the 32 x 32 form whose wave pairs split K '
+                                                   '(0: off; f <= 1: where its one round of workgroups fills at least f of the CUs)'),
     'UPSNET_WINO36_SPLITK': ('0', 'models/hipconv.py', 'res3 / res4 conv2 and FPN P4 on the split-K F(4x4) form (3-5 us per launch; more rounding error)'),
     'UPSNET_WINO36_PREFIX': ('0', 'models/hipconv.py', 'multi-map F(4x4) launches keep only the leading maps that fill whole rounds of workgroups (measured: no gain)'),
     'UPSNET_WINO36_ROI': ('1', 'models/hipconv.py', 'mask head (ROI batches) on the Winograd F(4x4,3x3) kernel (0: F(2x2) with the half-size tail)'),
diff --git a/upsnet_amd/models/fpn.py b/upsnet_amd/models/fpn.py
--- a/upsnet_amd/models/fpn.py
+++ b/upsnet_amd/models/fpn.py
@@ -80,10 +80,10 @@
             p4_plus = hipconv.conv(self.fpn_p4_1x1, res4, residual=self.fpn_upsample(p5_1x1))
             p3_plus = hipconv.conv(self.fpn_p3_1x1, res3, residual=self.fpn_upsample(p4_plus))
             p2_plus = hipconv.conv(self.fpn_p2_1x1, res2, residual=self.fpn_upsample(p3_plus))
-        p5 = hipconv.conv(self.fpn_p5, p5_1x1)
-        p4 = hipconv.conv(self.fpn_p4, p4_plus)
-        p3 = hipconv.conv(self.fpn_p3, p3_plus)
-        p2 = hipconv.conv(self.fpn_p2, p2_plus)
+        p5 = hipconv.conv(self.fpn_p5, p5_1x1, winograd='kw')
+        p4 = hipconv.conv(self.fpn_p4, p4_plus, winograd='kw')
+        p3 = hipconv.conv(self.fpn_p3, p3_plus, winograd='kw')
+        p2 = hipconv.conv(self.fpn_p2, p2_plus, winograd='kw')
         if hasattr(self, 'fpn_p6'):
             return p2, p3, p4, p5, self.fpn_p6(p5)
         return p2, p3, p4, p5
diff --git a/upsnet_amd/models/hipconv.py b/upsnet_amd/models/hipconv.py
--- a/upsnet_amd/models/hipconv.py
+++ b/upsnet_amd/models/hipconv.py
@@ -34,6 +34,7 @@
 WINO36_ROI = os.environ.get('UPSNET_WINO36_ROI', '1') != '0'
 WINO36_MIN_FILL = float(os.environ.get('UPSNET_WINO36_MIN_FILL', '0.65'))
 WINO36_SPLITK = os.environ.get('UPSNET_WINO36_SPLITK', '0') != '0'
+WINO36_KW = float(os.environ.get('UPSNET_WINO36_KW', '0.5'))
 SPLITK = os.environ.get('UPSNET_SPLITK', '1') != '0'
 CONV1X1 = os.environ.get('UPSNET_CONV1X1', '1') != '0'
 CONV1X1_MIN_WG = int(os.environ.get('UPSNET_CONV1X1_MIN_WG', '256'))
@@ -414,6 +415,14 @@
     return ks if ks >= 2 else 1
 
 
+def _use_winograd36_kw(m, x):
+    if not (WINO36_KW > 0 and WINO36 and WINOGRAD and _winograd36_shape_ok(m) and x.dtype == torch.float32 and m.in_channels >= 128):
+        return False
+    cus = _cus(x.device)
+    wgs = _wino36_workgroups(m, [x])[0]
+    return wgs < cus and WINO36_KW * cus <= 2 * wgs <= cus
+
+
 def _wino_choice(m, xs, always=False):
     if not (WINOGRAD and _plain(m, 3, 1) and m.in_channels % 16 == 0):
         return None
@@ -476,6 +485,9 @@
 
 
 def route(m, xs, residual=None, residual_up=False, winograd=True, pin=False, out_dtype=None, multi=False, cat=None):
+    kw_ok = winograd == 'kw'
+    if kw_ok:
+        winograd = True
     pinned, sfx, widen = pin or winograd == 'always', ' multi' if multi else '', {}
     if multi:
         if len(xs) > 5 or not all(supported(m, x) for x in xs):
@@ -504,6 +516,8 @@
                 return Route('wino36', 'winograd36 splitk%d' % ks, ksplit=ks, **widen)
         if _use_winograd36(m, xs):
             return Route('wino36', 'winograd36' + sfx, prefix=_wino36_round_prefix(m, xs), **widen)
+        if kw_ok and not multi and _use_winograd36_kw(m, x):
+            return Route('wino36', 'winograd36 kw2', tile=(32, 32), **widen)
     if winograd == 'always' and WINO36 and WINO36_ROI and bare and f32 and _winograd36_shape_ok(m) and x.shape[2] * x.shape[3] <= 1024:
         return Route('wino36', 'winograd36 roi', **widen)
     wino = _wino_choice(m, xs, winograd == 'always') if (winograd and not residual_up) else None
@@ -556,6 +570,8 @@
     wp, ldw = _winograd36_plan(m)
     if r.ksplit > 1:
         return [ops.conv2d_winograd36_splitk(xs[0], wp, ldw, m.bias, m.out_channels, r.ksplit, relu=relu)]
+    if r.tile == (32, 32):
+        return [ops.conv2d_winograd36_kw(xs[0], wp, ldw, m.bias, m.out_channels, relu=relu)]
     return ops.conv2d_winograd36_multi(xs, wp, ldw, m.bias, m.out_channels, relu=relu)
 
 
diff --git a/upsnet_amd/models/resnet.py b/upsnet_amd/models/resnet.py
--- a/upsnet_amd/models/resnet.py
+++ b/upsnet_amd/models/resnet.py
@@ -65,7 +65,7 @@
             hipconv._trace('dcn', module=self.conv2, xs=[y_in], offsets=[off], outs=[y], relu=True, 
                            form='dcn_fused' + (' bf16' if hipconv.ops.dcn_precision() == 'bf16' else ''))
         else:
-            y = hipconv.conv(self.conv2, y, relu=True, out_dtype=ad, winograd='f2x2' if self.feeds_deformable else True)
+            y = hipconv.conv(self.conv2, y, relu=True, out_dtype=ad, winograd='f2x2' if self.feeds_deformable else 'kw')
         if shortcut is None:
             shortcut = x if self.downsample is None else hipconv.conv(self.downsample[0], x, out_dtype=ad)
         if nxt is not None and isinstance(nxt.bn1, nn.Identity) and hipconv.use_pair(self.conv3, nxt.conv1, y, shortcut):
diff --git a/upsnet_amd/ops.py b/upsnet_amd/ops.py
--- a/upsnet_amd/ops.py
+++ b/upsnet_amd/ops.py
@@ -1508,8 +1508,8 @@
     require_cuda(weight)
     weight = f32c(weight)
     Cout, Cin, kh, kw = weight.shape
-    if (kh, kw) != (3, 3) or Cin % 32:
-        raise RuntimeError("pack_winograd36_weight: 3x3 kernel and Cin %% 32 == 0")
+    if (kh, kw) != (3, 3) or Cin % 16:
+        raise RuntimeError("pack_winograd36_weight: 3x3 kernel and Cin %% 16 == 0")
     ldw = (Cout + 63) // 64 * 64
     wp = torch.empty((36 * Cin, ldw), dtype=torch.float32, device=weight.device)
     check(lib().upsnet_conv_pack_weight_winograd36(stream(), ptr(weight), Cout, Cin, ldw, ptr(wp)), "conv_pack_weight_winograd36")
@@ -1534,17 +1534,38 @@
             outs.append(o)
         else:
             outs.append(_nhwc_out(N, cout, H, W, x.device))
+    kw = _W36_KW
+    if kw and len(xs) != 1:
+        raise RuntimeError("conv2d_winograd36_kw: one map per launch")
     ev0 = _prof_begin()
     bias = None if bias is None else f32c(bias)
-    check(lib().upsnet_conv2d_winograd36_nhwc_f32(stream(), len(xs), ptr_array(xs), ptr_array(outs), int_array([x.shape[0] for x in xs]),
-                                                  int_array([x.shape[2] for x in xs]), int_array([x.shape[3] for x in xs]), int(cin), ptr(wpack),
-                                                  int(ldw), ptr(bias), int(cout), int(bool(relu))),
-          "conv2d_winograd36_nhwc_f32")
+    if kw:
+        x = xs[0]
+        check(lib().upsnet_conv2d_winograd36_nhwc_f32_kw(stream(), ptr(x), ptr(outs[0]), x.shape[0], x.shape[2], x.shape[3], int(cin), ptr(wpack),
+                                                         int(ldw), ptr(bias), int(cout), int(bool(relu))),
+              "conv2d_winograd36_nhwc_f32_kw")
+    else:
+        check(lib().upsnet_conv2d_winograd36_nhwc_f32(stream(), len(xs), ptr_array(xs), ptr_array(outs), int_array([x.shape[0] for x in xs]),
+                                                      int_array([x.shape[2] for x in xs]), int_array([x.shape[3] for x in xs]), int(cin), ptr(wpack),
+                                                      int(ldw), ptr(bias), int(cout), int(bool(relu))),
+              "conv2d_winograd36_nhwc_f32")
     if ev0 is not None:
         npix = sum(o.shape[0] * o.shape[2] * o.shape[3] for o in outs)
         _prof_end(ev0, 'conv', 2.0 * cout * cin * 9 * npix, 4.0 * (cin * npix + cout * npix + cout * cin * 9),
-                  "winograd36 3x3/1 %d->%d %s" % (cin, cout, [tuple(x.shape[0:1] + x.shape[2:]) for x in xs]))
+                  "winograd36%s 3x3/1 %d->%d %s" % (" kw2" if kw else "", cin, cout, [tuple(x.shape[0:1] + x.shape[2:]) for x in xs]))
     return outs
+
+
+_W36_KW = False
+
+
+def conv2d_winograd36_kw(x, wpack, ldw, bias, cout, relu=False, out=None):
+    global _W36_KW
+    _W36_KW = True
+    try:
+        return conv2d_winograd36_multi([x], wpack, ldw, bias, cout, relu=relu, outs=None if out is None else [out])[0]
+    finally:
+        _W36_KW = False
 
 
 def conv2d_winograd36_splitk(x, wpack, ldw, bias, cout, ksplit, relu=False):
```

Result: no change. 173.6, median of 6 (+0.7%).
